# vseib/point-cloud-donkey

Hardware: AMD Instinct MI355X
Metric: objects/sec classified (ModelNet10-like, SHOT-352) (higher is better)
Workload: dtype f32; 1 GPU; configs[1]: ModelNet10-like test split, 16384 pts, 1024 uniform keypoints/object, SHOT-352 (Radius 0.4, LRF 0.3), exact kNN K=1 squared-L2, mean-shift bandwidth 0.6; points_per_object=16384, keypoints_per_object=1024, classes=10, codebook_words=102400, descriptor_dim=352, collective_world_size=1

## Files before the change

point-cloud-donkey_amd/csrc/common.h:

```cpp
#pragma once
#include <hip/hip_runtime.h>
#include <stdint.h>
#include <map>
#include <set>
#include <string>
#include <vector>
#include "../../include/ismhip.h"

#define ISM_WAVE 64

#define ISM_GRID_MAXDIM 32
#define ISM_GRID_MAXCELLS (ISM_GRID_MAXDIM * ISM_GRID_MAXDIM * ISM_GRID_MAXDIM)
#define ISM_GRID_STRIDE (ISM_GRID_MAXCELLS + 1)

#define ISM_GRID_XFRAC 3
struct GridMeta {
    float minv[3];
    float cell[3];
    float inv_cell[3];
    int   dim[3];
    float centroid[3];
    uint32_t n_finite;
};

struct ismhip_cloud {
    int n_obj = 0;
    uint32_t n_pts = 0;
    uint32_t max_pts = 0;
    std::vector<uint32_t> pt_off_h;
    uint32_t* pt_off = nullptr;
    const float *x = nullptr, *y = nullptr, *z = nullptr, *nx = nullptr, *ny = nullptr, *nz = nullptr;
    const uint32_t* rgba = nullptr;
    float4* sp4 = nullptr;
    float4* sn4 = nullptr;
    float4* slab4 = nullptr;
    uint32_t* cell_of_pt = nullptr;
    uint32_t* rank_of_pt = nullptr;
    uint32_t* members = nullptr;
    GridMeta* meta = nullptr;
    uint32_t* cell_start = nullptr;
    float requested_cell = 0.f;
    uint32_t* kp_perm = nullptr;
    size_t kp_perm_cap = 0;
    const float* kp_perm_key = nullptr;
    std::vector<uint32_t> kp_perm_off;
    uint16_t* cospair_code = nullptr;
    size_t cospair_code_cap = 0;
    bool cospair_code_valid = false;
    size_t cap_pts = 0; int cap_obj = 0; bool cap_color = false;
};

struct PcaImage {
    int m = 0;
    float* R = nullptr;
    unsigned short* f16t = nullptr;
    float* cn_scaled = nullptr;
    float* osc = nullptr;
    float sq = 1.f, sc = 1.f;
    float cmax2 = 0.f;
    float inv_sig2 = 1.f;
    float d_rel = 0.f;
    float dq_abs = 0.f, dc_abs = 0.f;
    float resid2 = 0.f;
    float energy = 0.f;
};

struct ismhip_codebook {
    int n_words = 0, dim = 0, dim_pad = 0, n_votes = 0, max_votes = 0, n_classes = 0;
    float* words = nullptr;
    int n_words_pad = 0;
    float* word_norm = nullptr;
    unsigned short* words_bf16_hi = nullptr;
    unsigned short* words_bf16_lo = nullptr;
    unsigned short* words_f16 = nullptr;
    unsigned short* words_f16t = nullptr;
    int ld16 = 0;
    float f16_scale = 1.f;
    bool words_nonneg = false;
    float max_norm2 = 0.f;
    float* word_weight = nullptr;
    uint32_t* vote_off = nullptr;
    float* vote_xyz = nullptr;
    float* vote_weight = nullptr;
    float* vote_class_weight = nullptr;
    uint32_t* vote_class = nullptr;
    uint32_t* vote_instance = nullptr;
    float* vote_bbox_quat = nullptr;
    float* vote_bbox_size = nullptr;
    float* class_sigma = nullptr;
    uint32_t* word_class = nullptr;
    float* word_keypoint = nullptr;
    ismhip_codebook* chi_shadow = nullptr;
    uint32_t* shadow_perm = nullptr;
    PcaImage pca, pca2;
    int8_t* bin_words = nullptr;
    int32_t* bin_norm = nullptr;
    int bin_ld = 0, bin_shift = 0;
};

struct TimerAcc {
    std::vector<std::pair<hipEvent_t, hipEvent_t>> pending;
    double ms = 0.0;
    int64_t launches = 0;
};

struct ismhip_ctx {
    int device = 0;
    hipStream_t stream = nullptr;
    bool own_stream = false;
    std::string err;
    bool timers_on = false;
    std::map<std::string, TimerAcc> timers;
    std::vector<hipEvent_t> event_pool;
    struct Slot { void* p = nullptr; size_t bytes = 0; };
    std::map<int, Slot> scratch;
    float* lut_srgb = nullptr;
    float* lut_sxyz = nullptr;
    std::vector<ismhip_cloud*> cloud_pool;
    uint32_t* truncated_d = nullptr;
    unsigned long long* ransac_counters_d = nullptr;
    uint32_t knn_stats[2] = {0, 0};
    std::set<const void*> attr_done;
    uint32_t knn_stage2_queries = 0;
    uint32_t knn_seed_launches = 0;
    bool knn_stage2_seed = true;
    bool knn_two_stage = true;
    bool knn_join = true;
    bool knn_qpanel2 = true;
    bool knn_half = false;
    int knn_splits = 0;
    int knn_t = 0;
    bool xcd_map = true;
    bool grid_fused = true;
    bool kp_order = true;
    float grid_xfrac = 0.f;
    int shot_var = 0;
    bool knn_hell_emit = true;
    bool knn_hellinger = true;
    int knn_t1 = 2;
    int knn_pre_step = 32;
    float knn_pre_gamma = 1.0f;
    bool knn_prepass = true;
    int knn_pca_m = -1;
    bool knn_stage2_t4 = false;
    bool codebook_light = false;
    int knn_pca_m2 = -1;
    uint32_t knn_pca_launches = 0;
    uint32_t knn_thr_overflow = 0;
    uint32_t knn_thr_mfma_launches = 0;
    bool knn_lk_fast = false;
    bool knn_lk_exact = false;
    float knn_lk_seed_scale = 1.0f;
    uint32_t knn_lk_stats[3] = {0, 0, 0};
    uint32_t knn_binary_launches = 0;
    uint32_t rank_launches = 0;
    int knn_mode = 0;
};

enum ScratchSlot {
    SCR_KP_OFF = 1, SCR_TIE_LIST, SCR_TIE_REC, SCR_TIE_KEYS, SCR_COUNTERS, SCR_KNN_CAND_IDX, SCR_KNN_CAND_VAL,
    SCR_QNORM, SCR_FPFH_FLAG, SCR_FPFH_LIST, SCR_FPFH_SPFH, SCR_FPFH_LOOKUP, SCR_SLOT_OFF, SCR_CLASS_BW,
    SCR_COMPACT_KEEP, SCR_COMPACT_POS, SCR_OBJ_COUNT, SCR_QPAD, SCR_LRF_COV, SCR_KNN_FLAGS, SCR_KNN_QSPLIT, SCR_MAX_REC, SCR_QNORM2, SCR_KNN_Q2, SCR_KNN_LIST2, SCR_TRAIN, SCR_TRAIN2, SCR_MAX_WORK, SCR_KMEANS, SCR_KNN_CLOCK, SCR_PCA, SCR_KNN_THR0, SCR_KNN_QSQRT, SCR_KNN_HELL_EMIT, SCR_KNN_THR, SCR_KNN_THR2, SCR_TRAIN_ACT, SCR_KNN_LK, SCR_KNN_LK2, SCR_KNN_LK3, SCR_PREFILTER, SCR_RANSAC, SCR_COSPAIR, SCR_KNNB_FLAG, SCR_KNNB_Q, SCR_KNNB_CAND, SCR_RANK, SCR_RANK_KNN
};

int  ism_set_err(ismhip_ctx* ctx, int code, const std::string& msg);
void* ism_scratch(ismhip_ctx* ctx, int slot, size_t bytes);
int  ism_lds_cap(ismhip_ctx* ctx, const void* kern, size_t bytes);

uint32_t* ism_upload_offsets(ismhip_ctx* ctx, int slot, const uint32_t* off_h, int n);
struct RaggedOffsets { uint32_t max_run = 0, total = 0; uint32_t* dev = nullptr; };
enum { RAGGED_START0 = 1,
       RAGGED_EMPTY = 2 };
int ism_ragged_offsets(ismhip_ctx* ctx, const std::string& name, const uint32_t* off_h, int n, int slot, int flags, RaggedOffsets* r);
int ism_offsets_from_counts(ismhip_ctx* ctx, int n, const uint32_t* cnt_d, uint32_t* off_h_out, uint32_t* max_run_out);
const uint32_t* ism_kp_order(ismhip_ctx* ctx, const ismhip_cloud* cloud, const uint32_t* kp_offsets_h, const uint32_t* ko,
                             const float* kpx, const float* kpy, const float* kpz, uint32_t maxk);

#define ISM_HIP(ctx, call)                                                                          \
    do {                                                                                            \
        hipError_t e__ = (call);                                                                    \
        if (e__ != hipSuccess)                                                                      \
            return ism_set_err((ctx), ISMHIP_ERR_HIP, std::string(#call) + ": " + hipGetErrorString(e__)); \
    } while (0)

#define ISM_CHECK_LAUNCH(ctx, name)                                                                 \
    do {                                                                                            \
        hipError_t e__ = hipGetLastError();                                                         \
        if (e__ != hipSuccess)                                                                      \
            return ism_set_err((ctx), ISMHIP_ERR_HIP, std::string("launch ") + name + ": " + hipGetErrorString(e__)); \
    } while (0)

struct TimerScope {
    ismhip_ctx* ctx; const char* name; hipEvent_t a = nullptr, b = nullptr;
    TimerScope(ismhip_ctx* c, const char* n);
    ~TimerScope();
};

#ifdef __HIPCC__
__device__ __forceinline__ int lane_id() { return threadIdx.x & 63; }

__device__ __forceinline__ float sqdist3(float ax, float ay, float az, float bx, float by, float bz) {
    float r = 0.f, d;
    d = ax - bx; r += d * d;
    d = ay - by; r += d * d;
    d = az - bz; r += d * d;
    return r;
}

template <int CTRL>
__device__ __forceinline__ int dpp_mov0(int v) { return __builtin_amdgcn_update_dpp(0, v, CTRL, 0xf, 0xf, false); }

__device__ __forceinline__ float wave_sum_f(float v) {
    v += __int_as_float(dpp_mov0<0xb1>(__float_as_int(v)));
    v += __int_as_float(dpp_mov0<0x4e>(__float_as_int(v)));
    v += __int_as_float(dpp_mov0<0x114>(__float_as_int(v)));
    v += __int_as_float(dpp_mov0<0x118>(__float_as_int(v)));
    v += __int_as_float(dpp_mov0<0x142>(__float_as_int(v)));
    v += __int_as_float(dpp_mov0<0x143>(__float_as_int(v)));
    return __int_as_float(__builtin_amdgcn_readlane(__float_as_int(v), 63));
}
__device__ __forceinline__ int wave_sum_i(int v) {
    v += dpp_mov0<0xb1>(v);
    v += dpp_mov0<0x4e>(v);
    v += dpp_mov0<0x114>(v);
    v += dpp_mov0<0x118>(v);
    v += dpp_mov0<0x142>(v);
    v += dpp_mov0<0x143>(v);
    return __builtin_amdgcn_readlane(v, 63);
}
template <int CTRL>
__device__ __forceinline__ int dpp_movi(int ident, int v) { return __builtin_amdgcn_update_dpp(ident, v, CTRL, 0xf, 0xf, false); }
__device__ __forceinline__ float wave_min_f(float v) {
    const int inf = 0x7f800000;
    v = fminf(v, __int_as_float(dpp_movi<0xb1>(inf, __float_as_int(v))));
    v = fminf(v, __int_as_float(dpp_movi<0x4e>(inf, __float_as_int(v))));
    v = fminf(v, __int_as_float(dpp_movi<0x114>(inf, __float_as_int(v))));
    v = fminf(v, __int_as_float(dpp_movi<0x118>(inf, __float_as_int(v))));
    v = fminf(v, __int_as_float(dpp_movi<0x142>(inf, __float_as_int(v))));
    v = fminf(v, __int_as_float(dpp_movi<0x143>(inf, __float_as_int(v))));
    return __int_as_float(__builtin_amdgcn_readlane(__float_as_int(v), 63));
}
template <int CTRL>
__device__ __forceinline__ unsigned long long dpp_min_u64(unsigned long long v) {
    const unsigned lo = (unsigned)dpp_movi<CTRL>(-1, (int)(unsigned)(v & 0xffffffffull)), hi = (unsigned)dpp_movi<CTRL>(-1, (int)(unsigned)(v >> 32));
    const unsigned long long o = ((unsigned long long)hi << 32) | lo;
    return o < v ? o : v;
}
__device__ __forceinline__ unsigned long long wave_min_u64(unsigned long long v) {
    v = dpp_min_u64<0xb1>(v); v = dpp_min_u64<0x4e>(v); v = dpp_min_u64<0x114>(v);
    v = dpp_min_u64<0x118>(v); v = dpp_min_u64<0x142>(v); v = dpp_min_u64<0x143>(v);
    const unsigned lo = (unsigned)__builtin_amdgcn_readlane((int)(unsigned)(v & 0xffffffffull), 63), hi = (unsigned)__builtin_amdgcn_readlane((int)(unsigned)(v >> 32), 63);
    return ((unsigned long long)hi << 32) | lo;
}
__device__ __forceinline__ float wave_max_f(float v) {
    const int ninf = (int)0xff800000;
    v = fmaxf(v, __int_as_float(dpp_movi<0xb1>(ninf, __float_as_int(v))));
    v = fmaxf(v, __int_as_float(dpp_movi<0x4e>(ninf, __float_as_int(v))));
    v = fmaxf(v, __int_as_float(dpp_movi<0x114>(ninf, __float_as_int(v))));
    v = fmaxf(v, __int_as_float(dpp_movi<0x118>(ninf, __float_as_int(v))));
    v = fmaxf(v, __int_as_float(dpp_movi<0x142>(ninf, __float_as_int(v))));
    v = fmaxf(v, __int_as_float(dpp_movi<0x143>(ninf, __float_as_int(v))));
    return __int_as_float(__builtin_amdgcn_readlane(__float_as_int(v), 63));
}
__device__ __forceinline__ uint32_t wave_max_u32(uint32_t v) {
    v = max(v, (uint32_t)dpp_mov0<0xb1>((int)v)); v = max(v, (uint32_t)dpp_mov0<0x4e>((int)v)); v = max(v, (uint32_t)dpp_mov0<0x114>((int)v));
    v = max(v, (uint32_t)dpp_mov0<0x118>((int)v)); v = max(v, (uint32_t)dpp_mov0<0x142>((int)v)); v = max(v, (uint32_t)dpp_mov0<0x143>((int)v));
    return (uint32_t)__builtin_amdgcn_readlane((int)v, 63);
}
template <int CTRL>
__device__ __forceinline__ unsigned long long dpp_mov0_u64(unsigned long long v) {
    const unsigned lo = (unsigned)dpp_mov0<CTRL>((int)(unsigned)(v & 0xffffffffull)), hi = (unsigned)dpp_mov0<CTRL>((int)(unsigned)(v >> 32));
    return ((unsigned long long)hi << 32) | lo;
}
__device__ __forceinline__ unsigned long long readlane63_u64(unsigned long long v) {
    const unsigned lo = (unsigned)__builtin_amdgcn_readlane((int)(unsigned)(v & 0xffffffffull), 63), hi = (unsigned)__builtin_amdgcn_readlane((int)(unsigned)(v >> 32), 63);
    return ((unsigned long long)hi << 32) | lo;
}
template <int CTRL>
__device__ __forceinline__ unsigned long long dpp_max_u64(unsigned long long v) { const unsigned long long o = dpp_mov0_u64<CTRL>(v); return o > v ? o : v; }
__device__ __forceinline__ unsigned long long wave_max_u64(unsigned long long v) {
    v = dpp_max_u64<0xb1>(v); v = dpp_max_u64<0x4e>(v); v = dpp_max_u64<0x114>(v);
    v = dpp_max_u64<0x118>(v); v = dpp_max_u64<0x142>(v); v = dpp_max_u64<0x143>(v);
    return readlane63_u64(v);
}
__device__ __forceinline__ unsigned long long wave_sum_u64(unsigned long long v) {
    v += dpp_mov0_u64<0xb1>(v); v += dpp_mov0_u64<0x4e>(v); v += dpp_mov0_u64<0x114>(v);
    v += dpp_mov0_u64<0x118>(v); v += dpp_mov0_u64<0x142>(v); v += dpp_mov0_u64<0x143>(v);
    return readlane63_u64(v);
}
__device__ __forceinline__ uint32_t wave_incl_scan_u32(uint32_t v) {
    int x = (int)v;
    x += dpp_mov0<0x111>(x); x += dpp_mov0<0x112>(x); x += dpp_mov0<0x114>(x); x += dpp_mov0<0x118>(x);
    x += __builtin_amdgcn_update_dpp(0, x, 0x142, 0xa, 0xf, false);
    x += __builtin_amdgcn_update_dpp(0, x, 0x143, 0xc, 0xf, false);
    return (uint32_t)x;
}
template <int NT>
struct BlockScan {
    uint32_t wave[NT / 64];
    uint32_t carry;
    __device__ __forceinline__ void init() {
        if (threadIdx.x == 0) carry = 0;
        __syncthreads();
    }
    __device__ __forceinline__ uint32_t step(uint32_t v) {
        const uint32_t incl = wave_incl_scan_u32(v);
        const int w = threadIdx.x >> 6;
        if (lane_id() == 63) wave[w] = incl;
        __syncthreads();
        uint32_t before = carry;
        for (int k = 0; k < w; ++k) before += wave[k];
        __syncthreads();
        if (threadIdx.x == NT - 1) carry = before + incl;
        __syncthreads();
        return before + incl - v;
// ... 256 lines not shown
```

point-cloud-donkey_amd/csrc/ctx.hip:

```cpp
#include "common.h"
#include <cmath>
#include <cstring>
#include <cstdlib>

extern "C" void ism_cloud_pool_release(ismhip_ctx* ctx);

int ism_set_err(ismhip_ctx* ctx, int code, const std::string& msg) {
    if (ctx) ctx->err = msg;
    return code;
}

int ism_lds_cap(ismhip_ctx* ctx, const void* kern, size_t bytes) {
    if (ctx->attr_done.count(kern)) return ISMHIP_OK;
    ISM_HIP(ctx, hipFuncSetAttribute(kern, hipFuncAttributeMaxDynamicSharedMemorySize, (int)bytes));
    ctx->attr_done.insert(kern);
    return ISMHIP_OK;
}

void* ism_scratch(ismhip_ctx* ctx, int slot, size_t bytes) {
    if (bytes == 0) bytes = 16;
    auto& s = ctx->scratch[slot];
    if (s.bytes >= bytes) return s.p;
    if (s.p) { (void)hipStreamSynchronize(ctx->stream); (void)hipFree(s.p); s.p = nullptr; s.bytes = 0; }
    size_t want = bytes + bytes / 4;
    void* p = nullptr;
    if (hipMalloc(&p, want) != hipSuccess) { ism_set_err(ctx, ISMHIP_ERR_NOMEM, "scratch hipMalloc failed"); return nullptr; }
    s.p = p; s.bytes = want;
    return p;
}

TimerScope::TimerScope(ismhip_ctx* c, const char* n) : ctx(c), name(n) {
    if (!ctx->timers_on) return;
    auto get = [&]() {
        hipEvent_t e = nullptr;
        if (!ctx->event_pool.empty()) { e = ctx->event_pool.back(); ctx->event_pool.pop_back(); }
        else (void)hipEventCreate(&e);
        return e;
    };
    a = get(); b = get();
    (void)hipEventRecord(a, ctx->stream);
}
TimerScope::~TimerScope() {
    if (!a) return;
    (void)hipEventRecord(b, ctx->stream);
    ctx->timers[name].pending.emplace_back(a, b);
}

extern "C" {

int ismhip_abi_version(void) { return ISMHIP_ABI_VERSION; }

static int ctx_create_impl(int device, void* stream, bool own, ismhip_ctx** out);

int ismhip_ctx_create(int device, void* stream, ismhip_ctx** out) { return ctx_create_impl(device, stream, stream == nullptr, out); }
int ismhip_ctx_create_on_stream(int device, void* stream, ismhip_ctx** out) { return ctx_create_impl(device, stream, false, out); }

static int ctx_create_impl(int device, void* stream, bool own, ismhip_ctx** out) {
    if (!out) return ISMHIP_ERR_INVALID;
    *out = nullptr;
    int n = 0;
    if (hipGetDeviceCount(&n) != hipSuccess || n <= 0) return ISMHIP_ERR_NODEVICE;
    if (device < 0 || device >= n) return ISMHIP_ERR_INVALID;
    if (hipSetDevice(device) != hipSuccess) return ISMHIP_ERR_HIP;
    hipDeviceProp_t prop;
    if (hipGetDeviceProperties(&prop, device) != hipSuccess) return ISMHIP_ERR_HIP;
    if (std::strncmp(prop.gcnArchName, "gfx950", 6) != 0) return ISMHIP_ERR_NODEVICE;
    ismhip_ctx* ctx = new ismhip_ctx();
    ctx->device = device;
    { const char* e = getenv("ISMHIP_KNN_MODE"); ctx->knn_mode = !e ? 0 : (!strcmp(e, "bf16x3") ? 1 : (!strcmp(e, "f32") ? 2 : 0)); }
    { const char* e = getenv("ISMHIP_XCD_MAP"); ctx->xcd_map = !(e && e[0] == '0'); }
    { const char* e = getenv("ISMHIP_GRID_FUSED"); ctx->grid_fused = !(e && e[0] == '0'); }
    { const char* e = getenv("ISMHIP_KP_ORDER"); ctx->kp_order = !(e && e[0] == '0'); }
    { const char* e = getenv("ISMHIP_GRID_XFRAC"); ctx->grid_xfrac = e ? (float)atof(e) : 0.f; }
    { const char* e = getenv("ISMHIP_SHOT_VAR"); ctx->shot_var = e ? atoi(e) : 0; }
    { const char* e = getenv("ISMHIP_KNN_TWOSTAGE"); ctx->knn_two_stage = !(e && e[0] == '0'); }
    { const char* e = getenv("ISMHIP_KNN_JOIN"); ctx->knn_join = !(e && e[0] == '0'); }
    { const char* e = getenv("ISMHIP_KNN_QPANEL2"); ctx->knn_qpanel2 = !(e && e[0] == '0'); }
    { const char* e = getenv("ISMHIP_KNN_HALF"); ctx->knn_half = e && e[0] == '1'; }
    { const char* e = getenv("ISMHIP_KNN_SPLITS"); ctx->knn_splits = e ? atoi(e) : 0; }
    { const char* e = getenv("ISMHIP_KNN_T"); ctx->knn_t = e ? atoi(e) : 0; }
    { const char* e = getenv("ISMHIP_KNN_HELL_EMIT"); ctx->knn_hell_emit = !(e && e[0] == '0'); }
    { const char* e = getenv("ISMHIP_KNN_HELLINGER"); ctx->knn_hellinger = !(e && e[0] == '0'); }
    { const char* e = getenv("ISMHIP_KNN_T1"); if (e) ctx->knn_t1 = atoi(e); }
    { const char* e = getenv("ISMHIP_KNN_STAGE2_T4"); if (e) ctx->knn_stage2_t4 = atoi(e) != 0; }
    { const char* e = getenv("ISMHIP_KNN_STAGE2_SEED"); ctx->knn_stage2_seed = !(e && e[0] == '0'); }
    { const char* e = getenv("ISMHIP_KNN_PRE_STEP"); if (e && atoi(e) > 0) ctx->knn_pre_step = atoi(e); }
    { const char* e = getenv("ISMHIP_KNN_PRE_GAMMA"); if (e) ctx->knn_pre_gamma = (float)atof(e); }
    { const char* e = getenv("ISMHIP_KNN_PREPASS"); ctx->knn_prepass = !(e && e[0] == '0'); }
    { const char* e = getenv("ISMHIP_KNN_PCA_M"); ctx->knn_pca_m = e ? atoi(e) : -1; }
    { const char* e = getenv("ISMHIP_KNN_LARGE_K_FAST"); ctx->knn_lk_fast = e && e[0] == '1'; }
    { const char* e = getenv("ISMHIP_KNN_LARGE_K_EXACT"); ctx->knn_lk_exact = e && e[0] == '1'; }
    { const char* e = getenv("ISMHIP_KNN_LARGE_K_SEED_SCALE"); if (e) ctx->knn_lk_seed_scale = (float)atof(e); }
    { const char* e = getenv("ISMHIP_KNN_PCA_M2"); ctx->knn_pca_m2 = e ? atoi(e) : -1; }
    if (!own) { ctx->stream = (hipStream_t)stream; ctx->own_stream = false; }
    else {
        if (hipStreamCreateWithFlags(&ctx->stream, hipStreamNonBlocking) != hipSuccess) { delete ctx; return ISMHIP_ERR_HIP; }
        ctx->own_stream = true;
    }
    std::vector<float> srgb(256), sxyz(4000);
    for (int i = 0; i < 256; i++) {
        float f = static_cast<float>(i) / 255.0f;
        srgb[i] = (f > 0.04045) ? powf((f + 0.055f) / 1.055f, 2.4f) : f / 12.92f;
    }
    for (int i = 0; i < 4000; i++) {
        float f = static_cast<float>(i) / 4000.0f;
        sxyz[i] = (f > 0.008856) ? static_cast<float>(powf(f, 0.3333f)) : static_cast<float>((7.787 * f) + (16.0 / 116.0));
    }
    if (hipMalloc((void**)&ctx->lut_srgb, 256 * 4) != hipSuccess || hipMalloc((void**)&ctx->lut_sxyz, 4000 * 4) != hipSuccess) {
        delete ctx; return ISMHIP_ERR_NOMEM;
    }
    (void)hipMemcpy(ctx->lut_srgb, srgb.data(), 256 * 4, hipMemcpyHostToDevice);
    (void)hipMemcpy(ctx->lut_sxyz, sxyz.data(), 4000 * 4, hipMemcpyHostToDevice);
    if (hipMalloc((void**)&ctx->truncated_d, 4) != hipSuccess) { delete ctx; return ISMHIP_ERR_NOMEM; }
    (void)hipMemset(ctx->truncated_d, 0, 4);
    (void)hipDeviceSynchronize();
    *out = ctx;
    return ISMHIP_OK;
}

int ismhip_ctx_destroy(ismhip_ctx* ctx) {
    if (!ctx) return ISMHIP_ERR_INVALID;
    (void)hipSetDevice(ctx->device);
    (void)hipStreamSynchronize(ctx->stream);
    ism_cloud_pool_release(ctx);
    for (auto& kv : ctx->scratch) if (kv.second.p) (void)hipFree(kv.second.p);
    for (auto& kv : ctx->timers) for (auto& pr : kv.second.pending) { (void)hipEventDestroy(pr.first); (void)hipEventDestroy(pr.second); }
    for (auto e : ctx->event_pool) (void)hipEventDestroy(e);
    if (ctx->lut_srgb) (void)hipFree(ctx->lut_srgb);
    if (ctx->lut_sxyz) (void)hipFree(ctx->lut_sxyz);
    if (ctx->truncated_d) (void)hipFree(ctx->truncated_d);
    if (ctx->ransac_counters_d) (void)hipFree(ctx->ransac_counters_d);
    if (ctx->own_stream) (void)hipStreamDestroy(ctx->stream);
    delete ctx;
    return ISMHIP_OK;
}

int ismhip_sync(ismhip_ctx* ctx) {
    if (!ctx) return ISMHIP_ERR_INVALID;
    if (ctx->truncated_d) {
        uint32_t n = 0;
        ISM_HIP(ctx, hipMemcpyAsync(&n, ctx->truncated_d, 4, hipMemcpyDeviceToHost, ctx->stream));
        ISM_HIP(ctx, hipStreamSynchronize(ctx->stream));
        if (n) {
            ISM_HIP(ctx, hipMemsetAsync(ctx->truncated_d, 0, 4, ctx->stream));
            ISM_HIP(ctx, hipStreamSynchronize(ctx->stream));
            return ism_set_err(ctx, ISMHIP_ERR_UNSUPPORTED, "find_maxima / hough3d_maxima: " + std::to_string(n) +
                               " (object, class) lists exceeded 128 maxima per class or 1024 per object since the last sync; the results of those objects are truncated");
        }
        return ISMHIP_OK;
    }
    ISM_HIP(ctx, hipStreamSynchronize(ctx->stream));
    return ISMHIP_OK;
}

const char* ismhip_last_error(const ismhip_ctx* ctx) { return ctx ? ctx->err.c_str() : "null ctx"; }

int ismhip_timers_enable(ismhip_ctx* ctx, int on) {
    if (!ctx) return ISMHIP_ERR_INVALID;
    ctx->timers_on = on != 0;
    return ISMHIP_OK;
}

static void resolve_timers(ismhip_ctx* ctx) {
    (void)hipStreamSynchronize(ctx->stream);
    for (auto& kv : ctx->timers) {
        for (auto& pr : kv.second.pending) {
            float ms = 0.f;
            if (hipEventElapsedTime(&ms, pr.first, pr.second) == hipSuccess) { kv.second.ms += ms; kv.second.launches++; }
            ctx->event_pool.push_back(pr.first); ctx->event_pool.push_back(pr.second);
        }
        kv.second.pending.clear();
    }
}

int ismhip_timers_reset(ismhip_ctx* ctx) {
    if (!ctx) return ISMHIP_ERR_INVALID;
    resolve_timers(ctx);
    for (auto& kv : ctx->timers) { kv.second.ms = 0; kv.second.launches = 0; }
    if (ctx->ransac_counters_d) { ISM_HIP(ctx, hipMemsetAsync(ctx->ransac_counters_d, 0, 4 * sizeof(unsigned long long), ctx->stream)); ISM_HIP(ctx, hipStreamSynchronize(ctx->stream)); }
    return ISMHIP_OK;
}

int ismhip_timer_get(ismhip_ctx* ctx, const char* name, double* ms_out, int64_t* launches_out) {
    if (!ctx || !name) return ISMHIP_ERR_INVALID;
    resolve_timers(ctx);
    if (std::strcmp(name, "knn_seed_launches") == 0) { if (ms_out) *ms_out = (double)ctx->knn_seed_launches; if (launches_out) *launches_out = 1; return ISMHIP_OK; }
    if (std::strcmp(name, "knn_binary_launches") == 0) { if (ms_out) *ms_out = (double)ctx->knn_binary_launches; if (launches_out) *launches_out = 1; return ISMHIP_OK; }
    if (std::strcmp(name, "rank_launches") == 0) { if (ms_out) *ms_out = (double)ctx->rank_launches; if (launches_out) *launches_out = 1; return ISMHIP_OK; }
    if (std::strcmp(name, "knn_pca_launches") == 0) { if (ms_out) *ms_out = (double)ctx->knn_pca_launches; if (launches_out) *launches_out = 1; return ISMHIP_OK; }
    if (std::strcmp(name, "knn_threshold_overflow_queries") == 0) { if (ms_out) *ms_out = (double)ctx->knn_thr_overflow; if (launches_out) *launches_out = 1; return ISMHIP_OK; }
    if (std::strcmp(name, "knn_threshold_mfma_launches") == 0) { if (ms_out) *ms_out = (double)ctx->knn_thr_mfma_launches; if (launches_out) *launches_out = 1; return ISMHIP_OK; }
    {
        static const char* const lk[3] = {"knn_large_k_certified_queries", "knn_large_k_retry_queries", "knn_large_k_exact_queries"};
        for (int i = 0; i < 3; ++i)
            if (std::strcmp(name, lk[i]) == 0) { if (ms_out) *ms_out = (double)ctx->knn_lk_stats[i]; if (launches_out) *launches_out = 1; return ISMHIP_OK; }
    }
    {
        static const char* const rs[4] = {"ransac_clusters", "ransac_clusters_kept", "ransac_hypotheses_needed", "ransac_hypotheses_evaluated"};
        for (int i = 0; i < 4; ++i)
            if (std::strcmp(name, rs[i]) == 0) {
                unsigned long long v[4] = {0, 0, 0, 0};
                if (ctx->ransac_counters_d) {
                    ISM_HIP(ctx, hipMemcpyAsync(v, ctx->ransac_counters_d, sizeof(v), hipMemcpyDeviceToHost, ctx->stream));
                    ISM_HIP(ctx, hipStreamSynchronize(ctx->stream));
                }
                if (ms_out) *ms_out = (double)v[i]; if (launches_out) *launches_out = 1; return ISMHIP_OK;
            }
    }
    if (std::strcmp(name, "knn_stage2_queries") == 0) { if (ms_out) *ms_out = (double)ctx->knn_stage2_queries; if (launches_out) *launches_out = 1; return ISMHIP_OK; }
    if (std::strcmp(name, "knn_flagged_queries") == 0 || std::strcmp(name, "knn_flagged_items") == 0) {
        if (ms_out) *ms_out = (double)ctx->knn_stats[name[12] == 'q' ? 0 : 1];
        if (launches_out) *launches_out = 1;
        return ISMHIP_OK;
    }
    auto it = ctx->timers.find(name);
    if (ms_out) *ms_out = it == ctx->timers.end() ? 0.0 : it->second.ms;
    if (launches_out) *launches_out = it == ctx->timers.end() ? 0 : it->second.launches;
    return ISMHIP_OK;
}

}
```

point-cloud-donkey_amd/csrc/knn.hip:

```cpp
#include "knn_internal.h"

int ism_pca_rotate_queries(ismhip_ctx* ctx, const ismhip_codebook* cb, const PcaImage* P, const float* q, int nq, int ldq, unsigned short* dst);

namespace {

__device__ __forceinline__ u16 f32_to_bf16_rn(float x) {
    const unsigned u = __float_as_uint(x);
    return (u16)((u + 0x7FFFu + ((u >> 16) & 1u)) >> 16);
}

__global__ void k_split_bf16(const float* __restrict__ src, int n, int dim, int ld, int n_pad, int dim_pad,
                             u16* __restrict__ hi, u16* __restrict__ lo) {
    const size_t i = (size_t)blockIdx.x * blockDim.x + threadIdx.x;
    if (i >= (size_t)n_pad * dim_pad) return;
    const int row = (int)(i / dim_pad), col = (int)(i % dim_pad);
    float x = 0.f;
    if (row < n && col < dim) x = src[(size_t)row * ld + col];
    const u16 h = f32_to_bf16_rn(x);
    const float hf = __uint_as_float((unsigned)h << 16);
    hi[i] = h; lo[i] = f32_to_bf16_rn(x - hf);
}


__global__ void k_absmax(const float* __restrict__ src, int n, int dim, int ld, uint32_t* __restrict__ out_bits) {
    uint32_t m = 0u;
    const size_t tot = (size_t)n * dim;
    if (ld == dim) {
        const size_t n4 = tot >> 2;
        const uint4* s4 = (const uint4*)src;
        for (size_t i = (size_t)blockIdx.x * blockDim.x + threadIdx.x; i < n4; i += (size_t)gridDim.x * blockDim.x) {
            const uint4 v = s4[i];
            const uint32_t a = max(max(v.x & 0x7fffffffu, v.y & 0x7fffffffu), max(v.z & 0x7fffffffu, v.w & 0x7fffffffu));
            m = a > m ? a : m;
        }
        for (size_t i = 4 * n4 + (size_t)blockIdx.x * blockDim.x + threadIdx.x; i < tot; i += (size_t)gridDim.x * blockDim.x) {
            const uint32_t b = __float_as_uint(src[i]) & 0x7fffffffu; m = b > m ? b : m;
        }
    } else
    for (size_t i = (size_t)blockIdx.x * blockDim.x + threadIdx.x; i < tot; i += (size_t)gridDim.x * blockDim.x) {
        const int row = (int)(i / dim), col = (int)(i % dim);
        const uint32_t b = __float_as_uint(src[(size_t)row * ld + col]) & 0x7fffffffu;
        m = b > m ? b : m;
    }
    __shared__ uint32_t s_m[4];
    m = block_max_u32(m, s_m);
    if (threadIdx.x == 0 && m) atomicMax(out_bits, m);
}
__device__ __forceinline__ float f16_image_scalars(uint32_t* __restrict__ sc, float other_scale, size_t i) {
    const float s = f16_scale_for(sc[0]);
    if (i == 0) {
        ((float*)sc)[1] = -2.0f / (s * other_scale);
        ((float*)sc)[2] = (sc[0] >> 23) == 255u ? __builtin_inff() : F16_FLUSH / s;
    }
    return s;
}
__device__ __forceinline__ u16 f16_image_element(const float* __restrict__ src, int n, int dim, int ld, size_t row, int col, float s) {
    float x = 0.f;
    if (row < (size_t)n && col < dim) x = src[row * ld + col];
    const _Float16 hx = (_Float16)(x * s);
    return __builtin_bit_cast(u16, hx);
}
__global__ void k_to_f16(const float* __restrict__ src, int n, int dim, int ld, int n_pad, int dim_pad,
                         uint32_t* __restrict__ sc, float other_scale, u16* __restrict__ dst) {
    const size_t i = (size_t)blockIdx.x * blockDim.x + threadIdx.x;
    const float s = f16_image_scalars(sc, other_scale, i);
    if (i >= (size_t)n_pad * dim_pad) return;
    dst[i] = f16_image_element(src, n, dim, ld, i / dim_pad, (int)(i % dim_pad), s);
}
__global__ void k_to_f16_tiled(const float* __restrict__ src, int n, int dim, int ld, int n_tiles, int nk,
                               uint32_t* __restrict__ sc, float other_scale, u16* __restrict__ dst) {
    const size_t i = (size_t)blockIdx.x * blockDim.x + threadIdx.x;
    const float s = f16_image_scalars(sc, other_scale, i);
    if (i >= f16t_halves(n_tiles, nk)) return;
    const int e = (int)(i & 7), p = (int)((i >> 3) & 3), r = (int)((i / F16T_KB) % F16T_ROWS);
    const size_t blk = i / F16T_BLOCK;
    const int col = (int)(blk % nk) * F16T_KB + ((p ^ f16t_swizzle(r)) << 3) + e;
    dst[i] = f16_image_element(src, n, dim, ld, blk / nk * F16T_ROWS + r, col, s);
}

__global__ void k_scale_norms(const float* __restrict__ norm, int n, const float* __restrict__ out_scale, float* __restrict__ dst) {
    const int i = blockIdx.x * blockDim.x + threadIdx.x;
    if (i < n) dst[i] = norm[i] * (1.0f / out_scale[0]);
}

#define KNN_MERGE_KEEP 16
__device__ __forceinline__ unsigned knn_sortable(float f) { const unsigned u = __float_as_uint(f); return (u & 0x80000000u) ? ~u : (u | 0x80000000u); }
__global__ __launch_bounds__(256) void k_knn_merge_splits(int nq, const float* __restrict__ cand_val, const int* __restrict__ cand_idx, int n_cand,
                                                          const float* __restrict__ cand_bound, int n_bound,
                                                          float* __restrict__ out_val, int* __restrict__ out_idx, float* __restrict__ out_bound) {
    const int qi = blockIdx.x * 4 + (threadIdx.x >> 6);
    if (qi >= nq) return;
    const int lane = lane_id();
    const float* v = cand_val + (size_t)qi * n_cand; const int* id = cand_idx + (size_t)qi * n_cand;
    unsigned long long prev = 0ull;
    bool first = true;
    float dropped = __builtin_inff();
    for (int r = 0; r <= KNN_MERGE_KEEP; ++r) {
        unsigned long long best = ~0ull;
        for (int i = lane; i < n_cand; i += 64) {
            if (id[i] < 0) continue;
            const unsigned long long key = ((unsigned long long)knn_sortable(v[i]) << 32) | (unsigned)i;
            if ((first || key > prev) && key < best) best = key;
        }
        best = wave_min_u64(best);
        if (r < KNN_MERGE_KEEP) {
            if (lane == 0) {
                const bool have = best != ~0ull;
                const int i = have ? (int)(best & 0xffffffffull) : 0;
                out_val[(size_t)qi * KNN_MERGE_KEEP + r] = have ? v[i] : __builtin_inff();
                out_idx[(size_t)qi * KNN_MERGE_KEEP + r] = have ? id[i] : -1;
            }
        } else if (best != ~0ull) dropped = v[(int)(best & 0xffffffffull)];
        if (best == ~0ull) { for (int rr = r + 1; rr < KNN_MERGE_KEEP; ++rr) if (lane == 0) { out_val[(size_t)qi * KNN_MERGE_KEEP + rr] = __builtin_inff(); out_idx[(size_t)qi * KNN_MERGE_KEEP + rr] = -1; } break; }
        prev = best; first = false;
    }
    float b = dropped;
    for (int i = lane; i < n_bound; i += 64) { const float x = cand_bound[(size_t)qi * n_bound + i]; if (x < b || x != x) b = x; }
#pragma unroll
    for (int o = 32; o > 0; o >>= 1) { const float x = __shfl_xor(b, o, 64); if (x < b || x != x) b = x; }
    if (lane == 0) out_bound[qi] = b;
}

#define KNN_HELL_CPL 4

#include "functor.h"

enum KnnCounter {
    KNN_CNT_QUERIES = 0, KNN_CNT_ITEMS = 1,
    KNN_CNT_QSC = 4,
    KNN_CNT_NEGATIVE = 12,
    KNN_CNT_WORDS = 16
};
enum KnnFbLayout { KNN_FB_TILE128 = 64, KNN_FB_TILE256 = 128, KNN_FB_RING = -1, KNN_FB_ALL = -2, KNN_FB_RING_HALF = -3 };

__device__ __forceinline__ int knn_load_cand(const int* __restrict__ cand_idx, const float* __restrict__ cand_val, int qi, int cand_stride,
                                             int j, int n_cand, int n_words, float& av) {
    int id = -1; av = __builtin_inff();
    if (j < n_cand) { id = cand_idx[(size_t)qi * cand_stride + j]; av = cand_val[(size_t)qi * cand_stride + j]; }
    if (!(id >= 0 && id < n_words)) { id = -1; av = __builtin_inff(); }
    return id;
}
template <int CPL>
__device__ __forceinline__ bool knn_select_write(unsigned long long* key, int qi, int k, int lane, int32_t* __restrict__ idx_out, float* __restrict__ dist_out, float& dk) {
    bool have_k = true;
    dk = 0.f;
    for (int j = 0; j < k; ++j) {
        unsigned long long lm = key[0];
#pragma unroll
        for (int c = 1; c < CPL; ++c) lm = key[c] < lm ? key[c] : lm;
        const unsigned long long mn = wave_min_u64(lm);
        if (lane == 0) {
            if (mn == ~0ull) { idx_out[(size_t)qi * k + j] = -1; dist_out[(size_t)qi * k + j] = __builtin_nanf(""); }
            else { idx_out[(size_t)qi * k + j] = (int)(mn & 0xffffffffull); dist_out[(size_t)qi * k + j] = __uint_as_float((unsigned)(mn >> 32)); }
        }
        if (mn == ~0ull) have_k = false; else dk = __uint_as_float((unsigned)(mn >> 32));
#pragma unroll
        for (int c = 0; c < CPL; ++c) if (key[c] == mn) key[c] = ~0ull;
    }
    return have_k;
}
__device__ __forceinline__ void knn_queue_unproven(bool viol, int qi, int lane, uint32_t* __restrict__ flag_count, uint32_t* __restrict__ qrec, uint32_t* __restrict__ items) {
    const unsigned long long vmask = __ballot(viol);
    if (vmask != 0ull) {
        const int nv = __popcll(vmask);
        uint32_t ibase = 0;
        if (lane == 0) {
            const uint32_t qs = atomicAdd(&flag_count[KNN_CNT_QUERIES], 1u);
            ibase = atomicAdd(&flag_count[KNN_CNT_ITEMS], (uint32_t)nv);
            qrec[3 * (size_t)qs] = (uint32_t)qi; qrec[3 * (size_t)qs + 1] = ibase; qrec[3 * (size_t)qs + 2] = (uint32_t)nv;
        }
        ibase = __shfl(ibase, 0, 64);
        if (viol) {
            const uint32_t it = ibase + __popcll(vmask & ((1ull << lane) - 1ull));
            items[2 * (size_t)it] = (uint32_t)qi; items[2 * (size_t)it + 1] = (uint32_t)lane;
        }
    }
}

__global__ __launch_bounds__(256) void k_knn_rerank(const float* __restrict__ words, int dim, int dim_pad, int n_words,
                                                    const float* __restrict__ q, int nq, int ldq, int metric,
                                                    const int* __restrict__ cand_idx, const float* __restrict__ cand_val, int cand_stride, int n_cand,
                                                    const float* __restrict__ cand_bound, int n_bound, VerifyParams vp,
                                                    int k, int32_t* __restrict__ idx_out, float* __restrict__ dist_out,
                                                    uint32_t* __restrict__ flag_count, uint32_t* __restrict__ qrec, uint32_t* __restrict__ items) {
    const int qi = blockIdx.x * 4 + (threadIdx.x >> 6);
    if (qi >= nq) return;
    const int lane = lane_id();
    const float* qp = q + (size_t)qi * ldq;
    const float qn2 = wave_norm2(qp, dim, lane);
    float av;
    const int id = knn_load_cand(cand_idx, cand_val, qi, cand_stride, lane, n_cand, n_words, av);
    float kth = av;
    {
        float cur = av;
        for (int j = 0; j < k; ++j) {
            const float mn = wave_min_f(cur);
            kth = mn;
            const unsigned long long eq = __ballot(cur == mn);
            if (eq && lane == __ffsll((long long)eq) - 1) cur = __builtin_inff();
        }
    }
    float slack;
    if (metric == ISMHIP_METRIC_CHI2) slack = 4.f * (((float)dim_pad + 8.f) * KNN_U + vp.ku) * fabsf(kth);
    else slack = 2.f * knn_eps_s_raw(vp, qn2) + 4.f * vp.ku * (qn2 + fabsf(kth) + vp.cmax2);
    unsigned long long key = ~0ull;
    {
        __shared__ __attribute__((aligned(16))) float s_terms[4][KNN_TERMS];
        float* sT = s_terms[threadIdx.x >> 6];
        unsigned long long need = __ballot(id >= 0 && !(av > kth + slack));
        while (need) {
            const int src = __ffsll((long long)need) - 1; need &= need - 1;
            const int cid = __shfl(id, src, 64);
            const float d = wave_functor(metric, qp, words + (size_t)cid * dim_pad, dim, lane, sT);
            if (lane == src) key = ((unsigned long long)__float_as_uint(d) << 32) | (unsigned)id;
        }
    }
    float bnd = __builtin_inff();
    if (lane < n_bound) bnd = cand_bound[(size_t)qi * n_bound + lane];
    float dk;
    const bool have_k = knn_select_write<1>(&key, qi, k, lane, idx_out, dist_out, dk);
    bool viol = false;
    const float eps_chk = metric == ISMHIP_METRIC_CHI2 ? qn2 + vp.cmax2 : knn_eps_s_raw(vp, qn2) + qn2;
    if (lane < n_bound && (bnd != __builtin_inff() || !(eps_chk < __builtin_inff()))) {
        if (!have_k) viol = true;
        else if (metric == ISMHIP_METRIC_CHI2) {
            const float lo = bnd * (1.f - ((float)dim_pad + 8.f) * KNN_U) * (1.f - vp.ku);
            viol = !(dk < lo);
        } else viol = !knn_l2_slot_proven(dk, bnd, qn2, vp);
    }
    knn_queue_unproven(viol, qi, lane, flag_count, qrec, items);
}

struct PcaVerify {
    const u16* qimg; int nk;
    float inv_sq2;
    float inv_sig2, d_rel, dq_abs, dc;
    float eps_c2, dot2, cmax2;
    float ku;
};
__device__ __forceinline__ PcaLb pca_lb_query(const PcaVerify& pv, int qi, float qn2, int lane) {
    float qn2h = 0.f;
    for (int i = lane; i < pv.nk * F16T_KB; i += 64) {
        const float v = (float)__builtin_bit_cast(_Float16, pv.qimg[f16t_stored(qi, pv.nk, i)]);
        qn2h += v * v;
    }
    PcaLb b;
    b.qn2h = wave_sum_f(qn2h) * pv.inv_sq2;
    b.dlt = pv.d_rel * (sqrtf(qn2) * 1.00001f) + pv.dq_abs + pv.dc;
    b.eps_s = (pv.eps_c2 + pv.dot2 * sqrtf(b.qn2h * pv.cmax2)) * 1.00001f;
    b.inv_sig2 = pv.inv_sig2;
    return b;
}
__global__ __launch_bounds__(256) void k_knn_rerank_pca(const float* __restrict__ words, int dim, int dim_pad, int n_words,
                                                        const float* __restrict__ q, int nq, int ldq,
                                                        const int* __restrict__ cand_idx, const float* __restrict__ cand_val, int cand_stride, int n_cand,
                                                        const float* __restrict__ cand_bound, int n_bound, PcaVerify pv,
                                                        int k, int32_t* __restrict__ idx_out, float* __restrict__ dist_out,
                                                        uint32_t* __restrict__ flag_count, uint32_t* __restrict__ qrec, uint32_t* __restrict__ items) {
    const int qi = blockIdx.x * 4 + (threadIdx.x >> 6);
    if (qi >= nq) return;
    const int lane = lane_id();
    const float* qp = q + (size_t)qi * ldq;
    const PcaLb lbq = pca_lb_query(pv, qi, wave_norm2(qp, dim, lane), lane);
    float av;
    const int id = knn_load_cand(cand_idx, cand_val, qi, cand_stride, lane, n_cand, n_words, av);
    const float lb = id >= 0 ? pca_lb_of(lbq, av) : __builtin_inff();
    bool done = id < 0;
    unsigned long long key = ~0ull;
    {
        __shared__ __attribute__((aligned(16))) float s_terms[4][KNN_TERMS];
        float* sT = s_terms[threadIdx.x >> 6];
        float kth = __builtin_inff(); int n_eval = 0;
        for (;;) {
            const float cur = done ? __builtin_inff() : lb;
            const float mn = wave_min_f(cur);
            if (!(mn < __builtin_inff())) break;
            if (n_eval >= k && mn * (1.f - pv.ku) > kth) break;
            const unsigned long long eq = __ballot(!done && cur == mn);
            const int src = __ffsll((long long)eq) - 1;
            const int cid = __shfl(id, src, 64);
            const float d = wave_functor(ISMHIP_METRIC_L2SQ, qp, words + (size_t)cid * dim_pad, dim, lane, sT);
            if (lane == src) { key = ((unsigned long long)__float_as_uint(d) << 32) | (unsigned)id; done = true; }
            if (++n_eval >= k) {
                unsigned long long kk = key, m_ = ~0ull;
                for (int j = 0; j < k; ++j) { m_ = wave_min_u64(kk); if (kk == m_) kk = ~0ull; }
                kth = __uint_as_float((unsigned)(m_ >> 32));
            }
        }
    }
    float bnd = __builtin_inff();
    if (lane < n_bound) bnd = cand_bound[(size_t)qi * n_bound + lane];
    float dk;
    const bool have_k = knn_select_write<1>(&key, qi, k, lane, idx_out, dist_out, dk);
    bool viol = false;
    if (lane < n_bound && (bnd != __builtin_inff() || !(lbq.eps_s + lbq.qn2h + lbq.dlt < __builtin_inff()))) {
        if (!have_k) viol = true;
        else viol = !pca_slot_proven(dk, bnd, lbq, pv.ku);
    }
    knn_queue_unproven(viol, qi, lane, flag_count, qrec, items);
}

__global__ __launch_bounds__(256) void k_knn_seed_thr(const float* __restrict__ q, int nq, int ldq, int dim, const float* __restrict__ seed_dk,
                                                      bool pca, PcaVerify pv, VerifyParams vp, const float* __restrict__ out_scale, float* __restrict__ thr) {
    const int qi = blockIdx.x * 4 + (threadIdx.x >> 6);
    if (qi >= nq) return;
    const int lane = lane_id();
    const float qn2 = wave_norm2(q + (size_t)qi * ldq, dim, lane);
    PcaLb lbq{};
    if (pca) lbq = pca_lb_query(pv, qi, qn2, lane);
    if (lane != 0) return;
    const float U = seed_dk[qi], osc = out_scale[0];
    float t0 = -__builtin_inff();
    if (U >= 0.f && U < __builtin_inff()) {
        float s, step;
        if (pca) {
            const float t = sqrtf((U + 1e-37f) / (lbq.inv_sig2 * (1.f - 8.f * KNN_U) * (1.f - pv.ku))) * (1.f + 4.f * KNN_U);
            const float rl = (t + lbq.dlt) / (1.f - 4.f * KNN_U);
            s = rl * rl * (1.f + 8.f * KNN_U) + lbq.eps_s - lbq.qn2h * (1.f - 16.f * KNN_U);
            step = 4.f * KNN_U * (lbq.qn2h + fabsf(s) + lbq.eps_s);
        } else {
            s = thr_tau_of(U, qn2, dim, vp);
            step = 4.f * KNN_U * (qn2 + fabsf(s) + vp.cmax2);
        }
        s += step;
        for (int it = 0; it < 24 && s < __builtin_inff(); ++it, s += step, step *= 2.f) {
            const float a = s / osc;
            if (pca ? pca_slot_proven(U, osc * a, lbq, pv.ku) : knn_l2_slot_proven(U, osc * a, qn2, vp)) { t0 = a; break; }
        }
    }
    thr[qi] = t0;
}

#define CHI_FAST_CH 6
__device__ __forceinline__ void chi2_fast_load_q(const float* __restrict__ qp, int n4, int lane, f32x4* qv) {
#pragma unroll
    for (int j = 0; j < CHI_FAST_CH; ++j) { const int g = lane + 64 * j; qv[j] = g < n4 ? *(const f32x4*)(qp + 4 * g) : f32x4{0.f, 0.f, 0.f, 0.f}; }
}
__device__ __forceinline__ float chi2_fast(const f32x4* qv, const float* __restrict__ wp, int n4, int lane) {
    f32x4 wv[CHI_FAST_CH];
#pragma unroll
    for (int j = 0; j < CHI_FAST_CH; ++j) { const int g = lane + 64 * j; wv[j] = g < n4 ? *(const f32x4*)(wp + 4 * g) : f32x4{0.f, 0.f, 0.f, 0.f}; }
    float part = 0.f;
#pragma unroll
    for (int j = 0; j < CHI_FAST_CH; ++j)
#pragma unroll
        for (int e = 0; e < 4; ++e) { const float sm = qv[j][e] + wv[j][e], df = qv[j][e] - wv[j][e]; part += sm > 0.f ? df * df / sm : 0.f; }
    return wave_sum_f(part);
}

__global__ __launch_bounds__(256) void k_knn_rerank_hell(const float* __restrict__ words, int dim, int dim_pad, int n_words,
                                                         const float* __restrict__ q, int nq, int ldq, const float* __restrict__ sq ,
                                                         const uint32_t* __restrict__ perm ,
                                                         const int* __restrict__ cand_idx, const float* __restrict__ cand_val, int cand_stride, int n_cand,
                                                         const float* __restrict__ cand_bound, int n_bound, VerifyParams vp,
                                                         int k, int32_t* __restrict__ idx_out, float* __restrict__ dist_out,
                                                         uint32_t* __restrict__ flag_count, uint32_t* __restrict__ qrec, uint32_t* __restrict__ items) {
    const int qi = blockIdx.x * 4 + (threadIdx.x >> 6);
    if (qi >= nq) return;
    const int lane = lane_id();
    const float* qp = q + (size_t)qi * ldq;
    const float qn2 = wave_norm2(sq + (size_t)qi * dim_pad, dim, lane);
    const float eps_s = knn_eps_s(vp, qn2);
    auto lb_of = [&](float s) -> float {
        float L = qn2 * (1.f - 16.f * KNN_U) + s - eps_s;
        L -= 4.f * KNN_U * (qn2 + fabsf(s));
        return L > 0.f ? L : 0.f;
    };
    int id[KNN_HELL_CPL]; float lb[KNN_HELL_CPL], fd[KNN_HELL_CPL]; unsigned long long key[KNN_HELL_CPL];
#pragma unroll
    for (int c = 0; c < KNN_HELL_CPL; ++c) {
        float av;
        const int x = knn_load_cand(cand_idx, cand_val, qi, cand_stride, lane + 64 * c, n_cand, n_words, av);
        id[c] = -1; lb[c] = __builtin_inff(); fd[c] = __builtin_inff(); key[c] = ~0ull;
        if (x >= 0) { id[c] = (int)perm[x]; lb[c] = lb_of(av); }
    }
    const float mg = 4.f * vp.ku;
    float kth_fast = __builtin_inff();
    {
        const int n4 = (ldq >= dim_pad ? dim_pad : dim) >> 2;
        f32x4 qv[CHI_FAST_CH];
        chi2_fast_load_q(qp, n4, lane, qv);
        int n_eval = 0;
        for (;;) {
            float cur = lb[0];
#pragma unroll
            for (int c = 1; c < KNN_HELL_CPL; ++c) cur = fminf(cur, lb[c]);
            const float mn = wave_min_f(cur);
            if (!(mn < __builtin_inff())) break;
            if (n_eval >= k && mn * (1.f - vp.ku) > kth_fast * (1.f + mg)) break;
            const unsigned long long eq = __ballot(cur == mn);
            const int src = __ffsll((long long)eq) - 1;
            int mine = -1, cs = 0;
#pragma unroll
            for (int c = KNN_HELL_CPL - 1; c >= 0; --c) if (lb[c] == mn) { mine = id[c]; cs = c; }
            const int cid = __shfl(mine, src, 64);
            float d = chi2_fast(qv, words + (size_t)cid * dim_pad, n4, lane);
            if (d != d) d = 0.f;
            if (lane == src) {
#pragma unroll
                for (int c = 0; c < KNN_HELL_CPL; ++c) if (c == cs) { fd[c] = d; lb[c] = __builtin_inff(); }
            }
            if (++n_eval >= k) {
                float ff[KNN_HELL_CPL], m_ = __builtin_inff();
#pragma unroll
                for (int c = 0; c < KNN_HELL_CPL; ++c) ff[c] = fd[c];
                for (int j = 0; j < k; ++j) {
                    float lm = ff[0];
#pragma unroll
                    for (int c = 1; c < KNN_HELL_CPL; ++c) lm = fminf(lm, ff[c]);
                    m_ = wave_min_f(lm);
                    const unsigned long long e2 = __ballot(lm == m_);
                    if (lane == __ffsll((long long)e2) - 1) {
                        bool gone = false;
#pragma unroll
                        for (int c = 0; c < KNN_HELL_CPL; ++c) if (!gone && ff[c] == m_) { ff[c] = __builtin_inff(); gone = true; }
                    }
                }
                kth_fast = m_;
            }
        }
    }
    {
        __shared__ __attribute__((aligned(16))) float s_terms[4][KNN_TERMS];
        float* sT = s_terms[threadIdx.x >> 6];
        const float win = kth_fast * (1.f + 3.f * mg);
        for (;;) {
            int mine = -1, cs = 0;
#pragma unroll
            for (int c = KNN_HELL_CPL - 1; c >= 0; --c) if (fd[c] <= win && key[c] == ~0ull && id[c] >= 0) { mine = id[c]; cs = c; }
            const unsigned long long pend = __ballot(mine >= 0);
            if (pend == 0ull) break;
            const int src = __ffsll((long long)pend) - 1;
            const int cid = __shfl(mine, src, 64);
            const float d = wave_functor(ISMHIP_METRIC_CHI2, qp, words + (size_t)cid * dim_pad, dim, lane, sT);
            if (lane == src) {
#pragma unroll
                for (int c = 0; c < KNN_HELL_CPL; ++c) if (c == cs) { key[c] = ((unsigned long long)__float_as_uint(d) << 32) | (unsigned)id[c]; fd[c] = __builtin_inff(); }
            }
        }
    }
    float bnd = __builtin_inff();
    if (lane < n_bound) bnd = cand_bound[(size_t)qi * n_bound + lane];
    float dk;
    const bool have_k = knn_select_write<KNN_HELL_CPL>(key, qi, k, lane, idx_out, dist_out, dk);
    bool viol = false;
    if (lane < n_bound && (bnd != __builtin_inff() || !(eps_s + qn2 < __builtin_inff()))) {
        if (!have_k) viol = true;
        else viol = !(dk < lb_of(bnd) * (1.f - vp.ku) - 1e-37f);
    }
    knn_queue_unproven(viol, qi, lane, flag_count, qrec, items);
}

#define KNN_FB_UNITS 8192u
__host__ __device__ inline uint32_t knn_fb_parts(uint32_t n_items) {
    if (n_items == 0 || n_items > KNN_FB_UNITS / 2) return 1u;
    const uint32_t p = KNN_FB_UNITS / n_items;
    return p > 256u ? 256u : p;
}
template <int KM>
__global__ __launch_bounds__(256) void k_knn_fallback(const float* __restrict__ words, int dim, int dim_pad, int n_words,
                                                      const float* __restrict__ q, int ldq, int metric, int k, int tiles_per_split, int n_tiles,
                                                      int tile_rows, int wr_rows ,
                                                      const uint32_t* __restrict__ flag_count, const uint32_t* __restrict__ items,
                                                      const int32_t* __restrict__ idx_in, const float* __restrict__ dist_in,
                                                      unsigned long long* __restrict__ item_out, size_t part_base) {
    __shared__ __attribute__((aligned(16))) float s_terms[4][KNN_TERMS];
    const int lane = threadIdx.x & 63;
    const int g = lane >> 4, l16 = lane & 15;
    const uint32_t n_items = flag_count[KNN_CNT_ITEMS];
    const bool l2 = metric != ISMHIP_METRIC_CHI2;
    const bool lay_all = l2 && wr_rows == KNN_FB_ALL;
    const bool lay16 = l2 && wr_rows == KNN_FB_RING;
    const bool lay16h = l2 && wr_rows == KNN_FB_RING_HALF;
    const int rows_per_tile = lay_all ? tile_rows : ((lay16 || lay16h) ? 32 : (l2 ? wr_rows / 2 : tile_rows));
    const int nj = dim_pad / 16;
    const uint32_t gw = blockIdx.x * 4 + (threadIdx.x >> 6), nw = gridDim.x * 4;
    const uint32_t P = knn_fb_parts(n_items);
    unsigned long long* outp = P > 1 ? item_out + KM * part_base : item_out;
    for (uint32_t u = gw; u < n_items * P; u += nw) {
        const uint32_t it = u / P, part_i = u % P;
        const int qi = (int)items[2 * (size_t)it], b = (int)items[2 * (size_t)it + 1];
        const float* qp = q + (size_t)qi * ldq;
        const int split = lay_all ? 0 : (lay16 ? (b >> 3) : (l2 ? (b >> 2) : b));
        const int wr = lay16h ? 0 : (lay16 ? (b >> 2) & 1 : (b >> 1) & 1), h = b & 1, fq = b & 3;
        const int mt0 = split * tiles_per_split, mt1 = min(n_tiles, mt0 + tiles_per_split);
        const int total = (mt1 - mt0) * rows_per_tile;
        unsigned long long best[KM];
#pragma unroll
        for (int j = 0; j < KM; ++j) best[j] = ~0ull;
        float thr = __builtin_inff();
        {
            const int id = idx_in[(size_t)qi * k + (k - 1)];
            if (id >= 0) thr = dist_in[(size_t)qi * k + (k - 1)];
        }
        const int steps = (total + 3) / 4;
        const int e_beg = 4 * (int)((long long)steps * part_i / P), e_end = min(total, 4 * (int)((long long)steps * (part_i + 1) / P));
        for (int e0 = e_beg; e0 < e_end; e0 += 4) {
            const int e = e0 + g;
            int r = n_words;
            if (e < e_end) {
                const int tile = mt0 + e / rows_per_tile, y = e % rows_per_tile;
                const int x = lay_all ? y : ((lay16 || lay16h) ? (wr * 128 + ((y >> 2) << 4) + (fq << 2) + (y & 3)) : (l2 ? (wr * wr_rows + (((y >> 2) << 3) | (h << 2) | (y & 3))) : y));
                r = tile * tile_rows + x;
            }
            float part = 0.f;
            if (r < n_words) {
                const float* wp = words + (size_t)r * dim_pad;
                if (!l2) { for (int j = 0; j < nj; ++j) { const int i = l16 + 16 * j; const float a = i < dim ? qp[i] : 0.f, c = wp[i], sm = a + c, df = a - c; part += sm > 0.f ? df * df / sm : 0.f; } }
                else { for (int j = 0; j < nj; ++j) { const int i = l16 + 16 * j; const float df = (i < dim ? qp[i] : 0.f) - wp[i]; part += df * df; } }
            }
#pragma unroll
            for (int o = 8; o > 0; o >>= 1) part += __shfl_xor(part, o, 64);
            const bool hit = r < n_words && !(part > thr * 1.0001f + 1e-30f);
            unsigned long long hm = __ballot(hit && l16 == 0);
            while (hm) {
                const int src = __ffsll((long long)hm) - 1; hm &= hm - 1;
                const int rr = __shfl(r, src, 64);
                const float d = wave_functor(metric, qp, words + (size_t)rr * dim_pad, dim, lane, s_terms[threadIdx.x >> 6]);
                unsigned long long key = ((unsigned long long)__float_as_uint(d) << 32) | (unsigned)rr;
                if (d != d) key = (0x7fc00000ull << 32) | (unsigned)rr;
#pragma unroll
                for (int j = 0; j < KM; ++j) if (j < k && key < best[j]) { const unsigned long long tmp = best[j]; best[j] = key; key = tmp; }
                unsigned long long kth = ~0ull;
#pragma unroll
                for (int j = 0; j < KM; ++j) if (j == k - 1) kth = best[j];
                if (kth != ~0ull) thr = fminf(thr, __uint_as_float((unsigned)(kth >> 32)));
            }
        }
#pragma unroll
        for (int j = 0; j < KM; ++j) if (lane == j) outp[KM * (size_t)u + j] = best[j];
    }
}

template <int KM>
__global__ __launch_bounds__(256) void k_knn_fallback_merge(int k, const uint32_t* __restrict__ flag_count, const uint32_t* __restrict__ qrec,
                                     const unsigned long long* __restrict__ item_out, size_t part_base, int32_t* __restrict__ idx_out, float* __restrict__ dist_out) {
    const uint32_t n_q = flag_count[KNN_CNT_QUERIES];
    const uint32_t P = knn_fb_parts(flag_count[KNN_CNT_ITEMS]);
    const unsigned long long* outp = P > 1 ? item_out + KM * part_base : item_out;
    const int lane = threadIdx.x & 63;
    for (uint32_t t = blockIdx.x * 4 + (threadIdx.x >> 6); t < n_q; t += gridDim.x * 4) {
        const int qi = (int)qrec[3 * (size_t)t]; const uint32_t ibase = qrec[3 * (size_t)t + 1], ni = qrec[3 * (size_t)t + 2];
        unsigned long long fin[KM];
#pragma unroll
        for (int j = 0; j < KM; ++j) fin[j] = ~0ull;
        auto ins = [&](unsigned long long key) {
#pragma unroll
            for (int j = 0; j < KM; ++j) if (fin[j] != ~0ull && (fin[j] & 0xffffffffull) == (key & 0xffffffffull)) return;
#pragma unroll
            for (int j = 0; j < KM; ++j) if (key < fin[j]) { const unsigned long long tmp = fin[j]; fin[j] = key; key = tmp; }
        };
        if (lane < k) {
            const int id = idx_out[(size_t)qi * k + lane];
            if (id >= 0) ins(((unsigned long long)__float_as_uint(dist_out[(size_t)qi * k + lane]) << 32) | (unsigned)id);
        }
        for (uint32_t i = lane; i < ni * P; i += 64)
            for (int j = 0; j < k; ++j) { const unsigned long long key = outp[KM * ((size_t)ibase * P + i) + j]; if (key != ~0ull) ins(key); }
        for (int j = 0; j < k; ++j) {
            const unsigned long long mn = wave_min_u64(fin[0]);
            if (lane == 0) {
                if (mn == ~0ull) { idx_out[(size_t)qi * k + j] = -1; dist_out[(size_t)qi * k + j] = __builtin_nanf(""); }
                else { idx_out[(size_t)qi * k + j] = (int)(mn & 0xffffffffull); dist_out[(size_t)qi * k + j] = __uint_as_float((unsigned)(mn >> 32)); }
            }
            if (mn == ~0ull) continue;
            bool gone = false;
#pragma unroll
            for (int x = 0; x < KM; ++x) {
                if (!gone && fin[x] != ~0ull && (fin[x] & 0xffffffffull) == (mn & 0xffffffffull)) gone = true;
                if (gone) fin[x] = x + 1 < KM ? fin[x + 1] : ~0ull;
            }
        }
    }
}

__global__ void k_pad_rows(const float* __restrict__ src, int n, int dim, float* __restrict__ dst, int dim_pad) {
    const size_t i = (size_t)blockIdx.x * blockDim.x + threadIdx.x;
    if (i >= (size_t)n * dim_pad) return;
    const int row = (int)(i / dim_pad), col = (int)(i % dim_pad);
    dst[i] = col < dim ? src[(size_t)row * dim + col] : 0.f;
}

__global__ void k_ratio(int nq, float thr, const int32_t* __restrict__ idx2, const float* __restrict__ d2,
                        int32_t* __restrict__ idx_out, float* __restrict__ dist_out) {
    const int i = blockIdx.x * blockDim.x + threadIdx.x;
    if (i >= nq) return;
    int id = idx2[i * 2]; const float a = d2[i * 2], b = d2[i * 2 + 1];
    if (idx2[i * 2 + 1] >= 0 && a / b > thr) id = -1;
    idx_out[i] = id; dist_out[i] = a;
}

__global__ void k_rule(int nq, float thr, const int32_t* __restrict__ idx3, const float* __restrict__ d3, const uint32_t* __restrict__ word_class,
                       int32_t* __restrict__ idx_out, float* __restrict__ dist_out) {
    const int i = blockIdx.x * blockDim.x + threadIdx.x;
    if (i >= nq) return;
    const int i0 = idx3[i * 3], i1 = idx3[i * 3 + 1], i2 = idx3[i * 3 + 2];
    const float a = d3[i * 3], b = d3[i * 3 + 1], c = d3[i * 3 + 2];
    int id = -1; float dd = __builtin_nanf("");
    if (i2 < 0) {
        if (i0 >= 0) { id = i0; dd = a; }
    } else {
        const uint32_t c0 = word_class[i0], c1 = word_class[i1], c2 = word_class[i2];
        if (c0 == c1 && c0 == c2) { id = i0; dd = a; }
        else if (c0 == c1 && c0 != c2) { if (a / c < thr) { id = i0; dd = a; } }
        else if (c0 != c1 && c1 == c2) { if (a / b >= thr) { id = i1; dd = b; } }
        else if (c0 != c1 && c1 != c2) { if (a / b < thr) { id = i0; dd = a; } }
    }
    idx_out[i] = id; dist_out[i] = dd;
}

struct KnnStage1 { uint32_t* flag_count; uint32_t* qrec; };
struct KnnRequest {
    KnnStage1* stage1 = nullptr;
    const char* tname = nullptr;
    bool many_splits = false;
    int use_pca = 0;
    const float* hell_q = nullptr;
    bool half = false;
    const float* seed_dk = nullptr;
};

enum KnnCand { KNN_CAND_F32, KNN_CAND_CHI2, KNN_CAND_MFMA16, KNN_CAND_RING16 };
struct KnnPlan {
    bool hell;
    int mode;
    KnnCand cand;
    const void* kern;
    int BM, BN, threads;
    bool big_tile, half, qpanel2, pca, merged, prepass, seeded, join;
    int slots, ring_nk;
    int n_qt, n_splits, tiles_per_split, cand_per_split, n_cand, n_bound;
    int fb_tiles_per_split; KnnFbLayout fb_layout;
    size_t lds, lds_cap;
};

KnnPlan knn_plan(const ismhip_ctx* ctx, const ismhip_codebook* cb, int metric, int nq, int k, int T, const KnnRequest& rq) {
    KnnPlan p{};
    p.hell = rq.hell_q != nullptr && metric == ISMHIP_METRIC_CHI2 && cb->chi_shadow;
    const ismhip_codebook* xb = p.hell ? cb->chi_shadow : cb;
    const bool l2 = p.hell || metric == ISMHIP_METRIC_L2SQ;
    const PcaImage& PI = rq.use_pca == 2 ? cb->pca2 : cb->pca;
    const bool short_dim = cb->dim <= 64 && ctx->knn_mode == 0 && !(rq.use_pca && PI.m > 0);
    p.mode = !l2 ? -1 : (p.hell ? 0 : (short_dim ? 2 : (ctx->knn_mode == 0 && cb->words_f16 ? 0 : (ctx->knn_mode <= 1 && cb->words_bf16_hi ? 1 : 2))));
    const bool use_lp = p.mode == 0 || p.mode == 1;
    p.big_tile = use_lp && nq >= 4096 && cb->n_words_pad >= 4096;
    const bool ring = p.big_tile && p.mode == 0 && xb->words_f16t && (cb->dim + 15) / 16 > 2;
    p.half = ring && (rq.half || ctx->knn_half);
    p.qpanel2 = ring && !p.half && ctx->knn_qpanel2 && rq.use_pca && PI.m > 0 && PI.m <= 160;
    p.pca = rq.use_pca && ring && PI.m > 0;
    p.ring_nk = p.pca ? PI.m / 32 : ((cb->dim + 15) / 16 + 1) / 2;
    p.merged = rq.many_splits && l2 && use_lp && !p.big_tile;
    p.join = ring && ctx->knn_join;
    p.BM = !l2 ? CHI_B : (p.half ? 128 : (p.big_tile ? 256 : KNN_BM));
    p.BN = !l2 ? CHI_B : (p.big_tile ? 256 : KNN_BN);
    p.slots = ring && !p.half ? 8 : 4;
    p.n_qt = (nq + p.BN - 1) / p.BN;
    const int n_mt = cb->n_words_pad / p.BM;
    if (l2) {
        const int max_s = (p.hell ? 64 * KNN_HELL_CPL : 64) / (p.slots * T);
        p.n_splits = std::max(1, std::min(std::min(max_s, n_mt), std::max(p.pca ? 2 : 3, (1024 + p.n_qt - 1) / p.n_qt)));
        if (p.big_tile && p.n_qt >= 512) p.n_splits = std::min(p.n_splits, std::max(1, n_mt / 32));
        if (p.hell) p.n_splits = std::max(1, std::min(std::min(max_s, 8), n_mt / 4));
        if (ctx->knn_splits > 0) p.n_splits = std::max(1, std::min(std::min(max_s, n_mt), ctx->knn_splits));
        if (p.merged) p.n_splits = std::max(1, std::min(n_mt, (1024 + 8 * ((p.n_qt + 7) / 8) - 1) / (8 * ((p.n_qt + 7) / 8))));
        p.cand_per_split = p.slots * T;
    } else {
        const int max_s = 64 / T;
        p.n_splits = std::max(1, std::min(std::min(max_s, n_mt), (2048 + p.n_qt - 1) / p.n_qt));
        if (k > T) p.n_splits = std::max(p.n_splits, std::min(std::min(max_s, n_mt), (2 * k + T - 1) / T));
        p.cand_per_split = T;
    }
    p.tiles_per_split = (n_mt + p.n_splits - 1) / p.n_splits;
    p.n_splits = (n_mt + p.tiles_per_split - 1) / p.tiles_per_split;
    p.n_cand = p.n_splits * p.cand_per_split;
    p.n_bound = l2 ? p.n_splits * p.slots : p.n_splits;
    p.prepass = rq.stage1 && ring && !p.half && ctx->knn_prepass && n_mt >= 128 && !(p.pca && PI.resid2 <= 0.f);
    p.seeded = rq.seed_dk && ring && !p.prepass;
    p.fb_tiles_per_split = p.merged ? n_mt : p.tiles_per_split;
    p.fb_layout = p.merged ? KNN_FB_ALL : (p.half ? KNN_FB_RING_HALF : (ring ? KNN_FB_RING : (p.big_tile ? KNN_FB_TILE256 : KNN_FB_TILE128)));
    p.threads = 256;
    if (!l2) p.cand = KNN_CAND_CHI2;
    else if (!use_lp) p.cand = KNN_CAND_F32;
    else if (ring) {
        p.cand = KNN_CAND_RING16;
        p.threads = p.half ? 256 : 512;
        if (p.half) { p.kern = knn_ring16_kernel(T, 1, 0); p.lds = p.lds_cap = Ring16Lds<1, 0>::total(0); }
        else if (p.qpanel2) { p.kern = knn_ring16_kernel(T, 2, 2); p.lds = Ring16Lds<2, 2>::total(p.ring_nk); p.lds_cap = Ring16Lds<2, 2>::total(160 / 32); }
        else { p.kern = knn_ring16_kernel(T, 2, 0); p.lds = p.lds_cap = Ring16Lds<2, 0>::total(0); }
    } else {
        p.cand = KNN_CAND_MFMA16;
        p.threads = p.big_tile ? 512 : 256;
        p.kern = knn_mfma16_kernel(T, p.mode, p.big_tile);
        p.lds = p.lds_cap = knn_mfma16_lds(p.BM, p.BN, p.mode == 1 ? 32 : 64, p.mode == 1 ? 3 : 1);
    }
    return p;
}

struct KnnScratch {
    float *cand_val, *cand_bound; int* cand_idx; int n_cand, n_bound;
    uint32_t *flag_count, *qrec, *items; unsigned long long* item_out; size_t q_items;
    uint32_t* qsc;
};
struct KnnRun : KnnScratch {
    ismhip_ctx* ctx; const ismhip_codebook *cb, *xb; const PcaImage* PI; const KnnRequest* rq; KnnPlan p;
    int metric, nq, k, T;
    const float* qq; int ldq;
    u16 *q_hi, *q_lo;
};

int knn_carve_scratch(KnnRun& r) {
    const KnnPlan& p = r.p; const size_t nq = (size_t)r.nq;
    r.n_cand = p.n_cand; r.n_bound = p.n_bound; r.q_items = nq * p.n_bound;
    r.cand_val = (float*)ism_scratch(r.ctx, SCR_KNN_CAND_VAL, nq * (p.n_cand + p.n_bound + (p.merged ? KNN_MERGE_KEEP + 1 : 0)) * sizeof(float));
    r.cand_idx = (int*)ism_scratch(r.ctx, SCR_KNN_CAND_IDX, nq * (p.n_cand + (p.merged ? KNN_MERGE_KEEP : 0)) * sizeof(int));
    r.flag_count = (uint32_t*)ism_scratch(r.ctx, SCR_KNN_FLAGS, (KNN_CNT_WORDS + 3 * nq + 2 * r.q_items) * sizeof(uint32_t) + 8 + (r.q_items + KNN_FB_UNITS) * (r.k > 4 ? KNN_MAX_K : 4) * sizeof(unsigned long long));
    if (!r.cand_val || !r.cand_idx || !r.flag_count) return ISMHIP_ERR_NOMEM;
    r.cand_bound = r.cand_val + nq * p.n_cand;
    r.qrec = r.flag_count + KNN_CNT_WORDS; r.items = r.qrec + 3 * nq; r.qsc = r.flag_count + KNN_CNT_QSC;
    r.item_out = (unsigned long long*)(((uintptr_t)(r.items + 2 * r.q_items) + 7) & ~(uintptr_t)7);
    ISM_HIP(r.ctx, hipMemsetAsync(r.flag_count, 0, KNN_CNT_WORDS * sizeof(uint32_t), r.ctx->stream));
    return ISMHIP_OK;
}

int knn_query_images(KnnRun& r) {
    ismhip_ctx* ctx = r.ctx; const ismhip_codebook* cb = r.cb; const KnnPlan& p = r.p; const int nq = r.nq;
    if (p.mode != 0 && p.mode != 1) return ISMHIP_OK;
    const bool ring = p.cand == KNN_CAND_RING16;
    const int nq_pad = ring ? (nq + F16T_ROWS - 1) / F16T_ROWS * F16T_ROWS : (nq + p.BN - 1) / p.BN * p.BN;
    const size_t tot = ring ? f16t_halves(nq_pad / F16T_ROWS, p.ring_nk) : (size_t)nq_pad * cb->ld16;
    r.q_hi = (u16*)ism_scratch(ctx, SCR_KNN_QSPLIT, tot * 2 * sizeof(u16));
    if (!r.q_hi) return ISMHIP_ERR_NOMEM;
    r.q_lo = r.q_hi + tot;
    if (p.pca) {
        TimerScope tr(ctx, "knn_rotate");
        const int rc = ism_pca_rotate_queries(ctx, cb, r.PI, r.qq, nq, r.ldq, r.q_hi);
        if (rc != ISMHIP_OK) return rc;
        ++ctx->knn_pca_launches;
    } else if (p.mode == 0) {
        const float* cq = p.hell ? r.rq->hell_q : r.qq; const int cldq = p.hell ? cb->dim_pad : r.ldq;
        hipLaunchKernelGGL(k_absmax, dim3(512), dim3(256), 0, ctx->stream, cq, nq, cb->dim, cldq, r.qsc);
        ISM_CHECK_LAUNCH(ctx, "k_absmax");
        if (ring) hipLaunchKernelGGL(k_to_f16_tiled, dim3((unsigned)((tot + 255) / 256)), dim3(256), 0, ctx->stream, cq, nq, cb->dim, cldq, nq_pad / F16T_ROWS, p.ring_nk, r.qsc, r.xb->f16_scale, r.q_hi);
        else hipLaunchKernelGGL(k_to_f16, dim3((unsigned)((tot + 255) / 256)), dim3(256), 0, ctx->stream, cq, nq, cb->dim, cldq, nq_pad, cb->ld16, r.qsc, r.xb->f16_scale, r.q_hi);
        ISM_CHECK_LAUNCH(ctx, "k_to_f16");
    } else {
        hipLaunchKernelGGL(k_split_bf16, dim3((unsigned)((tot + 255) / 256)), dim3(256), 0, ctx->stream, r.qq, nq, cb->dim, r.ldq, nq_pad, cb->ld16, r.q_hi, r.q_lo);
        ISM_CHECK_LAUNCH(ctx, "k_split_bf16");
    }
    return ISMHIP_OK;
}

PcaVerify knn_pca_verify(const KnnRun& r, const VerifyParams& vp) {
    const PcaImage& PI = *r.PI;
    PcaVerify pv;
    const float acc_rel = 1.01f * (float)PI.m * 1.1920929e-07f;
    pv.qimg = r.q_hi; pv.nk = r.p.ring_nk; pv.inv_sq2 = 1.0f / (PI.sq * PI.sq);
    pv.inv_sig2 = PI.inv_sig2; pv.d_rel = PI.d_rel; pv.dq_abs = PI.dq_abs;
    pv.dc = (PI.d_rel * sqrtf(r.cb->max_norm2) + PI.dc_abs) * 1.00001f;
    pv.cmax2 = PI.cmax2;
    const float fq = F16_FLUSH / PI.sq, fc = F16_FLUSH / PI.sc, sm = sqrtf((float)PI.m);
    pv.eps_c2 = (17.f * KNN_U + 1.01f * (float)(PI.m + 1) * 1.1920929e-07f) * PI.cmax2 + 2.02f * (sm * fq * sqrtf(PI.cmax2) + sm * sm * fq * fc);
    pv.dot2 = 2.f * acc_rel + 2.f * KNN_U + 2.02f * sm * fc / sqrtf(PI.cmax2);
    pv.ku = vp.ku;
    return pv;
}

int knn_launch_candidates(KnnRun& r) {
    ismhip_ctx* ctx = r.ctx; const ismhip_codebook *cb = r.cb, *xb = r.xb; const KnnPlan& p = r.p; const PcaImage& PI = *r.PI; const int nq = r.nq;
    {
        TimerScope ts(ctx, r.rq->tname ? r.rq->tname : (r.metric == ISMHIP_METRIC_L2SQ ? "knn_l2_mfma" : "knn_chi2"));
        const unsigned grid = 8 * ((p.n_qt + 7) / 8) * p.n_splits;
        KnnCandArgs a{};
        a.n_tiles_m = cb->n_words_pad / p.BM; a.ld = cb->ld16; a.k_steps = p.pca ? PI.m / 16 : (cb->dim + 15) / 16;
        a.qh = r.q_hi; a.ql = r.q_lo; a.nq = nq; a.out_scale = (const float*)(r.qsc + 1);
        a.tiles_per_split = p.tiles_per_split; a.n_splits = p.n_splits;
        a.cand_val = r.cand_val; a.cand_idx = r.cand_idx; a.cand_stride = r.n_cand; a.cand_bound = r.cand_bound; a.bound_stride = r.n_bound;
        int rc = ISMHIP_OK;
        if (p.cand == KNN_CAND_RING16) {
            rc = ism_lds_cap(ctx, p.kern, p.lds_cap);
            if (rc != ISMHIP_OK) return rc;
            a.wh = xb->words_f16t;
            if (p.pca) { a.wh = PI.f16t; a.out_scale = PI.osc; a.word_norm = PI.cn_scaled; }
            else {
                float* cn_scaled = (float*)ism_scratch(ctx, SCR_QNORM2, ((size_t)cb->n_words_pad + 256) * sizeof(float));
                if (!cn_scaled) return ISMHIP_ERR_NOMEM;
                hipLaunchKernelGGL(k_scale_norms, dim3((cb->n_words_pad + 255) / 256), dim3(256), 0, ctx->stream, xb->word_norm, cb->n_words_pad, a.out_scale, cn_scaled);
                ISM_CHECK_LAUNCH(ctx, "k_scale_norms");
                a.word_norm = cn_scaled;
            }
            unsigned int* clock = nullptr;
            if (p.join) {
                clock = (unsigned int*)ism_scratch(ctx, SCR_KNN_CLOCK, 8 * 64 * sizeof(unsigned int));
                if (!clock) return ISMHIP_ERR_NOMEM;
                ISM_HIP(ctx, hipMemsetAsync(clock, 0, 8 * 64 * sizeof(unsigned int), ctx->stream));
            }
            float* thr0 = nullptr;
            float relax = 0.f;
            if (p.prepass || p.seeded) {
                thr0 = (float*)ism_scratch(ctx, SCR_KNN_THR0, (size_t)((nq + 255) / 256 * 256) * sizeof(float));
                if (!thr0) return ISMHIP_ERR_NOMEM;
                if (p.pca) relax = -ctx->knn_pre_gamma * 2.0f * PI.resid2 * (PI.sq * PI.sc * 0.5f);
            }
            if (p.seeded) {
                const VerifyParams vp = knn_verify_params(xb, cb->dim_pad, p.mode, r.qsc, true);
                hipLaunchKernelGGL(k_knn_seed_thr, dim3((nq + 3) / 4), dim3(256), 0, ctx->stream, r.qq, nq, r.ldq, cb->dim, r.rq->seed_dk,
                                   p.pca, p.pca ? knn_pca_verify(r, vp) : PcaVerify{}, vp, a.out_scale, thr0);
                ISM_CHECK_LAUNCH(ctx, "k_knn_seed_thr");
                ++ctx->knn_seed_launches;
            }
            rc = knn_ring16_launch(ctx, r.T, p.kern, grid, p.threads, p.lds, a, clock, thr0, p.prepass ? ctx->knn_pre_step : 0, relax);
        } else if (p.cand == KNN_CAND_MFMA16) {
            rc = ism_lds_cap(ctx, p.kern, p.lds_cap);
            if (rc != ISMHIP_OK) return rc;
            a.wh = p.mode == 0 ? xb->words_f16 : xb->words_bf16_hi;
            a.wl = p.mode == 0 ? nullptr : xb->words_bf16_lo;
            a.word_norm = xb->word_norm;
            rc = knn_mfma16_launch(ctx, p.kern, grid, p.threads, p.lds, a, nullptr, nullptr, nullptr, 0);
        } else if (p.cand == KNN_CAND_F32) {
            rc = knn_l2_f32_launch(ctx, r.T, grid, cb, r.qq, nq, r.ldq, p.tiles_per_split, p.n_splits, r.cand_val, r.cand_idx, r.n_cand, r.cand_bound, r.n_bound);
        } else {
            rc = knn_chi2_launch(ctx, r.T, p.n_qt, cb, r.qq, nq, r.ldq, r.flag_count + KNN_CNT_NEGATIVE, p.tiles_per_split, p.n_splits, r.cand_val, r.cand_idx, r.n_cand, r.cand_bound, r.n_bound);
        }
        if (rc != ISMHIP_OK) return rc;
    }
    if (p.merged) {
        float* m_val = r.cand_bound + (size_t)nq * r.n_bound; float* m_bound = m_val + (size_t)nq * KNN_MERGE_KEEP;
        int* m_idx = r.cand_idx + (size_t)nq * r.n_cand;
        hipLaunchKernelGGL(k_knn_merge_splits, dim3((nq + 3) / 4), dim3(256), 0, ctx->stream, nq, r.cand_val, r.cand_idx, r.n_cand, r.cand_bound, r.n_bound, m_val, m_idx, m_bound);
        ISM_CHECK_LAUNCH(ctx, "k_knn_merge_splits");
        r.cand_val = m_val; r.cand_idx = m_idx; r.cand_bound = m_bound; r.n_cand = KNN_MERGE_KEEP; r.n_bound = 1;
    }
    return ISMHIP_OK;
}

int knn_rerank_prove(KnnRun& r, int32_t* idx_out, float* dist_out) {
    ismhip_ctx* ctx = r.ctx; const ismhip_codebook* cb = r.cb; const KnnPlan& p = r.p;
    const VerifyParams vp = knn_verify_params(r.xb, cb->dim_pad, p.mode, r.qsc, true);
    const dim3 grid((r.nq + 3) / 4), block(256);
    TimerScope trr(ctx, "knn_rerank");
    if (p.pca) {
        const PcaVerify pv = knn_pca_verify(r, vp);
        hipLaunchKernelGGL(k_knn_rerank_pca, grid, block, 0, ctx->stream, cb->words, cb->dim, cb->dim_pad, cb->n_words,
                           r.qq, r.nq, r.ldq, r.cand_idx, r.cand_val, r.n_cand, r.n_cand, r.cand_bound, r.n_bound, pv, r.k, idx_out, dist_out, r.flag_count, r.qrec, r.items);
    } else if (p.hell) {
        hipLaunchKernelGGL(k_knn_rerank_hell, grid, block, 0, ctx->stream, cb->words, cb->dim, cb->dim_pad, cb->n_words,
                           r.qq, r.nq, r.ldq, r.rq->hell_q, r.xb->shadow_perm, r.cand_idx, r.cand_val, r.n_cand, r.n_cand, r.cand_bound, r.n_bound, vp, r.k, idx_out, dist_out, r.flag_count, r.qrec, r.items);
    } else
    hipLaunchKernelGGL(k_knn_rerank, grid, block, 0, ctx->stream, cb->words, cb->dim, cb->dim_pad, cb->n_words,
                       r.qq, r.nq, r.ldq, r.metric, r.cand_idx, r.cand_val, r.n_cand, r.n_cand, r.cand_bound, r.n_bound, vp, r.k, idx_out, dist_out, r.flag_count, r.qrec, r.items);
    ISM_CHECK_LAUNCH(ctx, "k_knn_rerank");
    return ISMHIP_OK;
}

int knn_exact_scan(KnnRun& r, int32_t* idx_out, float* dist_out) {
    ismhip_ctx* ctx = r.ctx; const ismhip_codebook* cb = r.cb; const KnnPlan& p = r.p; const int k = r.k;
    TimerScope ts(ctx, "knn_fallback");
    const int n_tiles = cb->n_words_pad / p.BM;
    const auto scan = k <= 4 ? k_knn_fallback<4> : k_knn_fallback<KNN_MAX_K>;
    const auto merge = k <= 4 ? k_knn_fallback_merge<4> : k_knn_fallback_merge<KNN_MAX_K>;
    hipLaunchKernelGGL(scan, dim3(1024), dim3(256), 0, ctx->stream, cb->words, cb->dim, cb->dim_pad, cb->n_words, r.qq, r.ldq, r.metric, k,
                       p.fb_tiles_per_split, n_tiles, p.BM, (int)p.fb_layout, r.flag_count, r.items, idx_out, dist_out, r.item_out, r.q_items);
    ISM_CHECK_LAUNCH(ctx, "k_knn_fallback");
    hipLaunchKernelGGL(merge, dim3(256), dim3(256), 0, ctx->stream, k, r.flag_count, r.qrec, r.item_out, r.q_items, idx_out, dist_out);
    ISM_CHECK_LAUNCH(ctx, "k_knn_fallback_merge");
    return ISMHIP_OK;
}

int run_knn(ismhip_ctx* ctx, const ismhip_codebook* cb, int metric, int nq, const float* q, int k, int T,
            int32_t* idx_out, float* dist_out, const KnnRequest& rq = KnnRequest()) {
    if (cb->dim_pad / 16 > KNN_FB_MAXJ) return ism_set_err(ctx, ISMHIP_ERR_UNSUPPORTED, "knn: descriptor longer than 1344 not built");
    KnnRun r{};
    r.ctx = ctx; r.cb = cb; r.rq = &rq; r.metric = metric; r.nq = nq; r.k = k; r.T = T;
    r.p = knn_plan(ctx, cb, metric, nq, k, T, rq);
    if (r.p.cand == KNN_CAND_MFMA16 && !r.p.kern) return ism_set_err(ctx, ISMHIP_ERR_UNSUPPORTED, "knn: f16 256x256 tile without the ring not built");
    r.xb = r.p.hell ? cb->chi_shadow : cb;
    r.PI = rq.use_pca == 2 ? &cb->pca2 : &cb->pca;
    r.qq = q; r.ldq = cb->dim;
    if (cb->dim_pad != cb->dim) {
        float* qpad = (float*)ism_scratch(ctx, SCR_QPAD, (size_t)nq * cb->dim_pad * sizeof(float));
        if (!qpad) return ISMHIP_ERR_NOMEM;
        const size_t tot = (size_t)nq * cb->dim_pad;
        hipLaunchKernelGGL(k_pad_rows, dim3((unsigned)((tot + 255) / 256)), dim3(256), 0, ctx->stream, q, nq, cb->dim, qpad, cb->dim_pad);
        ISM_CHECK_LAUNCH(ctx, "k_pad_rows");
        r.qq = qpad; r.ldq = cb->dim_pad;
    }
    int rc = knn_carve_scratch(r);
    if (rc == ISMHIP_OK) rc = knn_query_images(r);
    if (rc == ISMHIP_OK) rc = knn_launch_candidates(r);
    if (rc == ISMHIP_OK) rc = knn_rerank_prove(r, idx_out, dist_out);
    if (rc != ISMHIP_OK) return rc;
    if (rq.stage1) { *rq.stage1 = KnnStage1{r.flag_count, r.qrec}; return ISMHIP_OK; }
    rc = knn_exact_scan(r, idx_out, dist_out);
    if (rc != ISMHIP_OK) return rc;
    if (ctx->timers_on) ISM_HIP(ctx, hipMemcpyAsync(ctx->knn_stats, r.flag_count, 8, hipMemcpyDeviceToHost, ctx->stream));
    return ISMHIP_OK;
}

__global__ __launch_bounds__(256) void k_knn_gather_flagged(const uint32_t* __restrict__ qrec, int n2, const float* __restrict__ q, int dim,
                                                            float* __restrict__ q2, uint32_t* __restrict__ list2,
                                                            const int32_t* __restrict__ idx1, const float* __restrict__ dist1, int k, float* __restrict__ dk2) {
    const int i = blockIdx.x;
    if (i >= n2) return;
    const uint32_t qi = qrec[3 * (size_t)i];
    if (threadIdx.x == 0) {
        list2[i] = qi;
        if (dk2) dk2[i] = idx1[(size_t)qi * k + (k - 1)] >= 0 ? dist1[(size_t)qi * k + (k - 1)] : __builtin_nanf("");
    }
    for (int c = threadIdx.x; c < dim; c += blockDim.x) q2[(size_t)i * dim + c] = q[(size_t)qi * dim + c];
}
__global__ void k_knn_scatter_results(const uint32_t* __restrict__ list2, int n2, int k, const int32_t* __restrict__ idx2, const float* __restrict__ dist2,
                                      int32_t* __restrict__ idx_out, float* __restrict__ dist_out) {
    const int t = blockIdx.x * blockDim.x + threadIdx.x;
    if (t >= n2 * k) return;
    const size_t o = (size_t)list2[t / k] * k + (t % k);
    idx_out[o] = idx2[t]; dist_out[o] = dist2[t];
}

struct KnnStage2 { int n2; float* q2; uint32_t* list2; int32_t* idx2; float* dist2; float* dk2; };
int knn_gather_stage2(ismhip_ctx* ctx, const ismhip_codebook* cb, const KnnStage1& s1, const float* q, int k, KnnStage2& g,
                      const int32_t* idx1, const float* dist1) {
    uint32_t n2u = 0;
    ISM_HIP(ctx, hipMemcpyAsync(&n2u, s1.flag_count, 4, hipMemcpyDeviceToHost, ctx->stream));
    ISM_HIP(ctx, hipStreamSynchronize(ctx->stream));
    ctx->knn_stage2_queries = n2u;
    const int n2 = g.n2 = (int)n2u;
    if (n2 == 0) { ctx->knn_stats[0] = ctx->knn_stats[1] = 0; return ISMHIP_OK; }
    g.q2 = (float*)ism_scratch(ctx, SCR_KNN_Q2, (size_t)n2 * cb->dim * sizeof(float));
    g.list2 = (uint32_t*)ism_scratch(ctx, SCR_KNN_LIST2, (size_t)n2 * (sizeof(uint32_t) + (size_t)k * (sizeof(int32_t) + sizeof(float)) + (idx1 ? sizeof(float) : 0)));
    if (!g.q2 || !g.list2) return ISMHIP_ERR_NOMEM;
    g.idx2 = (int32_t*)(g.list2 + n2);
    g.dist2 = (float*)(g.idx2 + (size_t)n2 * k);
    g.dk2 = idx1 ? g.dist2 + (size_t)n2 * k : nullptr;
    hipLaunchKernelGGL(k_knn_gather_flagged, dim3(n2), dim3(256), 0, ctx->stream, s1.qrec, n2, q, cb->dim, g.q2, g.list2, idx1, dist1, k, g.dk2);
    ISM_CHECK_LAUNCH(ctx, "k_knn_gather_flagged");
    return ISMHIP_OK;
}
int knn_scatter_stage2(ismhip_ctx* ctx, const KnnStage2& g, int k, int32_t* idx_out, float* dist_out) {
    hipLaunchKernelGGL(k_knn_scatter_results, dim3((g.n2 * k + 255) / 256), dim3(256), 0, ctx->stream, g.list2, g.n2, k, g.idx2, g.dist2, idx_out, dist_out);
    ISM_CHECK_LAUNCH(ctx, "k_knn_scatter_results");
    return ISMHIP_OK;
}

int run_knn_two_stage(ismhip_ctx* ctx, const ismhip_codebook* cb, int nq, const float* q, int k, int32_t* idx_out, float* dist_out) {
    KnnStage1 s1{};
    KnnRequest r1; r1.stage1 = &s1; r1.use_pca = 1;
    int rc = run_knn(ctx, cb, ISMHIP_METRIC_L2SQ, nq, q, k, ctx->knn_t1 == 1 && k == 1 ? 1 : 2, idx_out, dist_out, r1);
    if (rc != ISMHIP_OK) return rc;
    KnnStage2 g;
    const bool seed = ctx->knn_stage2_seed;
    rc = knn_gather_stage2(ctx, cb, s1, q, k, g, seed ? idx_out : nullptr, seed ? dist_out : nullptr);
    if (rc != ISMHIP_OK || g.n2 == 0) return rc;
    const int n2 = g.n2;
    for (int o = 0; o < n2;) {
        const int left = n2 - o, n = left >= 32768 ? left / 32768 * 32768 : left;
        KnnRequest r2; r2.tname = "knn_stage2"; r2.many_splits = n < 4096;
        r2.use_pca = cb->pca2.m > 0 && !(n < 4096) ? 2 : 0;
        r2.half = n >= 4096 && n < 32768 && !ctx->knn_stage2_t4;
        r2.seed_dk = g.dk2 ? g.dk2 + o : nullptr;
        rc = run_knn(ctx, cb, ISMHIP_METRIC_L2SQ, n, g.q2 + (size_t)o * cb->dim, k, 4, g.idx2 + (size_t)o * k, g.dist2 + (size_t)o * k, r2);
        if (rc != ISMHIP_OK) return rc;
        o += n;
    }
    return knn_scatter_stage2(ctx, g, k, idx_out, dist_out);
}


__global__ void k_sqrt_rows(const float* __restrict__ src, int n, int dim, int ld, int dim_pad, float* __restrict__ dst, uint32_t* __restrict__ flag) {
    const size_t i = (size_t)blockIdx.x * blockDim.x + threadIdx.x;
    bool bad = false;
    if (i < (size_t)n * dim_pad) {
        const int row = (int)(i / dim_pad), col = (int)(i % dim_pad);
        float v = 0.f;
        if (col < dim) { v = src[(size_t)row * ld + col]; bad = !(v >= 0.f); }
        dst[i] = sqrtf(v);
    }
    if (__any(bad) && (threadIdx.x & 63) == 0) atomicOr(flag, 1u);
}

#define HELL_EMIT_CAP 2048
__global__ __launch_bounds__(256) void k_hell_tau(int n2, const uint32_t* __restrict__ list2, const float* __restrict__ sq2, int dim, int dim_pad,
                                                  const float* __restrict__ dist_out, VerifyParams vp, float* __restrict__ tau) {
    const int i = blockIdx.x * 4 + (threadIdx.x >> 6);
    if (i >= n2) return;
    const int lane = lane_id();
    const float qn2 = wave_norm2(sq2 + (size_t)i * dim_pad, dim, lane);
    if (lane == 0) {
        const float dk = dist_out[list2[i]];
        const float eps_s = knn_eps_s(vp, qn2);
        float t = dk * (1.f + 2.f * vp.ku) - qn2 * (1.f - 16.f * KNN_U) + eps_s + 8.f * KNN_U * (qn2 + vp.cmax2 + dk);
        if (!(dk == dk)) t = __builtin_inff();
        tau[i] = t;
    }
}
__global__ __launch_bounds__(256) void k_hell_eval(int n2, const uint32_t* __restrict__ list2, const uint32_t* __restrict__ cnt, const uint32_t* __restrict__ rows, int cap,
                                                   const uint32_t* __restrict__ perm, const float* __restrict__ q, int dim, const float* __restrict__ words, int dim_pad, float ku,
                                                   int32_t* __restrict__ idx_out, float* __restrict__ dist_out, uint32_t* __restrict__ overflow) {
    __shared__ float s_fast[HELL_EMIT_CAP];
    __shared__ __attribute__((aligned(16))) float s_terms[KNN_TERMS];
    const int i = blockIdx.x;
    const int lane = lane_id(), wv = threadIdx.x >> 6;
    const uint32_t qi = list2[i];
    const uint32_t n = cnt[i];
    if (n > (uint32_t)cap) { if (threadIdx.x == 0) atomicAdd(overflow, 1u); return; }
    const float* qp = q + (size_t)qi * dim;
    {
        const int n4 = dim >> 2;
        f32x4 qv[CHI_FAST_CH];
        chi2_fast_load_q(qp, n4, lane, qv);
        for (uint32_t s_ = wv; s_ < n; s_ += 4) {
            const float part = chi2_fast(qv, words + (size_t)perm[rows[(size_t)i * cap + s_]] * dim_pad, n4, lane);
            if (lane == 0) s_fast[s_] = part;
        }
    }
    __syncthreads();
    if (wv != 0) return;
    float mn = __builtin_inff();
    for (uint32_t s_ = lane; s_ < n; s_ += 64) mn = fminf(mn, s_fast[s_]);
    mn = wave_min_f(mn);
    const float win = mn * (1.f + 12.f * ku);
    unsigned long long best = ~0ull;
    {
        const int id0 = idx_out[qi];
        if (id0 >= 0) best = ((unsigned long long)__float_as_uint(dist_out[qi]) << 32) | (unsigned)id0;
    }
    for (uint32_t s0 = 0; s0 < n; s0 += 64) {
        const uint32_t s_ = s0 + lane;
        const bool in = s_ < n && !(s_fast[s_] > win);
        unsigned long long pend = __ballot(in);
        const int row = in ? (int)perm[rows[(size_t)i * cap + s_]] : -1;
        while (pend) {
            const int src = __ffsll((long long)pend) - 1; pend &= pend - 1;
            const int cid = __shfl(row, src, 64);
            const float d = wave_functor(ISMHIP_METRIC_CHI2, qp, words + (size_t)cid * dim_pad, dim, lane, s_terms);
            const unsigned long long key = ((unsigned long long)__float_as_uint(d) << 32) | (unsigned)cid;
            best = key < best ? key : best;
        }
    }
    if (lane == 0 && best != ~0ull) { idx_out[qi] = (int)(best & 0xffffffffull); dist_out[qi] = __uint_as_float((unsigned)(best >> 32)); }
}

int run_knn_chi2_hellinger(ismhip_ctx* ctx, const ismhip_codebook* cb, int nq, const float* q, int k, int32_t* idx_out, float* dist_out, bool& taken) {
    taken = false;
    float* sq = (float*)ism_scratch(ctx, SCR_KNN_QSQRT, (size_t)nq * cb->dim_pad * sizeof(float) + 16);
    if (!sq) return ISMHIP_ERR_NOMEM;
    bool neg = false;
    int rc = knn_sqrt_queries(ctx, cb, nq, q, sq, neg);
    if (rc != ISMHIP_OK || neg) return rc;
    taken = true;
    KnnStage1 s1{};
    KnnRequest rh; rh.stage1 = &s1; rh.hell_q = sq;
    rc = run_knn(ctx, cb, ISMHIP_METRIC_CHI2, nq, q, k, 4, idx_out, dist_out, rh);
    if (rc != ISMHIP_OK) return rc;
    KnnStage2 g;
    rc = knn_gather_stage2(ctx, cb, s1, q, k, g, nullptr, nullptr);
    if (rc != ISMHIP_OK || g.n2 == 0) return rc;
    const int n2 = g.n2;
    uint32_t* list2 = g.list2;
    if (k == 1 && ctx->knn_hell_emit) {
        uint32_t over = 0;
        {
        TimerScope t2(ctx, "knn_stage2");
        const ismhip_codebook* xb = cb->chi_shadow;
        const int dp = cb->dim_pad, cap = HELL_EMIT_CAP;
        const int n2p = (n2 + 127) / 128 * 128;
        const size_t b_sq2 = (size_t)n2 * dp * 4, b_tau = (size_t)n2p * 4, b_cnt = (size_t)n2p * 4 + 64, b_rows = (size_t)n2 * cap * 4, b_img = (size_t)n2p * cb->ld16 * 2;
        char* buf = (char*)ism_scratch(ctx, SCR_KNN_HELL_EMIT, b_sq2 + b_tau + b_cnt + b_rows + b_img + 64);
        if (!buf) return ISMHIP_ERR_NOMEM;
        float* sq2 = (float*)buf; float* tau = (float*)(buf + b_sq2); uint32_t* cnt = (uint32_t*)(buf + b_sq2 + b_tau);
        uint32_t* sc = cnt + n2p;
        uint32_t* rows = (uint32_t*)(buf + b_sq2 + b_tau + b_cnt); u16* qimg = (u16*)(buf + b_sq2 + b_tau + b_cnt + b_rows);
        ISM_HIP(ctx, hipMemsetAsync(cnt, 0, b_cnt, ctx->stream));
        hipLaunchKernelGGL(k_knn_gather_flagged, dim3(n2), dim3(256), 0, ctx->stream, s1.qrec, n2, (const float*)sq, dp, sq2, list2,
                           (const int32_t*)nullptr, (const float*)nullptr, k, (float*)nullptr);
        ISM_CHECK_LAUNCH(ctx, "k_knn_gather_flagged");
        rc = knn_f16_emit_image(ctx, cb, xb, sq2, n2, dp, n2p, sc, qimg);
        if (rc != ISMHIP_OK) return rc;
        const VerifyParams vp = knn_verify_params(xb, dp, 0, sc, false);
        hipLaunchKernelGGL(k_hell_tau, dim3((n2 + 3) / 4), dim3(256), 0, ctx->stream, n2, (const uint32_t*)list2, (const float*)sq2, cb->dim, dp, (const float*)dist_out, vp, tau);
        ISM_CHECK_LAUNCH(ctx, "k_hell_tau");
        rc = knn_mfma16_emit(ctx, cb, xb, n2, n2p, sc, qimg, tau, cnt, rows, cap);
        if (rc != ISMHIP_OK) return rc;
        hipLaunchKernelGGL(k_hell_eval, dim3(n2), dim3(256), 0, ctx->stream, n2, (const uint32_t*)list2, (const uint32_t*)cnt, (const uint32_t*)rows, cap,
                           (const uint32_t*)xb->shadow_perm, q, cb->dim, (const float*)cb->words, dp, vp.ku, idx_out, dist_out, sc + 8);
        ISM_CHECK_LAUNCH(ctx, "k_hell_eval");
        ISM_HIP(ctx, hipMemcpyAsync(&over, sc + 8, 4, hipMemcpyDeviceToHost, ctx->stream));
        ISM_HIP(ctx, hipStreamSynchronize(ctx->stream));
        }
        ctx->knn_stats[0] = over; ctx->knn_stats[1] = 0;
        if (over == 0) return ISMHIP_OK;
    }
    {
        TimerScope t2(ctx, "knn_stage2");
        KnnRequest rv; rv.tname = "knn_chi2_valu";
        rc = run_knn(ctx, cb, ISMHIP_METRIC_CHI2, g.n2, g.q2, k, k > 2 ? 4 : 2, g.idx2, g.dist2, rv);
        if (rc != ISMHIP_OK) return rc;
    }
    return knn_scatter_stage2(ctx, g, k, idx_out, dist_out);
}

}

int knn_sqrt_queries(ismhip_ctx* ctx, const ismhip_codebook* cb, int nq, const float* q, float* sq, bool& negative) {
    uint32_t* flag = (uint32_t*)(sq + (size_t)nq * cb->dim_pad);
    ISM_HIP(ctx, hipMemsetAsync(flag, 0, 4, ctx->stream));
    const size_t tot = (size_t)nq * cb->dim_pad;
    hipLaunchKernelGGL(k_sqrt_rows, dim3((unsigned)((tot + 255) / 256)), dim3(256), 0, ctx->stream, q, nq, cb->dim, cb->dim, cb->dim_pad, sq, flag);
    ISM_CHECK_LAUNCH(ctx, "k_sqrt_rows");
    uint32_t neg = 0;
    ISM_HIP(ctx, hipMemcpyAsync(&neg, flag, 4, hipMemcpyDeviceToHost, ctx->stream));
    ISM_HIP(ctx, hipStreamSynchronize(ctx->stream));
    negative = neg != 0;
// ... 92 lines not shown
```

point-cloud-donkey_amd/csrc/knn_internal.h:

```cpp
#pragma once
#include "common.h"

namespace {

typedef float f32x16 __attribute__((ext_vector_type(16)));
typedef float f32x4 __attribute__((ext_vector_type(4)));
typedef __bf16 bf16x8 __attribute__((ext_vector_type(8)));
typedef unsigned short u16;
typedef _Float16 f16x8 __attribute__((ext_vector_type(8)));

#define KNN_BM 128
#define KNN_BN 128
#define CHI_B 64
#define KNN_MAX_K 16
#define KNN_FB_MAXJ 84
#define KNN_TERMS (16 * KNN_FB_MAXJ)

template <int T>
struct TopT {
    float v[T]; int i[T];
    __device__ __forceinline__ void init() {
#pragma unroll
        for (int t = 0; t < T; ++t) { v[t] = __builtin_inff(); i[t] = -1; }
    }
    __device__ __forceinline__ void push_flat(float x, int idx) {
        bool c[T];
#pragma unroll
        for (int t = 0; t < T; ++t) c[t] = x < v[t];
#pragma unroll
        for (int t = T - 1; t > 0; --t) {
            v[t] = c[t - 1] ? v[t - 1] : (c[t] ? x : v[t]);
            i[t] = c[t - 1] ? i[t - 1] : (c[t] ? idx : i[t]);
        }
        v[0] = c[0] ? x : v[0];
        i[0] = c[0] ? idx : i[0];
    }
    __device__ __forceinline__ void push(float x, int idx) {
        if (!(x < v[T - 1])) return;
        v[T - 1] = x; i[T - 1] = idx;
#pragma unroll
        for (int t = T - 1; t > 0; --t) {
            if (v[t] < v[t - 1]) {
                float tv = v[t]; v[t] = v[t - 1]; v[t - 1] = tv;
                int ti = i[t]; i[t] = i[t - 1]; i[t - 1] = ti;
            }
        }
    }
};

constexpr size_t knn_mfma16_lds(int BM, int BN, int KB, int NTERM) { return (size_t)2 * (BM + BN) * KB * sizeof(u16) * (NTERM == 3 ? 2 : 1) + BM * sizeof(float); }
#define RG_BN 256
#define RG_KB 32
template <int WR, int QP>
struct Ring16Lds {
    static constexpr int STAGES = WR == 2 ? 4 : 3, STAGE_HALVES = (QP ? WR * 128 : WR * 128 + RG_BN) * RG_KB;
    static constexpr size_t cn = (size_t)STAGES * STAGE_HALVES * sizeof(u16);
    static constexpr size_t thr = cn + 4 * 256 * sizeof(float);
    static constexpr size_t panel = thr + (WR == 2 ? 8 * 4 * 64 * sizeof(float) : 0);
    static constexpr size_t total(int ring_nk) { return panel + (QP ? (size_t)ring_nk * 256 * RG_KB * sizeof(u16) : 0); }
};

#define F16_FLUSH 6.103515625e-05f
__host__ __device__ inline float f16_scale_for(uint32_t bits) {
    const int e = (int)(bits >> 23);
    if (e == 0 || e == 255) return 1.0f;
    int k = 13 - (e - 127);
    k = k > 40 ? 40 : (k < -40 ? -40 : k);
    return __builtin_bit_cast(float, (uint32_t)(127 + k) << 23);
}
#define F16T_ROWS 256
#define F16T_KB 32
#define F16T_BLOCK (F16T_ROWS * F16T_KB)
__host__ __device__ inline size_t f16t_halves(size_t n_tiles, int nk) { return n_tiles * nk * F16T_BLOCK; }
__device__ __forceinline__ int f16t_swizzle(int r) { return (0x78 >> (2 * ((r >> 2) & 3))) & 3; }
__device__ __forceinline__ size_t f16t_row(size_t tile, int r, int nk, int kc) { return ((tile * nk + kc) * F16T_ROWS + r) * F16T_KB; }
__device__ __forceinline__ size_t f16t_stored(unsigned row, int nk, unsigned h) { return f16t_row(row / F16T_ROWS, row % F16T_ROWS, nk, h / F16T_KB) + h % F16T_KB; }

struct VerifyParams {
    float ku;
    float dot_rel;
    float cmax2;
    float dabs_c;
    const float* dabs_q;
    float sqrt_dim;
    float cn_acc;
};
__device__ __forceinline__ float knn_abs_err(const VerifyParams& vp, float qn2) {
    if (!vp.dabs_q) return 0.f;
    const float dq = vp.dabs_q[0], dc = vp.dabs_c;
    return 1.01f * (vp.sqrt_dim * (dq * sqrtf(vp.cmax2) + dc * sqrtf(qn2)) + vp.sqrt_dim * vp.sqrt_dim * dq * dc);
}
#define KNN_U 5.9604645e-08f
__device__ __forceinline__ float knn_eps_s_raw(const VerifyParams& vp, float qn2) {
    return 17.f * KNN_U * vp.cmax2 + (2.f * vp.dot_rel + 2.f * KNN_U) * sqrtf(qn2 * vp.cmax2) + 2.f * knn_abs_err(vp, qn2) + vp.cn_acc * vp.cmax2;
}
__device__ __forceinline__ float knn_eps_s(const VerifyParams& vp, float qn2) { return knn_eps_s_raw(vp, qn2) * 1.00001f; }
__device__ __forceinline__ float wave_norm2(const float* __restrict__ x, int dim, int lane) {
    float s = 0.f;
    for (int i = lane; i < dim; i += 64) { const float v = x[i]; s += v * v; }
    return wave_sum_f(s);
}

VerifyParams knn_verify_params(const ismhip_codebook* xb, int dim_pad, int mode, const uint32_t* qsc, bool cn_acc) {
    VerifyParams vp;
    vp.ku = 1.01f * (float)dim_pad * KNN_U;
    vp.dot_rel = mode == 0 ? (2.002f * 4.8828125e-04f + 1.01f * (float)dim_pad * 1.1920929e-07f)
               : mode == 1 ? (3.1f * 1.52587890625e-05f + 1.01f * 3.f * (float)dim_pad * 1.1920929e-07f) : vp.ku;
    vp.cmax2 = xb->max_norm2;
    vp.dabs_c = mode == 0 ? F16_FLUSH / xb->f16_scale : 0.f;
    vp.dabs_q = mode == 0 ? (const float*)(qsc + 2) : nullptr;
    vp.sqrt_dim = sqrtf((float)dim_pad);
    vp.cn_acc = mode == 0 && cn_acc ? 1.01f * (float)(dim_pad + 1) * 1.1920929e-07f : 0.f;
    return vp;
}

__device__ __forceinline__ float thr_tau_of(float thr, float qn2, int dim, const VerifyParams& vp) {
    const float eps_s = knn_eps_s(vp, qn2);
    float t = thr * (1.f + 2.f * vp.ku) - qn2 * (1.f - 16.f * KNN_U) + eps_s + 8.f * KNN_U * (qn2 + vp.cmax2 + thr)
            + (float)(dim / 64 + 8) * KNN_U * qn2;
    if (!(fabsf(t) < __builtin_inff())) t = __builtin_inff();
    return t;
}

__device__ __forceinline__ bool knn_l2_slot_proven(float dk, float bnd, float qn2, const VerifyParams& vp) {
    const float eps_s = knn_eps_s_raw(vp, qn2);
    const float rhs = qn2 * (1.f - 16.f * KNN_U) + bnd - eps_s;
    return dk < rhs - vp.ku * fabsf(rhs) - 1e-37f;
}
struct PcaLb { float qn2h, eps_s, dlt, inv_sig2; };
__device__ __forceinline__ float pca_lb_of(const PcaLb& b, float s) {
    float L = b.qn2h * (1.f - 16.f * KNN_U) + s - b.eps_s;
    L -= 4.f * KNN_U * (b.qn2h + fabsf(s));
    if (!(L > 0.f)) return 0.f;
    const float t = sqrtf(L) * (1.f - 4.f * KNN_U) - b.dlt;
    if (!(t > 0.f)) return 0.f;
    return t * t * b.inv_sig2 * (1.f - 8.f * KNN_U);
}
__device__ __forceinline__ bool pca_slot_proven(float dk, float bnd, const PcaLb& b, float ku) { return dk < pca_lb_of(b, bnd) * (1.f - ku) - 1e-37f; }

bool knn_matrix_gate(const ismhip_ctx* ctx, const ismhip_codebook* cb, int nq) {
    return ctx->knn_mode == 0 && ctx->knn_t == 0 && nq >= 256 && cb->n_words >= 1024 && cb->dim % 4 == 0;
}

}

int knn_sqrt_queries(ismhip_ctx* ctx, const ismhip_codebook* cb, int nq, const float* q, float* sq, bool& negative);
int knn_f16_emit_image(ismhip_ctx* ctx, const ismhip_codebook* cb, const ismhip_codebook* xb, const float* qv, int n, int ldv, int n_pad,
                       uint32_t* sc, u16* qimg);

struct KnnCandArgs {
    const u16 *wh, *wl; const float* word_norm; int n_tiles_m, ld, k_steps;
    const u16 *qh, *ql; int nq; const float* out_scale; int tiles_per_split, n_splits;
    float* cand_val; int* cand_idx; int cand_stride; float* cand_bound; int bound_stride;
};
const void* knn_ring16_kernel(int T, int WR, int QP, int PRE = 0);
int knn_ring16_launch(ismhip_ctx* ctx, int T, const void* kern, unsigned grid, int threads, size_t lds, KnnCandArgs a,
                      unsigned int* stream_clock, float* thr0, int pre_step, float pre_relax);
const void* knn_mfma16_kernel(int T, int mode, bool big_tile);
int knn_mfma16_launch(ismhip_ctx* ctx, const void* kern, unsigned grid, int threads, size_t lds, KnnCandArgs a,
                      const float* emit_tau, uint32_t* emit_cnt, uint32_t* emit_list, int emit_cap);
int knn_mfma16_emit(ismhip_ctx* ctx, const ismhip_codebook* cb, const ismhip_codebook* xb, int n, int n_pad, const uint32_t* sc, const u16* qimg,
                    const float* tau, uint32_t* emit_cnt, uint32_t* rows, int cap);

int knn_l2_f32_launch(ismhip_ctx* ctx, int T, unsigned grid, const ismhip_codebook* cb, const float* q, int nq, int ldq, int tiles_per_split, int n_splits,
                      float* cand_val, int* cand_idx, int n_cand, float* cand_bound, int n_bound);
int knn_chi2_launch(ismhip_ctx* ctx, int T, int n_qt, const ismhip_codebook* cb, const float* q, int nq, int ldq, uint32_t* q_negative, int tiles_per_split, int n_splits,
                    float* cand_val, int* cand_idx, int n_cand, float* cand_bound, int n_bound);
```

point-cloud-donkey_amd/csrc/knn_mfma16.hip:

```cpp
#include "knn_internal.h"

namespace {


template <int T, int WR, int WC, int MI, int NI, int NTERM, int KB, int EMIT = 0>
__global__ __launch_bounds__(WR * WC * 64, 2) void k_knn_l2_mfma16(const u16* __restrict__ wh, const u16* __restrict__ wl,
                                                          const float* __restrict__ word_norm, int n_tiles_m, int ld, int k_steps,
                                                          const u16* __restrict__ qh, const u16* __restrict__ ql, int nq,
                                                          const float* __restrict__ out_scale,
                                                          int tiles_per_split, int n_splits,
                                                          float* __restrict__ cand_val, int* __restrict__ cand_idx, int cand_stride,
                                                          float* __restrict__ cand_bound, int bound_stride,
                                                          const float* __restrict__ emit_tau, uint32_t* __restrict__ emit_cnt, uint32_t* __restrict__ emit_list, int emit_cap) {
    constexpr int BM = WR * MI * 32, BN = WC * NI * 32, NT = WR * WC * 64;
    constexpr int SEGS = KB / 8;
    constexpr int KS = KB / 16;
    constexpr int RPP = NT / SEGS;
    constexpr int PA = BM / RPP, PB = BN / RPP;
    constexpr int SW_SH = KB == 64 ? 1 : 2, SW_MASK = SEGS - 1;
    extern __shared__ __attribute__((aligned(16))) unsigned char knn_smem[];
    constexpr bool X3 = NTERM == 3;
    u16* sAh = (u16*)knn_smem;
    u16* sAl = sAh + (X3 ? 2 * BM * KB : 0);
    u16* sBh = sAl + 2 * BM * KB;
    u16* sBl = sBh + (X3 ? 2 * BN * KB : 0);
    float* sCn = (float*)(sBl + 2 * BN * KB);
    const float oscale = NTERM == 1 ? out_scale[0] : -2.0f;

    const int tid = threadIdx.x;
    const int lane = tid & 63, wv = tid >> 6;
    const int wr = wv / WC, wc = wv % WC;
    const int r = lane & 31, h = lane >> 5;
    const int xcd = blockIdx.x & 7, jx = blockIdx.x >> 3;
    const int split = jx % n_splits, qtile = (jx / n_splits) * 8 + xcd;
    if (qtile * BN >= nq) return;
    const int mt0 = split * tiles_per_split;
    const int mt1 = min(n_tiles_m, mt0 + tiles_per_split);
    const int nk = (k_steps + KS - 1) / KS;

    const int srow = tid / SEGS, sseg = tid % SEGS;
    const int sdst0 = srow * KB + ((sseg ^ ((srow >> SW_SH) & SW_MASK)) << 3);
    const size_t qoff = (size_t)(qtile * BN + srow) * ld + sseg * 8;
    const int fragA = (wr * (MI * 32) + r) * KB, fragB = (wc * (NI * 32) + r) * KB;
    const int fsw = (r >> SW_SH) & SW_MASK;

    TopT<T + 1> top[NI];
    float tau[NI];
#pragma unroll
    for (int n = 0; n < NI; ++n) {
        top[n].init();
        tau[n] = -__builtin_inff();
        if (EMIT) { const int qi_ = qtile * BN + wc * (NI * 32) + n * 32 + r; if (qi_ < nq) tau[n] = emit_tau[qi_]; }
    }

    for (int mt = mt0; mt < mt1; ++mt) {
        const size_t aoff = (size_t)(mt * BM + srow) * ld + sseg * 8;
        f32x16 acc[MI][NI];
#pragma unroll
        for (int mi = 0; mi < MI; ++mi)
#pragma unroll
            for (int ni = 0; ni < NI; ++ni)
#pragma unroll
                for (int e = 0; e < 16; ++e) acc[mi][ni][e] = 0.f;

        f32x4 gah[PA], gal[X3 ? PA : 1], gbh[PB], gbl[X3 ? PB : 1];
#pragma unroll
        for (int p = 0; p < PA; ++p) { gah[p] = *(const f32x4*)(wh + aoff + (size_t)p * RPP * ld); if constexpr (X3) gal[p] = *(const f32x4*)(wl + aoff + (size_t)p * RPP * ld); }
#pragma unroll
        for (int p = 0; p < PB; ++p) { gbh[p] = *(const f32x4*)(qh + qoff + (size_t)p * RPP * ld); if constexpr (X3) gbl[p] = *(const f32x4*)(ql + qoff + (size_t)p * RPP * ld); }
        __syncthreads();
        for (int i = tid; i < BM; i += NT) sCn[i] = word_norm[mt * BM + i];
#pragma unroll
        for (int p = 0; p < PA; ++p) { *(f32x4*)(&sAh[sdst0 + p * RPP * KB]) = gah[p]; if constexpr (X3) *(f32x4*)(&sAl[sdst0 + p * RPP * KB]) = gal[p]; }
#pragma unroll
        for (int p = 0; p < PB; ++p) { *(f32x4*)(&sBh[sdst0 + p * RPP * KB]) = gbh[p]; if constexpr (X3) *(f32x4*)(&sBl[sdst0 + p * RPP * KB]) = gbl[p]; }
        __syncthreads();

        for (int kc = 0; kc < nk; ++kc) {
            const int cur = kc & 1;
            if (kc + 1 < nk) {
                const int ko = (kc + 1) * KB;
#pragma unroll
                for (int p = 0; p < PA; ++p) { gah[p] = *(const f32x4*)(wh + aoff + (size_t)p * RPP * ld + ko); if constexpr (X3) gal[p] = *(const f32x4*)(wl + aoff + (size_t)p * RPP * ld + ko); }
#pragma unroll
                for (int p = 0; p < PB; ++p) { gbh[p] = *(const f32x4*)(qh + qoff + (size_t)p * RPP * ld + ko); if constexpr (X3) gbl[p] = *(const f32x4*)(ql + qoff + (size_t)p * RPP * ld + ko); }
            }
            const u16* cAh = sAh + cur * BM * KB + fragA; const u16* cAl = sAl + cur * BM * KB + fragA;
            const u16* cBh = sBh + cur * BN * KB + fragB; const u16* cBl = sBl + cur * BN * KB + fragB;
            const int ks_n = min(KS, k_steps - kc * KS);
#pragma unroll
            for (int ks = 0; ks < KS; ++ks) {
                if (ks < ks_n) {
                    const int so = ((ks * 2 + h) ^ fsw) << 3;
                    if constexpr (X3) {
                        bf16x8 bh[NI], bl[NI];
#pragma unroll
                        for (int n = 0; n < NI; ++n) { bh[n] = *(const bf16x8*)(cBh + n * 32 * KB + so); bl[n] = *(const bf16x8*)(cBl + n * 32 * KB + so); }
#pragma unroll
                        for (int mi = 0; mi < MI; ++mi) {
                            const bf16x8 ah = *(const bf16x8*)(cAh + mi * 32 * KB + so);
                            const bf16x8 al = *(const bf16x8*)(cAl + mi * 32 * KB + so);
#pragma unroll
                            for (int ni = 0; ni < NI; ++ni) {
                                acc[mi][ni] = __builtin_amdgcn_mfma_f32_32x32x16_bf16(al, bh[ni], acc[mi][ni], 0, 0, 0);
                                acc[mi][ni] = __builtin_amdgcn_mfma_f32_32x32x16_bf16(ah, bl[ni], acc[mi][ni], 0, 0, 0);
                                acc[mi][ni] = __builtin_amdgcn_mfma_f32_32x32x16_bf16(ah, bh[ni], acc[mi][ni], 0, 0, 0);
                            }
                        }
                    } else {
                        f16x8 bh[NI];
#pragma unroll
                        for (int n = 0; n < NI; ++n) bh[n] = *(const f16x8*)(cBh + n * 32 * KB + so);
#pragma unroll
                        for (int mi = 0; mi < MI; ++mi) {
                            const f16x8 ah = *(const f16x8*)(cAh + mi * 32 * KB + so);
#pragma unroll
                            for (int ni = 0; ni < NI; ++ni) acc[mi][ni] = __builtin_amdgcn_mfma_f32_32x32x16_f16(ah, bh[ni], acc[mi][ni], 0, 0, 0);
                        }
                    }
                }
            }
            if (kc + 1 < nk) {
                const int nx = cur ^ 1;
#pragma unroll
                for (int p = 0; p < PA; ++p) { *(f32x4*)(&sAh[nx * BM * KB + sdst0 + p * RPP * KB]) = gah[p]; if constexpr (X3) *(f32x4*)(&sAl[nx * BM * KB + sdst0 + p * RPP * KB]) = gal[p]; }
#pragma unroll
                for (int p = 0; p < PB; ++p) { *(f32x4*)(&sBh[nx * BN * KB + sdst0 + p * RPP * KB]) = gbh[p]; if constexpr (X3) *(f32x4*)(&sBl[nx * BN * KB + sdst0 + p * RPP * KB]) = gbl[p]; }
            }
            __syncthreads();
        }
#pragma unroll
        for (int mi = 0; mi < MI; ++mi) {
            float cn[16];
#pragma unroll
            for (int e = 0; e < 16; ++e) cn[e] = sCn[wr * (MI * 32) + mi * 32 + (e & 3) + 8 * (e >> 2) + 4 * h];
#pragma unroll
            for (int ni = 0; ni < NI; ++ni) {
                if (EMIT) {
                    bool any = false;
#pragma unroll
                    for (int e = 0; e < 16; ++e) { acc[mi][ni][e] = cn[e] + oscale * acc[mi][ni][e]; any |= acc[mi][ni][e] <= tau[ni]; }
                    if (__any(any)) {
                        const int qi_ = qtile * BN + wc * (NI * 32) + ni * 32 + r;
#pragma unroll
                        for (int e = 0; e < 16; ++e)
                            if (acc[mi][ni][e] <= tau[ni]) {
                                const int row_ = mt * BM + wr * (MI * 32) + mi * 32 + (e & 3) + 8 * (e >> 2) + 4 * h;
                                if (row_ < cand_stride) {
                                    const uint32_t slot = atomicAdd(&emit_cnt[qi_], 1u);
                                    if (slot < (uint32_t)emit_cap) emit_list[(size_t)qi_ * emit_cap + slot] = (uint32_t)row_;
                                }
                            }
                    }
                    continue;
                }
                const float tau_ = top[ni].v[T];
                bool any = false;
#pragma unroll
                for (int e = 0; e < 16; ++e) { acc[mi][ni][e] = cn[e] + oscale * acc[mi][ni][e]; any |= acc[mi][ni][e] < tau_; }
                if (__any(any)) {
#pragma unroll
                    for (int e = 0; e < 16; ++e)
                        top[ni].push(acc[mi][ni][e], mt * BM + wr * (MI * 32) + mi * 32 + (e & 3) + 8 * (e >> 2) + 4 * h);
                }
            }
        }
    }
    if (EMIT) return;
#pragma unroll
    for (int ni = 0; ni < NI; ++ni) {
        const int qi = qtile * BN + wc * (NI * 32) + ni * 32 + r;
        if (qi < nq) {
#pragma unroll
            for (int t = 0; t < T; ++t) {
                const size_t o = (size_t)qi * cand_stride + split * (2 * WR * T) + (wr * 2 + h) * T + t;
                cand_val[o] = top[ni].v[t]; cand_idx[o] = top[ni].i[t];
            }
            cand_bound[(size_t)qi * bound_stride + split * (2 * WR) + (wr * 2 + h)] = top[ni].v[T];
        }
    }
}

template <int T>
const void* mfma16_instance(int mode, bool big_tile) {
    if (mode == 1) return big_tile ? (const void*)k_knn_l2_mfma16<T, 2, 4, 4, 2, 3, 32> : (const void*)k_knn_l2_mfma16<T, 2, 2, 2, 2, 3, 32>;
    return big_tile ? nullptr : (const void*)k_knn_l2_mfma16<T, 2, 2, 2, 2, 1, 64>;
}

}

const void* knn_mfma16_kernel(int T, int mode, bool big_tile) {
    switch (T) {
    case 1: return mfma16_instance<1>(mode, big_tile);
    case 2: return mfma16_instance<2>(mode, big_tile);
    case 3: return mfma16_instance<3>(mode, big_tile);
    case 4: return mfma16_instance<4>(mode, big_tile);
    }
    return nullptr;
}

int knn_mfma16_launch(ismhip_ctx* ctx, const void* kern, unsigned grid, int threads, size_t lds, KnnCandArgs a,
                      const float* emit_tau, uint32_t* emit_cnt, uint32_t* emit_list, int emit_cap) {
    void* args[] = {&a.wh, &a.wl, &a.word_norm, &a.n_tiles_m, &a.ld, &a.k_steps, &a.qh, &a.ql, &a.nq, &a.out_scale, &a.tiles_per_split, &a.n_splits,
                    &a.cand_val, &a.cand_idx, &a.cand_stride, &a.cand_bound, &a.bound_stride, &emit_tau, &emit_cnt, &emit_list, &emit_cap};
    ISM_HIP(ctx, hipLaunchKernel(kern, dim3(grid), dim3(threads), args, lds, ctx->stream));
    ISM_CHECK_LAUNCH(ctx, (emit_tau ? "k_knn_l2_mfma16<emit>" : "k_knn_l2_mfma16"));
    return ISMHIP_OK;
}

int knn_mfma16_emit(ismhip_ctx* ctx, const ismhip_codebook* cb, const ismhip_codebook* xb, int n, int n_pad, const uint32_t* sc, const u16* qimg,
                    const float* tau, uint32_t* emit_cnt, uint32_t* rows, int cap) {
    const void* kern = (const void*)k_knn_l2_mfma16<4, 2, 2, 2, 2, 1, 64, 1>;
    const size_t lds = knn_mfma16_lds(128, 128, 64, 1);
    const int rc = ism_lds_cap(ctx, kern, lds);
    if (rc != ISMHIP_OK) return rc;
    const int n_qt = n_pad / 128, n_mt = cb->n_words_pad / 128;
    int nsp = std::max(1, std::min(n_mt / 2, (2048 + 8 * ((n_qt + 7) / 8) - 1) / (8 * ((n_qt + 7) / 8))));
    int tps = (n_mt + nsp - 1) / nsp; nsp = (n_mt + tps - 1) / tps;
    KnnCandArgs a{};
    a.wh = xb->words_f16; a.word_norm = xb->word_norm; a.n_tiles_m = n_mt; a.ld = cb->ld16; a.k_steps = (cb->dim + 15) / 16;
    a.qh = qimg; a.nq = n; a.out_scale = (const float*)(sc + 1); a.tiles_per_split = tps; a.n_splits = nsp; a.cand_stride = cb->n_words;
    return knn_mfma16_launch(ctx, kern, 8 * ((n_qt + 7) / 8) * nsp, 256, lds, a, tau, emit_cnt, rows, cap);
}
```

point-cloud-donkey_amd/csrc/knn_ring16.hip:

```cpp
#include "knn_internal.h"

namespace {

__device__ __forceinline__ void lds_dma16(const void* g, void* l) {
    __builtin_amdgcn_global_load_lds((const void __attribute__((address_space(1)))*)g, (void __attribute__((address_space(3)))*)l, 16, 0, 0);
}
__device__ __forceinline__ float max_of_row_groups(float x) {
    const auto h = __builtin_amdgcn_permlane32_swap(__float_as_uint(x), __float_as_uint(x), false, false);
    float sh;
    asm("v_max_f32 %0, %1, %2" : "=v"(sh) : "v"(__uint_as_float(h[0])), "v"(__uint_as_float(h[1])));
    const auto q = __builtin_amdgcn_permlane16_swap(__float_as_uint(sh), __float_as_uint(sh), false, false);
    asm("v_max_f32 %0, %1, %2" : "=v"(sh) : "v"(__uint_as_float(q[0])), "v"(__uint_as_float(q[1])));
    return sh;
}
__device__ __forceinline__ float sel_f(unsigned long long m, float t, float f) { float r; asm("v_cndmask_b32_e64 %0, %1, %2, %3" : "=v"(r) : "v"(f), "v"(t), "s"(m)); return r; }
__device__ __forceinline__ int sel_i(unsigned long long m, int t, int f) { int r; asm("v_cndmask_b32_e64 %0, %1, %2, %3" : "=v"(r) : "v"(f), "v"(t), "s"(m)); return r; }
template <int N>
__device__ __forceinline__ void push_cnd(TopT<N>& tp, float x, int idx) {
    unsigned long long c[N];
#pragma unroll
    for (int t = 0; t < N; ++t) asm("v_cmp_lt_f32_e64 %0, %1, %2" : "=s"(c[t]) : "v"(x), "v"(tp.v[t]));
#pragma unroll
    for (int t = N - 1; t > 0; --t) {
        tp.v[t] = sel_f(c[t - 1], tp.v[t - 1], sel_f(c[t], x, tp.v[t]));
        tp.i[t] = sel_i(c[t - 1], tp.i[t - 1], sel_i(c[t], idx, tp.i[t]));
    }
    tp.v[0] = sel_f(c[0], x, tp.v[0]);
    tp.i[0] = sel_i(c[0], idx, tp.i[0]);
}
template <int T, int WR = 2, int QP = 0, int PRE = 0>
__global__ __launch_bounds__(WR * 256, 2) void k_knn_l2_ring16(const u16* __restrict__ wh, const float* __restrict__ word_norm, int n_tiles_m, int ld, int k_steps,
                                                          const u16* __restrict__ qh, int nq, const float* __restrict__ out_scale,
                                                          int tiles_per_split, int n_splits,
                                                          float* __restrict__ cand_val, int* __restrict__ cand_idx, int cand_stride,
                                                          float* __restrict__ cand_bound, int bound_stride, unsigned int* __restrict__ stream_clock,
                                                          const float* __restrict__ thr_init, float* __restrict__ thr_out, int tile_step, float thr_relax) {
    using L = Ring16Lds<WR, QP>;
    constexpr int WC = 4, MT = 8, NT = 4, KB = RG_KB, BM = WR * 128, BN = RG_BN;
    constexpr int STAGES = L::STAGES, STAGE_HALVES = L::STAGE_HALVES, CNS = 256;
    constexpr bool LEAN_WALK = T <= 3;
    extern __shared__ __attribute__((aligned(16))) unsigned char knn_smem[];
    u16* ring = (u16*)knn_smem;
    float* sCn = (float*)(knn_smem + L::cn);
    float* sThr = (float*)(knn_smem + L::thr);
    u16* panel = (u16*)(knn_smem + L::panel);
    const float oscale = out_scale[0];

    const int tid = threadIdx.x;
    const int lane = tid & 63;
    const int wv = __builtin_amdgcn_readfirstlane(tid >> 6);
    const int wr = wv / WC, wc = wv % WC;
    const int fr = lane & 15, fq = lane >> 4;
    const int xcd = blockIdx.x & 7, jx = blockIdx.x >> 3;
    const int split = jx % n_splits, qtile = (jx / n_splits) * 8 + xcd;
    if (qtile * BN >= nq) return;
    const int mt0 = split * tiles_per_split;
    const int n_t = PRE ? (n_tiles_m + tile_step - 1) / tile_step : min(n_tiles_m, mt0 + tiles_per_split) - mt0;
    if (n_t <= 0) return;
    const int nk = (k_steps + 1) / 2;
    const int G = n_t * nk;
    int toff = 0; unsigned c0 = 0u;
    if (stream_clock) {
        unsigned int* clk = stream_clock + xcd * n_splits + split;
        if (tid == 0) *(volatile unsigned*)ring = __hip_atomic_load(clk, __ATOMIC_RELAXED, __HIP_MEMORY_SCOPE_AGENT);
        __syncthreads();
        c0 = __builtin_amdgcn_readfirstlane(*(volatile unsigned*)ring);
        __syncthreads();
        toff = (int)(c0 % (unsigned)n_t);
        stream_clock = clk;
    }
    auto tile_of = [&](int i) { if (PRE) return i * tile_step; const int x = i + toff; return mt0 + (x >= n_t ? x - n_t : x); };

    constexpr int NA = QP ? 2 : (WR == 2 ? 4 : 2), NB = 4;
    const bool dma_a = QP || WR == 1 || wv < 4, dma_b = !QP && (WR == 1 || wv >= 4);
    const unsigned lane_off = (unsigned)(lane * 16);
    const int row_a = QP ? wv * 32 : (WR == 2 ? (wv & 3) * 64 : wv * 32), row_b = (wv & 3) * 64;
    const char* qbase = QP ? (const char*)(qh + (size_t)qtile * nk * (256 * KB)) + (wv * 32) * (KB * 2)
                           : (const char*)(qh + (size_t)qtile * nk * (BN * KB)) + row_b * (KB * 2);
    if (QP) {
        for (int s_ = 0; s_ < nk; ++s_) {
            lds_dma16(qbase + (size_t)s_ * (256 * KB * 2) + lane_off, panel + (s_ * 256 + wv * 32) * KB);
            lds_dma16(qbase + (size_t)s_ * (256 * KB * 2) + 16 * KB * 2 + lane_off, panel + (s_ * 256 + wv * 32 + 16) * KB);
        }
    }
    int pt = 0, pkc = 0, ps = 0;
    auto issue = [&]() {
        u16* st = ring + ps * STAGE_HALVES;
        const int tt = tile_of(pt);
        if (wv == 0 && pkc == 0) lds_dma16(word_norm + (size_t)tt * BM + lane * 4, sCn + (pt & 3) * CNS);
        if (dma_a) {
            const char* sp = (const char*)wh + ((size_t)(WR == 2 ? tt : (tt >> 1)) * nk + pkc) * (256 * KB * 2) + ((WR == 2 ? 0 : (tt & 1) * 128) + row_a) * (KB * 2);
#pragma unroll
            for (int j = 0; j < NA; ++j) lds_dma16(sp + j * (16 * KB * 2) + lane_off, st + (row_a + j * 16) * KB);
        }
        if (dma_b) {
            const char* sp = qbase + (size_t)pkc * (BN * KB * 2);
#pragma unroll
            for (int j = 0; j < NB; ++j) lds_dma16(sp + j * (16 * KB * 2) + lane_off, st + BM * KB + (row_b + j * 16) * KB);
        }
        if (++ps == STAGES) ps = 0;
        if (pt * nk + pkc + 1 < G) { if (++pkc == nk) { pkc = 0; ++pt; } }
    };
#pragma unroll
    for (int i = 0; i < STAGES; ++i) issue();

    const int fso = (fr * KB) + ((fq ^ f16t_swizzle(fr)) << 3);
    const int fragA = wr * (MT * 16) * KB + fso, fragB = (QP ? 0 : BM * KB) + wc * (NT * 16) * KB + fso;
    TopT<T + 1> top[NT];
    float thr[NT];
#pragma unroll
    for (int n = 0; n < NT; ++n) {
        top[n].init(); thr[n] = -__builtin_inff();
        if (!PRE && thr_init) { const int qi_ = qtile * BN + wc * (NT * 16) + n * 16 + fr; if (qi_ < nq) thr[n] = thr_init[qi_]; }
    }
    f32x4 acc[MT][NT];
    const int pw = (1 - wr) * WC + wc;
    if (WR == 2) {
#pragma unroll
        for (int n = 0; n < NT; ++n) sThr[(wv * NT + n) * 64 + lane] = -__builtin_inff();
    }

    f16x8 xa[4], ya[4], bq[NT];
    if (QP) asm volatile("s_waitcnt vmcnt(6)\n\ts_barrier" ::: "memory");
    else asm volatile("s_waitcnt vmcnt(12)\n\ts_barrier" ::: "memory");
#pragma unroll
    for (int m = 0; m < 4; ++m) xa[m] = *(const f16x8*)(ring + fragA + m * 16 * KB);
    int t = 0, kc = 0, gs = 0;
    for (int g = 0; g < G; ++g) {
        const int gn = gs + 1 == STAGES ? 0 : gs + 1;
        const u16* st = ring + gs * STAGE_HALVES;
        const u16* sn = ring + gn * STAGE_HALVES;
        gs = gn;
#pragma unroll
        for (int n = 0; n < NT; ++n) bq[n] = *(const f16x8*)((QP ? panel + kc * (256 * KB) : st) + fragB + n * 16 * KB);
        __builtin_amdgcn_sched_barrier(0);
        __builtin_amdgcn_s_setprio(1);
        const float* cnp = sCn + (t & 3) * CNS + wr * (MT * 16) + 4 * fq;
        auto mma4 = [&](int mb, const f16x8* af, f16x8* nxt, const u16* nsrc) {
            if (kc == 0) {
#pragma unroll
                for (int mt = 0; mt < 4; ++mt) {
                    const f32x4 c0 = *(const f32x4*)(cnp + (mb + mt) * 16);
#pragma unroll
                    for (int nt = 0; nt < NT; ++nt) acc[mb + mt][nt] = __builtin_amdgcn_mfma_f32_16x16x32_f16(af[mt], bq[nt], c0, 0, 0, 0);
                    nxt[mt] = *(const f16x8*)(nsrc + mt * 16 * KB);
                    __builtin_amdgcn_sched_barrier(0);
                }
            } else {
#pragma unroll
                for (int mt = 0; mt < 4; ++mt) {
#pragma unroll
                    for (int nt = 0; nt < NT; ++nt) acc[mb + mt][nt] = __builtin_amdgcn_mfma_f32_16x16x32_f16(af[mt], bq[nt], acc[mb + mt][nt], 0, 0, 0);
                    nxt[mt] = *(const f16x8*)(nsrc + mt * 16 * KB);
                    __builtin_amdgcn_sched_barrier(0);
                }
            }
        };
        mma4(0, xa, ya, st + fragA + 4 * 16 * KB);
        __builtin_amdgcn_sched_barrier(0);
        if (QP) asm volatile("s_waitcnt vmcnt(4) lgkmcnt(0)\n\ts_barrier" ::: "memory");
        else if (WR == 2) asm volatile("s_waitcnt vmcnt(8) lgkmcnt(0)\n\ts_barrier" ::: "memory");
        else asm volatile("s_waitcnt vmcnt(6) lgkmcnt(0)\n\ts_barrier" ::: "memory");
        issue();
        __builtin_amdgcn_sched_barrier(0);
        mma4(4, ya, xa, sn + fragA);
        __builtin_amdgcn_s_setprio(0);
        __builtin_amdgcn_sched_barrier(0);
        if (++kc == nk) {
            const int row0 = tile_of(t) * BM + wr * (MT * 16) + 4 * fq;
            if (stream_clock && tid == 0) atomicMax(stream_clock, c0 + (unsigned)t + 1u);
            if (PRE) {
#pragma unroll
                for (int nt = 0; nt < NT; ++nt) {
                    float m = thr[nt];
#pragma unroll
                    for (int mt = 0; mt < MT; ++mt) {
                        asm("v_max3_f32 %0, %1, %2, %3" : "=v"(m) : "v"(m), "v"(acc[mt][nt][0]), "v"(acc[mt][nt][1]));
                        asm("v_max3_f32 %0, %1, %2, %3" : "=v"(m) : "v"(m), "v"(acc[mt][nt][2]), "v"(acc[mt][nt][3]));
                    }
                    thr[nt] = m;
                }
            } else {
                float other[NT];
                if (WR == 2) {
#pragma unroll
                    for (int nt = 0; nt < NT; ++nt) other[nt] = sThr[(pw * NT + nt) * 64 + lane];
                    __builtin_amdgcn_sched_barrier(0);
                }
                float gm[LEAN_WALK ? NT : 1][MT], mx[NT];
#pragma unroll
                for (int nt = 0; nt < NT; ++nt) {
                    float m;
                    if (LEAN_WALK) {
#pragma unroll
                        for (int mt = 0; mt < MT; ++mt) {
                            asm("v_max3_f32 %0, %1, %2, %3" : "=v"(gm[nt][mt]) : "v"(acc[mt][nt][0]), "v"(acc[mt][nt][1]), "v"(acc[mt][nt][2]));
                            asm("v_max_f32 %0, %1, %2" : "=v"(gm[nt][mt]) : "v"(gm[nt][mt]), "v"(acc[mt][nt][3]));
                        }
                        asm("v_max3_f32 %0, %1, %2, %3" : "=v"(m) : "v"(gm[nt][0]), "v"(gm[nt][1]), "v"(gm[nt][2]));
                        asm("v_max3_f32 %0, %1, %2, %3" : "=v"(m) : "v"(m), "v"(gm[nt][3]), "v"(gm[nt][4]));
                        asm("v_max3_f32 %0, %1, %2, %3" : "=v"(m) : "v"(m), "v"(gm[nt][5]), "v"(gm[nt][6]));
                        asm("v_max_f32 %0, %1, %2" : "=v"(m) : "v"(m), "v"(gm[nt][7]));
                    } else {
                        asm("v_max3_f32 %0, %1, %2, %3" : "=v"(m) : "v"(acc[0][nt][0]), "v"(acc[0][nt][1]), "v"(acc[0][nt][2]));
                        asm("v_max_f32 %0, %1, %2" : "=v"(m) : "v"(m), "v"(acc[0][nt][3]));
#pragma unroll
                        for (int mt = 1; mt < MT; ++mt) {
                            asm("v_max3_f32 %0, %1, %2, %3" : "=v"(m) : "v"(m), "v"(acc[mt][nt][0]), "v"(acc[mt][nt][1]));
                            asm("v_max3_f32 %0, %1, %2, %3" : "=v"(m) : "v"(m), "v"(acc[mt][nt][2]), "v"(acc[mt][nt][3]));
                        }
                    }
                    mx[nt] = m;
                }
                if (WR == 2) {
#pragma unroll
                    for (int nt = 0; nt < NT; ++nt) asm("v_max_f32 %0, %1, %2" : "=v"(thr[nt]) : "v"(thr[nt]), "v"(other[nt]));
                }
                unsigned long long hit[NT];
#pragma unroll
                for (int nt = 0; nt < NT; ++nt) hit[nt] = __ballot(mx[nt] > thr[nt]);
                unsigned long long any_hit = 0ull;
#pragma unroll
                for (int nt = 0; nt < NT; ++nt) any_hit |= hit[nt];
                if (any_hit != 0ull) {
#pragma unroll
                    for (int nt = 0; nt < NT; ++nt) {
                        if (hit[nt] == 0ull) continue;
                        float gl[MT];
#pragma unroll
                        for (int mt = 0; mt < MT; ++mt) {
                            if (LEAN_WALK) gl[mt] = gm[nt][mt];
                            else {
                                asm("v_max3_f32 %0, %1, %2, %3" : "=v"(gl[mt]) : "v"(acc[mt][nt][0]), "v"(acc[mt][nt][1]), "v"(acc[mt][nt][2]));
                                asm("v_max_f32 %0, %1, %2" : "=v"(gl[mt]) : "v"(gl[mt]), "v"(acc[mt][nt][3]));
                            }
                        }
                        unsigned long long gk[MT];
#pragma unroll
                        for (int mt = 0; mt < MT; ++mt) gk[mt] = __ballot(gl[mt] > thr[nt]);
                        asm volatile("" :: "s"(gk[0]), "s"(gk[1]), "s"(gk[2]), "s"(gk[3]), "s"(gk[4]), "s"(gk[5]), "s"(gk[6]), "s"(gk[7]));
#pragma unroll
                        for (int mt = 0; mt < MT; ++mt) {
                            if (gk[mt] == 0ull) continue;
                            unsigned long long mk[4];
#pragma unroll
                            for (int j = 0; j < 4; ++j) mk[j] = __ballot(acc[mt][nt][j] > thr[nt]);
                            asm volatile("" :: "s"(mk[0]), "s"(mk[1]), "s"(mk[2]), "s"(mk[3]));
#pragma unroll
                            for (int j = 0; j < 4; ++j) {
                                if (mk[j] == 0ull) continue;
                                const float a = acc[mt][nt][j];
                                const float x = a > thr[nt] ? -a : __builtin_inff();
                                if (LEAN_WALK) push_cnd(top[nt], x, row0 + mt * 16 + j); else top[nt].push_flat(x, row0 + mt * 16 + j);
                                asm("v_max_f32_e64 %0, %1, -%2" : "=v"(thr[nt]) : "v"(thr[nt]), "v"(top[nt].v[T]));
                            }
                        }
                        thr[nt] = max_of_row_groups(thr[nt]);
                        if (WR == 2) sThr[(wv * NT + nt) * 64 + lane] = thr[nt];
                    }
                }
            }
            kc = 0; ++t;
        }
    }
    asm volatile("s_waitcnt vmcnt(0)" ::: "memory");
    if (PRE) {
#pragma unroll
        for (int nt = 0; nt < NT; ++nt) thr[nt] = max_of_row_groups(thr[nt]);
        __syncthreads();
#pragma unroll
        for (int nt = 0; nt < NT; ++nt) sThr[(wv * NT + nt) * 64 + lane] = thr[nt];
        __syncthreads();
        if (wr == 0 && fq == 0) {
#pragma unroll
            for (int nt = 0; nt < NT; ++nt) {
                const int qi = qtile * BN + wc * (NT * 16) + nt * 16 + fr;
                const float b = fmaxf(thr[nt], sThr[(pw * NT + nt) * 64 + lane]);
                if (qi < nq) thr_out[qi] = b - fabsf(b) * 3.814697265625e-06f + thr_relax;
            }
        }
        return;
    }
    if (WR == 2) {
        __syncthreads();
#pragma unroll
        for (int nt = 0; nt < NT; ++nt) sThr[(wv * NT + nt) * 64 + lane] = thr[nt];
        __syncthreads();
#pragma unroll
        for (int nt = 0; nt < NT; ++nt) thr[nt] = fmaxf(thr[nt], sThr[(pw * NT + nt) * 64 + lane]);
    }
#pragma unroll
    for (int nt = 0; nt < NT; ++nt) {
        const int qi = qtile * BN + wc * (NT * 16) + nt * 16 + fr;
        if (qi < nq) {
#pragma unroll
            for (int tt = 0; tt < T; ++tt) {
                const size_t o = (size_t)qi * cand_stride + split * (WR * 4 * T) + (wr * 4 + fq) * T + tt;
                cand_val[o] = -oscale * top[nt].v[tt]; cand_idx[o] = top[nt].i[tt];
            }
            cand_bound[(size_t)qi * bound_stride + split * (WR * 4) + (wr * 4 + fq)] = oscale * thr[nt];
        }
    }
}

template <int T>
const void* ring16_instance(int WR, int QP, int PRE) {
    if (PRE) return (const void*)k_knn_l2_ring16<T, 2, 0, 1>;
    if (WR == 1) return (const void*)k_knn_l2_ring16<T, 1>;
    return QP ? (const void*)k_knn_l2_ring16<T, 2, 2> : (const void*)k_knn_l2_ring16<T, 2>;
}

}

const void* knn_ring16_kernel(int T, int WR, int QP, int PRE) {
    switch (T) {
    case 1: return ring16_instance<1>(WR, QP, PRE);
    case 2: return ring16_instance<2>(WR, QP, PRE);
    case 3: return ring16_instance<3>(WR, QP, PRE);
    case 4: return ring16_instance<4>(WR, QP, PRE);
    }
    return nullptr;
}

int knn_ring16_launch(ismhip_ctx* ctx, int T, const void* kern, unsigned grid, int threads, size_t lds, KnnCandArgs a,
                      unsigned int* stream_clock, float* thr0, int pre_step, float pre_relax) {
    const float* thr_init = nullptr; float* thr_out = nullptr; int tile_step = 1;
    if (thr0 && pre_step > 0) {
        const void* pk = knn_ring16_kernel(T, 2, 0, 1);
        const size_t plds = Ring16Lds<2, 0>::total(0);
        const int rc2 = ism_lds_cap(ctx, pk, plds);
        if (rc2 != ISMHIP_OK) return rc2;
        int one = 1, all = a.n_tiles_m; unsigned int* noclk = nullptr; const float* noinit = nullptr;
        void* pargs[] = {&a.wh, &a.word_norm, &a.n_tiles_m, &a.ld, &a.k_steps, &a.qh, &a.nq, &a.out_scale, &all, &one, &a.cand_val, &a.cand_idx, &a.cand_stride, &a.cand_bound, &a.bound_stride, &noclk, &noinit, &thr0, &pre_step, &pre_relax};
        ISM_HIP(ctx, hipLaunchKernel(pk, dim3(grid / a.n_splits), dim3(512), pargs, plds, ctx->stream));
        ISM_CHECK_LAUNCH(ctx, "k_knn_l2_ring16<pre>");
    }
    thr_init = thr0;
    float no_relax = 0.f;
    void* rargs[] = {&a.wh, &a.word_norm, &a.n_tiles_m, &a.ld, &a.k_steps, &a.qh, &a.nq, &a.out_scale, &a.tiles_per_split, &a.n_splits, &a.cand_val, &a.cand_idx, &a.cand_stride, &a.cand_bound, &a.bound_stride, &stream_clock, &thr_init, &thr_out, &tile_step, &no_relax};
    ISM_HIP(ctx, hipLaunchKernel(kern, dim3(grid), dim3(threads), rargs, lds, ctx->stream));
    ISM_CHECK_LAUNCH(ctx, "k_knn_l2_ring16");
    return ISMHIP_OK;
}
```

Before: 18990 objects/s.

## Add per-query-tile codebook row ranges and shared queue for stage-2 kNN

Measured after the change: 19570 objects/s, median of 6. +3.0%, better.

```diff
diff --git a/point-cloud-donkey_amd/csrc/common.h b/point-cloud-donkey_amd/csrc/common.h
--- a/point-cloud-donkey_amd/csrc/common.h
+++ b/point-cloud-donkey_amd/csrc/common.h
@@ -122,7 +122,10 @@
     uint32_t knn_stats[2] = {0, 0};
     std::set<const void*> attr_done;
     uint32_t knn_stage2_queries = 0;
+    uint32_t knn_stage2_list_entries = 0;
+    uint32_t knn_stage2_ranged = 0;
     uint32_t knn_seed_launches = 0;
+    bool knn_stage2_splits = true;
     bool knn_stage2_seed = true;
     bool knn_two_stage = true;
     bool knn_join = true;
@@ -160,7 +163,7 @@
 enum ScratchSlot {
     SCR_KP_OFF = 1, SCR_TIE_LIST, SCR_TIE_REC, SCR_TIE_KEYS, SCR_COUNTERS, SCR_KNN_CAND_IDX, SCR_KNN_CAND_VAL,
     SCR_QNORM, SCR_FPFH_FLAG, SCR_FPFH_LIST, SCR_FPFH_SPFH, SCR_FPFH_LOOKUP, SCR_SLOT_OFF, SCR_CLASS_BW,
-    SCR_COMPACT_KEEP, SCR_COMPACT_POS, SCR_OBJ_COUNT, SCR_QPAD, SCR_LRF_COV, SCR_KNN_FLAGS, SCR_KNN_QSPLIT, SCR_MAX_REC, SCR_QNORM2, SCR_KNN_Q2, SCR_KNN_LIST2, SCR_TRAIN, SCR_TRAIN2, SCR_MAX_WORK, SCR_KMEANS, SCR_KNN_CLOCK, SCR_PCA, SCR_KNN_THR0, SCR_KNN_QSQRT, SCR_KNN_HELL_EMIT, SCR_KNN_THR, SCR_KNN_THR2, SCR_TRAIN_ACT, SCR_KNN_LK, SCR_KNN_LK2, SCR_KNN_LK3, SCR_PREFILTER, SCR_RANSAC, SCR_COSPAIR, SCR_KNNB_FLAG, SCR_KNNB_Q, SCR_KNNB_CAND, SCR_RANK, SCR_RANK_KNN
+    SCR_COMPACT_KEEP, SCR_COMPACT_POS, SCR_OBJ_COUNT, SCR_QPAD, SCR_LRF_COV, SCR_KNN_FLAGS, SCR_KNN_QSPLIT, SCR_MAX_REC, SCR_QNORM2, SCR_KNN_Q2, SCR_KNN_LIST2, SCR_TRAIN, SCR_TRAIN2, SCR_MAX_WORK, SCR_KMEANS, SCR_KNN_CLOCK, SCR_PCA, SCR_KNN_THR0, SCR_KNN_QSQRT, SCR_KNN_HELL_EMIT, SCR_KNN_THR, SCR_KNN_THR2, SCR_TRAIN_ACT, SCR_KNN_LK, SCR_KNN_LK2, SCR_KNN_LK3, SCR_PREFILTER, SCR_RANSAC, SCR_COSPAIR, SCR_KNNB_FLAG, SCR_KNNB_Q, SCR_KNNB_CAND, SCR_RANK, SCR_RANK_KNN, SCR_KNN_LISTS, SCR_KNN_QUEUE
 };
 
 int  ism_set_err(ismhip_ctx* ctx, int code, const std::string& msg);
diff --git a/point-cloud-donkey_amd/csrc/ctx.hip b/point-cloud-donkey_amd/csrc/ctx.hip
--- a/point-cloud-donkey_amd/csrc/ctx.hip
+++ b/point-cloud-donkey_amd/csrc/ctx.hip
@@ -83,6 +83,7 @@
     { const char* e = getenv("ISMHIP_KNN_HELLINGER"); ctx->knn_hellinger = !(e && e[0] == '0'); }
     { const char* e = getenv("ISMHIP_KNN_T1"); if (e) ctx->knn_t1 = atoi(e); }
     { const char* e = getenv("ISMHIP_KNN_STAGE2_T4"); if (e) ctx->knn_stage2_t4 = atoi(e) != 0; }
+    { const char* e = getenv("ISMHIP_KNN_STAGE2_SPLITS"); ctx->knn_stage2_splits = !(e && e[0] == '0'); }
     { const char* e = getenv("ISMHIP_KNN_STAGE2_SEED"); ctx->knn_stage2_seed = !(e && e[0] == '0'); }
     { const char* e = getenv("ISMHIP_KNN_PRE_STEP"); if (e && atoi(e) > 0) ctx->knn_pre_step = atoi(e); }
     { const char* e = getenv("ISMHIP_KNN_PRE_GAMMA"); if (e) ctx->knn_pre_gamma = (float)atof(e); }
@@ -207,6 +208,8 @@
                 if (ms_out) *ms_out = (double)v[i]; if (launches_out) *launches_out = 1; return ISMHIP_OK;
             }
     }
+    if (std::strcmp(name, "knn_stage2_list_entries") == 0) { if (ms_out) *ms_out = (double)ctx->knn_stage2_list_entries; if (launches_out) *launches_out = 1; return ISMHIP_OK; }
+    if (std::strcmp(name, "knn_stage2_ranged") == 0) { if (ms_out) *ms_out = (double)ctx->knn_stage2_ranged; if (launches_out) *launches_out = 1; return ISMHIP_OK; }
     if (std::strcmp(name, "knn_stage2_queries") == 0) { if (ms_out) *ms_out = (double)ctx->knn_stage2_queries; if (launches_out) *launches_out = 1; return ISMHIP_OK; }
     if (std::strcmp(name, "knn_flagged_queries") == 0 || std::strcmp(name, "knn_flagged_items") == 0) {
         if (ms_out) *ms_out = (double)ctx->knn_stats[name[12] == 'q' ? 0 : 1];
diff --git a/point-cloud-donkey_amd/csrc/knn.hip b/point-cloud-donkey_amd/csrc/knn.hip
--- a/point-cloud-donkey_amd/csrc/knn.hip
+++ b/point-cloud-donkey_amd/csrc/knn.hip
@@ -159,7 +159,13 @@
     }
     return have_k;
 }
-__device__ __forceinline__ void knn_queue_unproven(bool viol, int qi, int lane, uint32_t* __restrict__ flag_count, uint32_t* __restrict__ qrec, uint32_t* __restrict__ items) {
+struct KnnQueueTag { const uint32_t* live; int q_base, slot_tag; const float* known_dk; };
+__device__ __forceinline__ bool knn_is_padding(const KnnQueueTag& tg, int qi) { return tg.live && tg.live[qi] == ~0u; }
+__device__ __forceinline__ bool knn_proof_dk(const KnnQueueTag& tg, int qi, bool have_k, float& dk) {
+    if (tg.known_dk) { const float U = tg.known_dk[qi]; if (U == U) { dk = have_k ? fminf(dk, U) : U; return true; } }
+    return have_k;
+}
+__device__ __forceinline__ void knn_queue_unproven(bool viol, int qi, int lane, uint32_t* __restrict__ flag_count, uint32_t* __restrict__ qrec, uint32_t* __restrict__ items, const KnnQueueTag& tg) {
     const unsigned long long vmask = __ballot(viol);
     if (vmask != 0ull) {
         const int nv = __popcll(vmask);
@@ -167,12 +173,12 @@
         if (lane == 0) {
             const uint32_t qs = atomicAdd(&flag_count[KNN_CNT_QUERIES], 1u);
             ibase = atomicAdd(&flag_count[KNN_CNT_ITEMS], (uint32_t)nv);
-            qrec[3 * (size_t)qs] = (uint32_t)qi; qrec[3 * (size_t)qs + 1] = ibase; qrec[3 * (size_t)qs + 2] = (uint32_t)nv;
+            qrec[3 * (size_t)qs] = (uint32_t)(qi + tg.q_base); qrec[3 * (size_t)qs + 1] = ibase; qrec[3 * (size_t)qs + 2] = (uint32_t)nv;
         }
         ibase = __shfl(ibase, 0, 64);
         if (viol) {
             const uint32_t it = ibase + __popcll(vmask & ((1ull << lane) - 1ull));
-            items[2 * (size_t)it] = (uint32_t)qi; items[2 * (size_t)it + 1] = (uint32_t)lane;
+            items[2 * (size_t)it] = (uint32_t)(qi + tg.q_base); items[2 * (size_t)it + 1] = (uint32_t)(lane | tg.slot_tag);
         }
     }
 }
@@ -182,9 +188,9 @@
                                                     const int* __restrict__ cand_idx, const float* __restrict__ cand_val, int cand_stride, int n_cand,
                                                     const float* __restrict__ cand_bound, int n_bound, VerifyParams vp,
                                                     int k, int32_t* __restrict__ idx_out, float* __restrict__ dist_out,
-                                                    uint32_t* __restrict__ flag_count, uint32_t* __restrict__ qrec, uint32_t* __restrict__ items) {
+                                                    uint32_t* __restrict__ flag_count, uint32_t* __restrict__ qrec, uint32_t* __restrict__ items, KnnQueueTag tg) {
     const int qi = blockIdx.x * 4 + (threadIdx.x >> 6);
-    if (qi >= nq) return;
+    if (qi >= nq || knn_is_padding(tg, qi)) return;
     const int lane = lane_id();
     const float* qp = q + (size_t)qi * ldq;
     const float qn2 = wave_norm2(qp, dim, lane);
@@ -218,7 +224,7 @@
     float bnd = __builtin_inff();
     if (lane < n_bound) bnd = cand_bound[(size_t)qi * n_bound + lane];
     float dk;
-    const bool have_k = knn_select_write<1>(&key, qi, k, lane, idx_out, dist_out, dk);
+    const bool have_k = knn_proof_dk(tg, qi, knn_select_write<1>(&key, qi, k, lane, idx_out, dist_out, dk), dk);
     bool viol = false;
     const float eps_chk = metric == ISMHIP_METRIC_CHI2 ? qn2 + vp.cmax2 : knn_eps_s_raw(vp, qn2) + qn2;
     if (lane < n_bound && (bnd != __builtin_inff() || !(eps_chk < __builtin_inff()))) {
@@ -228,7 +234,7 @@
             viol = !(dk < lo);
         } else viol = !knn_l2_slot_proven(dk, bnd, qn2, vp);
     }
-    knn_queue_unproven(viol, qi, lane, flag_count, qrec, items);
+    knn_queue_unproven(viol, qi, lane, flag_count, qrec, items, tg);
 }
 
 struct PcaVerify {
@@ -256,9 +262,9 @@
                                                         const int* __restrict__ cand_idx, const float* __restrict__ cand_val, int cand_stride, int n_cand,
                                                         const float* __restrict__ cand_bound, int n_bound, PcaVerify pv,
                                                         int k, int32_t* __restrict__ idx_out, float* __restrict__ dist_out,
-                                                        uint32_t* __restrict__ flag_count, uint32_t* __restrict__ qrec, uint32_t* __restrict__ items) {
+                                                        uint32_t* __restrict__ flag_count, uint32_t* __restrict__ qrec, uint32_t* __restrict__ items, KnnQueueTag tg) {
     const int qi = blockIdx.x * 4 + (threadIdx.x >> 6);
-    if (qi >= nq) return;
+    if (qi >= nq || knn_is_padding(tg, qi)) return;
     const int lane = lane_id();
     const float* qp = q + (size_t)qi * ldq;
     const PcaLb lbq = pca_lb_query(pv, qi, wave_norm2(qp, dim, lane), lane);
@@ -291,19 +297,21 @@
     float bnd = __builtin_inff();
     if (lane < n_bound) bnd = cand_bound[(size_t)qi * n_bound + lane];
     float dk;
-    const bool have_k = knn_select_write<1>(&key, qi, k, lane, idx_out, dist_out, dk);
+    const bool have_k = knn_proof_dk(tg, qi, knn_select_write<1>(&key, qi, k, lane, idx_out, dist_out, dk), dk);
     bool viol = false;
     if (lane < n_bound && (bnd != __builtin_inff() || !(lbq.eps_s + lbq.qn2h + lbq.dlt < __builtin_inff()))) {
         if (!have_k) viol = true;
         else viol = !pca_slot_proven(dk, bnd, lbq, pv.ku);
     }
-    knn_queue_unproven(viol, qi, lane, flag_count, qrec, items);
+    knn_queue_unproven(viol, qi, lane, flag_count, qrec, items, tg);
 }
 
 __global__ __launch_bounds__(256) void k_knn_seed_thr(const float* __restrict__ q, int nq, int ldq, int dim, const float* __restrict__ seed_dk,
-                                                      bool pca, PcaVerify pv, VerifyParams vp, const float* __restrict__ out_scale, float* __restrict__ thr) {
+                                                      bool pca, PcaVerify pv, VerifyParams vp, const float* __restrict__ out_scale, float* __restrict__ thr,
+                                                      const uint32_t* __restrict__ live ) {
     const int qi = blockIdx.x * 4 + (threadIdx.x >> 6);
     if (qi >= nq) return;
+    if (live && live[qi] == ~0u) { if (lane_id() == 0) thr[qi] = __builtin_inff(); return; }
     const int lane = lane_id();
     const float qn2 = wave_norm2(q + (size_t)qi * ldq, dim, lane);
     PcaLb lbq{};
@@ -354,9 +362,9 @@
                                                          const int* __restrict__ cand_idx, const float* __restrict__ cand_val, int cand_stride, int n_cand,
                                                          const float* __restrict__ cand_bound, int n_bound, VerifyParams vp,
                                                          int k, int32_t* __restrict__ idx_out, float* __restrict__ dist_out,
-                                                         uint32_t* __restrict__ flag_count, uint32_t* __restrict__ qrec, uint32_t* __restrict__ items) {
+                                                         uint32_t* __restrict__ flag_count, uint32_t* __restrict__ qrec, uint32_t* __restrict__ items, KnnQueueTag tg) {
     const int qi = blockIdx.x * 4 + (threadIdx.x >> 6);
-    if (qi >= nq) return;
+    if (qi >= nq || knn_is_padding(tg, qi)) return;
     const int lane = lane_id();
     const float* qp = q + (size_t)qi * ldq;
     const float qn2 = wave_norm2(sq + (size_t)qi * dim_pad, dim, lane);
@@ -448,7 +456,7 @@
         if (!have_k) viol = true;
         else viol = !(dk < lb_of(bnd) * (1.f - vp.ku) - 1e-37f);
     }
-    knn_queue_unproven(viol, qi, lane, flag_count, qrec, items);
+    knn_queue_unproven(viol, qi, lane, flag_count, qrec, items, tg);
 }
 
 #define KNN_FB_UNITS 8192u
@@ -457,10 +465,11 @@
     const uint32_t p = KNN_FB_UNITS / n_items;
     return p > 256u ? 256u : p;
 }
+struct KnnFbDesc { int tiles_per_split, n_tiles, tile_rows, wr_rows, n_splits; };
 template <int KM>
 __global__ __launch_bounds__(256) void k_knn_fallback(const float* __restrict__ words, int dim, int dim_pad, int n_words,
-                                                      const float* __restrict__ q, int ldq, int metric, int k, int tiles_per_split, int n_tiles,
-                                                      int tile_rows, int wr_rows ,
+                                                      const float* __restrict__ q, int ldq, int metric, int k, KnnFbDesc d0, KnnFbDesc d1,
+                                                      const int* __restrict__ qrange,
                                                       const uint32_t* __restrict__ flag_count, const uint32_t* __restrict__ items,
                                                       const int32_t* __restrict__ idx_in, const float* __restrict__ dist_in,
                                                       unsigned long long* __restrict__ item_out, size_t part_base) {
@@ -469,21 +478,27 @@
     const int g = lane >> 4, l16 = lane & 15;
     const uint32_t n_items = flag_count[KNN_CNT_ITEMS];
     const bool l2 = metric != ISMHIP_METRIC_CHI2;
-    const bool lay_all = l2 && wr_rows == KNN_FB_ALL;
-    const bool lay16 = l2 && wr_rows == KNN_FB_RING;
-    const bool lay16h = l2 && wr_rows == KNN_FB_RING_HALF;
-    const int rows_per_tile = lay_all ? tile_rows : ((lay16 || lay16h) ? 32 : (l2 ? wr_rows / 2 : tile_rows));
     const int nj = dim_pad / 16;
     const uint32_t gw = blockIdx.x * 4 + (threadIdx.x >> 6), nw = gridDim.x * 4;
     const uint32_t P = knn_fb_parts(n_items);
     unsigned long long* outp = P > 1 ? item_out + KM * part_base : item_out;
     for (uint32_t u = gw; u < n_items * P; u += nw) {
         const uint32_t it = u / P, part_i = u % P;
-        const int qi = (int)items[2 * (size_t)it], b = (int)items[2 * (size_t)it + 1];
+        const int qi = (int)items[2 * (size_t)it], bt = (int)items[2 * (size_t)it + 1], b = bt & 255;
+        const KnnFbDesc d = (bt >> 8) ? d1 : d0;
+        const int wr_rows = d.wr_rows, tile_rows = d.tile_rows;
+        const bool lay_all = l2 && wr_rows == KNN_FB_ALL;
+        const bool lay16 = l2 && wr_rows == KNN_FB_RING;
+        const bool lay16h = l2 && wr_rows == KNN_FB_RING_HALF;
+        const int rows_per_tile = lay_all ? tile_rows : ((lay16 || lay16h) ? 32 : (l2 ? wr_rows / 2 : tile_rows));
         const float* qp = q + (size_t)qi * ldq;
         const int split = lay_all ? 0 : (lay16 ? (b >> 3) : (l2 ? (b >> 2) : b));
         const int wr = lay16h ? 0 : (lay16 ? (b >> 2) & 1 : (b >> 1) & 1), h = b & 1, fq = b & 3;
-        const int mt0 = split * tiles_per_split, mt1 = min(n_tiles, mt0 + tiles_per_split);
+        int mt0 = split * d.tiles_per_split, mt1 = min(d.n_tiles, mt0 + d.tiles_per_split);
+        if (qrange) {
+            const int* rg = qrange + 4 * (qi >> 8);
+            knn_range_split(rg[0] / tile_rows, rg[1] / tile_rows, split, lay_all ? 1 : d.n_splits, mt0, mt1);
+        }
         const int total = (mt1 - mt0) * rows_per_tile;
         unsigned long long best[KM];
 #pragma unroll
@@ -608,7 +623,8 @@
     idx_out[i] = id; dist_out[i] = dd;
 }
 
-struct KnnStage1 { uint32_t* flag_count; uint32_t* qrec; };
+struct KnnStage1 { uint32_t* flag_count; uint32_t* qrec; uint32_t* items; int n_splits, slots, rows_per_split; };
+struct KnnQueue { uint32_t *count, *qrec, *items; unsigned long long* item_out; size_t q_items; KnnFbDesc desc[2]; };
 struct KnnRequest {
     KnnStage1* stage1 = nullptr;
     const char* tname = nullptr;
@@ -617,6 +633,10 @@
     const float* hell_q = nullptr;
     bool half = false;
     const float* seed_dk = nullptr;
+    const int* qrange = nullptr; const uint32_t* live = nullptr; KnnQueue* queue = nullptr;
+    int q_base = 0, chunk = 0, range_rows_min = 0, range_rows_max = 0;
+    const float* known_dk = nullptr;
+    int q_ld = 0;
 };
 
 enum KnnCand { KNN_CAND_F32, KNN_CAND_CHI2, KNN_CAND_MFMA16, KNN_CAND_RING16 };
@@ -626,7 +646,7 @@
     KnnCand cand;
     const void* kern;
     int BM, BN, threads;
-    bool big_tile, half, qpanel2, pca, merged, prepass, seeded, join;
+    bool big_tile, half, qpanel2, pca, merged, prepass, seeded, join, ranged;
     int slots, ring_nk;
     int n_qt, n_splits, tiles_per_split, cand_per_split, n_cand, n_bound;
     int fb_tiles_per_split; KnnFbLayout fb_layout;
@@ -645,7 +665,7 @@
     p.big_tile = use_lp && nq >= 4096 && cb->n_words_pad >= 4096;
     const bool ring = p.big_tile && p.mode == 0 && xb->words_f16t && (cb->dim + 15) / 16 > 2;
     p.half = ring && (rq.half || ctx->knn_half);
-    p.qpanel2 = ring && !p.half && ctx->knn_qpanel2 && rq.use_pca && PI.m > 0 && PI.m <= 160;
+    p.qpanel2 = ring && !p.half && ctx->knn_qpanel2 && rq.use_pca && PI.m > 0 && PI.m <= 160 && !rq.range_rows_max;
     p.pca = rq.use_pca && ring && PI.m > 0;
     p.ring_nk = p.pca ? PI.m / 32 : ((cb->dim + 15) / 16 + 1) / 2;
     p.merged = rq.many_splits && l2 && use_lp && !p.big_tile;
@@ -654,7 +674,8 @@
     p.BN = !l2 ? CHI_B : (p.big_tile ? 256 : KNN_BN);
     p.slots = ring && !p.half ? 8 : 4;
     p.n_qt = (nq + p.BN - 1) / p.BN;
-    const int n_mt = cb->n_words_pad / p.BM;
+    p.ranged = rq.range_rows_max > 0 && l2 && use_lp;
+    const int n_mt = (p.ranged ? rq.range_rows_max : cb->n_words_pad) / p.BM;
     if (l2) {
         const int max_s = (p.hell ? 64 * KNN_HELL_CPL : 64) / (p.slots * T);
         p.n_splits = std::max(1, std::min(std::min(max_s, n_mt), std::max(p.pca ? 2 : 3, (1024 + p.n_qt - 1) / p.n_qt)));
@@ -669,8 +690,9 @@
         if (k > T) p.n_splits = std::max(p.n_splits, std::min(std::min(max_s, n_mt), (2 * k + T - 1) / T));
         p.cand_per_split = T;
     }
+    if (p.ranged) p.n_splits = std::max(1, std::min(p.n_splits, rq.range_rows_min / p.BM));
     p.tiles_per_split = (n_mt + p.n_splits - 1) / p.n_splits;
-    p.n_splits = (n_mt + p.tiles_per_split - 1) / p.tiles_per_split;
+    if (!p.ranged) p.n_splits = (n_mt + p.tiles_per_split - 1) / p.tiles_per_split;
     p.n_cand = p.n_splits * p.cand_per_split;
     p.n_bound = l2 ? p.n_splits * p.slots : p.n_splits;
     p.prepass = rq.stage1 && ring && !p.half && ctx->knn_prepass && n_mt >= 128 && !(p.pca && PI.resid2 <= 0.f);
@@ -683,9 +705,9 @@
     else if (ring) {
         p.cand = KNN_CAND_RING16;
         p.threads = p.half ? 256 : 512;
-        if (p.half) { p.kern = knn_ring16_kernel(T, 1, 0); p.lds = p.lds_cap = Ring16Lds<1, 0>::total(0); }
+        if (p.half) { p.kern = knn_ring16_kernel(T, 1, 0, 0, p.ranged); p.lds = p.lds_cap = Ring16Lds<1, 0>::total(0); }
         else if (p.qpanel2) { p.kern = knn_ring16_kernel(T, 2, 2); p.lds = Ring16Lds<2, 2>::total(p.ring_nk); p.lds_cap = Ring16Lds<2, 2>::total(160 / 32); }
-        else { p.kern = knn_ring16_kernel(T, 2, 0); p.lds = p.lds_cap = Ring16Lds<2, 0>::total(0); }
+        else { p.kern = knn_ring16_kernel(T, 2, 0, 0, p.ranged); p.lds = p.lds_cap = Ring16Lds<2, 0>::total(0); }
     } else {
         p.cand = KNN_CAND_MFMA16;
         p.threads = p.big_tile ? 512 : 256;
@@ -698,6 +720,7 @@
 struct KnnScratch {
     float *cand_val, *cand_bound; int* cand_idx; int n_cand, n_bound;
     uint32_t *flag_count, *qrec, *items; unsigned long long* item_out; size_t q_items;
+    uint32_t* qcount;
     uint32_t* qsc;
 };
 struct KnnRun : KnnScratch {
@@ -718,6 +741,8 @@
     r.qrec = r.flag_count + KNN_CNT_WORDS; r.items = r.qrec + 3 * nq; r.qsc = r.flag_count + KNN_CNT_QSC;
     r.item_out = (unsigned long long*)(((uintptr_t)(r.items + 2 * r.q_items) + 7) & ~(uintptr_t)7);
     ISM_HIP(r.ctx, hipMemsetAsync(r.flag_count, 0, KNN_CNT_WORDS * sizeof(uint32_t), r.ctx->stream));
+    r.qcount = r.flag_count;
+    if (const KnnQueue* Q = r.rq->queue) { r.qcount = Q->count; r.qrec = Q->qrec; r.items = Q->items; r.item_out = Q->item_out; r.q_items = Q->q_items; }
     return ISMHIP_OK;
 }
 
@@ -774,6 +799,7 @@
         a.qh = r.q_hi; a.ql = r.q_lo; a.nq = nq; a.out_scale = (const float*)(r.qsc + 1);
         a.tiles_per_split = p.tiles_per_split; a.n_splits = p.n_splits;
         a.cand_val = r.cand_val; a.cand_idx = r.cand_idx; a.cand_stride = r.n_cand; a.cand_bound = r.cand_bound; a.bound_stride = r.n_bound;
+        a.qrange = p.ranged ? r.rq->qrange : nullptr;
         int rc = ISMHIP_OK;
         if (p.cand == KNN_CAND_RING16) {
             rc = ism_lds_cap(ctx, p.kern, p.lds_cap);
@@ -803,7 +829,7 @@
             if (p.seeded) {
                 const VerifyParams vp = knn_verify_params(xb, cb->dim_pad, p.mode, r.qsc, true);
                 hipLaunchKernelGGL(k_knn_seed_thr, dim3((nq + 3) / 4), dim3(256), 0, ctx->stream, r.qq, nq, r.ldq, cb->dim, r.rq->seed_dk,
-                                   p.pca, p.pca ? knn_pca_verify(r, vp) : PcaVerify{}, vp, a.out_scale, thr0);
+                                   p.pca, p.pca ? knn_pca_verify(r, vp) : PcaVerify{}, vp, a.out_scale, thr0, r.rq->live);
                 ISM_CHECK_LAUNCH(ctx, "k_knn_seed_thr");
                 ++ctx->knn_seed_launches;
             }
@@ -836,33 +862,38 @@
     ismhip_ctx* ctx = r.ctx; const ismhip_codebook* cb = r.cb; const KnnPlan& p = r.p;
     const VerifyParams vp = knn_verify_params(r.xb, cb->dim_pad, p.mode, r.qsc, true);
     const dim3 grid((r.nq + 3) / 4), block(256);
+    const KnnQueueTag tg{r.rq->live, r.rq->q_base, r.rq->chunk << 8, r.rq->known_dk};
     TimerScope trr(ctx, "knn_rerank");
     if (p.pca) {
         const PcaVerify pv = knn_pca_verify(r, vp);
         hipLaunchKernelGGL(k_knn_rerank_pca, grid, block, 0, ctx->stream, cb->words, cb->dim, cb->dim_pad, cb->n_words,
-                           r.qq, r.nq, r.ldq, r.cand_idx, r.cand_val, r.n_cand, r.n_cand, r.cand_bound, r.n_bound, pv, r.k, idx_out, dist_out, r.flag_count, r.qrec, r.items);
+                           r.qq, r.nq, r.ldq, r.cand_idx, r.cand_val, r.n_cand, r.n_cand, r.cand_bound, r.n_bound, pv, r.k, idx_out, dist_out, r.qcount, r.qrec, r.items, tg);
     } else if (p.hell) {
         hipLaunchKernelGGL(k_knn_rerank_hell, grid, block, 0, ctx->stream, cb->words, cb->dim, cb->dim_pad, cb->n_words,
-                           r.qq, r.nq, r.ldq, r.rq->hell_q, r.xb->shadow_perm, r.cand_idx, r.cand_val, r.n_cand, r.n_cand, r.cand_bound, r.n_bound, vp, r.k, idx_out, dist_out, r.flag_count, r.qrec, r.items);
+                           r.qq, r.nq, r.ldq, r.rq->hell_q, r.xb->shadow_perm, r.cand_idx, r.cand_val, r.n_cand, r.n_cand, r.cand_bound, r.n_bound, vp, r.k, idx_out, dist_out, r.qcount, r.qrec, r.items, tg);
     } else
     hipLaunchKernelGGL(k_knn_rerank, grid, block, 0, ctx->stream, cb->words, cb->dim, cb->dim_pad, cb->n_words,
-                       r.qq, r.nq, r.ldq, r.metric, r.cand_idx, r.cand_val, r.n_cand, r.n_cand, r.cand_bound, r.n_bound, vp, r.k, idx_out, dist_out, r.flag_count, r.qrec, r.items);
+                       r.qq, r.nq, r.ldq, r.metric, r.cand_idx, r.cand_val, r.n_cand, r.n_cand, r.cand_bound, r.n_bound, vp, r.k, idx_out, dist_out, r.qcount, r.qrec, r.items, tg);
     ISM_CHECK_LAUNCH(ctx, "k_knn_rerank");
     return ISMHIP_OK;
 }
 
-int knn_exact_scan(KnnRun& r, int32_t* idx_out, float* dist_out) {
-    ismhip_ctx* ctx = r.ctx; const ismhip_codebook* cb = r.cb; const KnnPlan& p = r.p; const int k = r.k;
+int knn_scan_queue(ismhip_ctx* ctx, const ismhip_codebook* cb, int metric, int k, const float* q, int ldq, const KnnQueue& Q, const int* qrange,
+                   int32_t* idx_out, float* dist_out) {
     TimerScope ts(ctx, "knn_fallback");
-    const int n_tiles = cb->n_words_pad / p.BM;
     const auto scan = k <= 4 ? k_knn_fallback<4> : k_knn_fallback<KNN_MAX_K>;
     const auto merge = k <= 4 ? k_knn_fallback_merge<4> : k_knn_fallback_merge<KNN_MAX_K>;
-    hipLaunchKernelGGL(scan, dim3(1024), dim3(256), 0, ctx->stream, cb->words, cb->dim, cb->dim_pad, cb->n_words, r.qq, r.ldq, r.metric, k,
-                       p.fb_tiles_per_split, n_tiles, p.BM, (int)p.fb_layout, r.flag_count, r.items, idx_out, dist_out, r.item_out, r.q_items);
+    hipLaunchKernelGGL(scan, dim3(1024), dim3(256), 0, ctx->stream, cb->words, cb->dim, cb->dim_pad, cb->n_words, q, ldq, metric, k,
+                       Q.desc[0], Q.desc[1], qrange, Q.count, Q.items, idx_out, dist_out, Q.item_out, Q.q_items);
     ISM_CHECK_LAUNCH(ctx, "k_knn_fallback");
-    hipLaunchKernelGGL(merge, dim3(256), dim3(256), 0, ctx->stream, k, r.flag_count, r.qrec, r.item_out, r.q_items, idx_out, dist_out);
+    hipLaunchKernelGGL(merge, dim3(256), dim3(256), 0, ctx->stream, k, Q.count, Q.qrec, Q.item_out, Q.q_items, idx_out, dist_out);
     ISM_CHECK_LAUNCH(ctx, "k_knn_fallback_merge");
     return ISMHIP_OK;
+}
+KnnFbDesc knn_fb_desc(const KnnPlan& p, const ismhip_codebook* cb) { return KnnFbDesc{p.fb_tiles_per_split, cb->n_words_pad / p.BM, p.BM, (int)p.fb_layout, p.n_splits}; }
+int knn_exact_scan(KnnRun& r, int32_t* idx_out, float* dist_out) {
+    KnnQueue Q{r.qcount, r.qrec, r.items, r.item_out, r.q_items, {knn_fb_desc(r.p, r.cb), KnnFbDesc{}}};
+    return knn_scan_queue(r.ctx, r.cb, r.metric, r.k, r.qq, r.ldq, Q, nullptr, idx_out, dist_out);
 }
 
 int run_knn(ismhip_ctx* ctx, const ismhip_codebook* cb, int metric, int nq, const float* q, int k, int T,
@@ -872,10 +903,11 @@
     r.ctx = ctx; r.cb = cb; r.rq = &rq; r.metric = metric; r.nq = nq; r.k = k; r.T = T;
     r.p = knn_plan(ctx, cb, metric, nq, k, T, rq);
     if (r.p.cand == KNN_CAND_MFMA16 && !r.p.kern) return ism_set_err(ctx, ISMHIP_ERR_UNSUPPORTED, "knn: f16 256x256 tile without the ring not built");
+    if (r.p.cand == KNN_CAND_RING16 && !r.p.kern) return ism_set_err(ctx, ISMHIP_ERR_UNSUPPORTED, "knn: ranged ring instance not built for this T");
     r.xb = r.p.hell ? cb->chi_shadow : cb;
     r.PI = rq.use_pca == 2 ? &cb->pca2 : &cb->pca;
-    r.qq = q; r.ldq = cb->dim;
-    if (cb->dim_pad != cb->dim) {
+    r.qq = q; r.ldq = rq.q_ld ? rq.q_ld : cb->dim;
+    if (cb->dim_pad != r.ldq) {
         float* qpad = (float*)ism_scratch(ctx, SCR_QPAD, (size_t)nq * cb->dim_pad * sizeof(float));
         if (!qpad) return ISMHIP_ERR_NOMEM;
         const size_t tot = (size_t)nq * cb->dim_pad;
@@ -888,7 +920,8 @@
     if (rc == ISMHIP_OK) rc = knn_launch_candidates(r);
     if (rc == ISMHIP_OK) rc = knn_rerank_prove(r, idx_out, dist_out);
     if (rc != ISMHIP_OK) return rc;
-    if (rq.stage1) { *rq.stage1 = KnnStage1{r.flag_count, r.qrec}; return ISMHIP_OK; }
+    if (rq.stage1) { *rq.stage1 = KnnStage1{r.flag_count, r.qrec, r.items, r.p.n_splits, r.p.slots, r.p.tiles_per_split * r.p.BM}; return ISMHIP_OK; }
+    if (rq.queue) { rq.queue->desc[rq.chunk] = knn_fb_desc(r.p, cb); return ISMHIP_OK; }
     rc = knn_exact_scan(r, idx_out, dist_out);
     if (rc != ISMHIP_OK) return rc;
     if (ctx->timers_on) ISM_HIP(ctx, hipMemcpyAsync(ctx->knn_stats, r.flag_count, 8, hipMemcpyDeviceToHost, ctx->stream));
@@ -915,15 +948,36 @@
     idx_out[o] = idx2[t]; dist_out[o] = dist2[t];
 }
 
-struct KnnStage2 { int n2; float* q2; uint32_t* list2; int32_t* idx2; float* dist2; float* dk2; };
+struct KnnStage2 { int n2; float* q2; uint32_t* list2; int32_t* idx2; float* dist2; float* dk2;
+                   bool want_lists = false; uint32_t *head_d = nullptr, *lists_d = nullptr; uint32_t cnt[16] = {}; };
+int knn_gather_unsplit(ismhip_ctx* ctx, const ismhip_codebook* cb, const KnnStage1& s1, const float* q, int k, KnnStage2& g, const int32_t* idx1, const float* dist1);
+__global__ void k_knn_split_lists(const uint32_t* __restrict__ flag_count, const uint32_t* __restrict__ qrec, const uint32_t* __restrict__ items,
+                                  int slots, int nq, uint32_t* __restrict__ head, uint32_t* __restrict__ lists);
 int knn_gather_stage2(ismhip_ctx* ctx, const ismhip_codebook* cb, const KnnStage1& s1, const float* q, int k, KnnStage2& g,
-                      const int32_t* idx1, const float* dist1) {
-    uint32_t n2u = 0;
-    ISM_HIP(ctx, hipMemcpyAsync(&n2u, s1.flag_count, 4, hipMemcpyDeviceToHost, ctx->stream));
+                      const int32_t* idx1, const float* dist1, int nq = 0) {
+    uint32_t hb[17] = {0};
+    if (g.want_lists) {
+        g.head_d = (uint32_t*)ism_scratch(ctx, SCR_KNN_LISTS, (32 + (size_t)s1.n_splits * nq) * sizeof(uint32_t));
+        if (!g.head_d) return ISMHIP_ERR_NOMEM;
+        g.lists_d = g.head_d + 32;
+        ISM_HIP(ctx, hipMemsetAsync(g.head_d, 0, 32 * sizeof(uint32_t), ctx->stream));
+        hipLaunchKernelGGL(k_knn_split_lists, dim3(256), dim3(256), 0, ctx->stream, (const uint32_t*)s1.flag_count, (const uint32_t*)s1.qrec, (const uint32_t*)s1.items,
+                           s1.slots, nq, g.head_d, g.lists_d);
+        ISM_CHECK_LAUNCH(ctx, "k_knn_split_lists");
+        ISM_HIP(ctx, hipMemcpyAsync(hb, g.head_d, 17 * sizeof(uint32_t), hipMemcpyDeviceToHost, ctx->stream));
+    } else ISM_HIP(ctx, hipMemcpyAsync(hb, s1.flag_count, 4, hipMemcpyDeviceToHost, ctx->stream));
     ISM_HIP(ctx, hipStreamSynchronize(ctx->stream));
-    ctx->knn_stage2_queries = n2u;
-    const int n2 = g.n2 = (int)n2u;
-    if (n2 == 0) { ctx->knn_stats[0] = ctx->knn_stats[1] = 0; return ISMHIP_OK; }
+    ctx->knn_stage2_queries = hb[0];
+    for (int s = 0; s < 16; ++s) g.cnt[s] = hb[1 + s];
+    ctx->knn_stage2_list_entries = 0;
+    for (int s = 0; s < 16; ++s) ctx->knn_stage2_list_entries += g.cnt[s];
+    g.n2 = (int)hb[0];
+    if (g.n2 == 0) { ctx->knn_stats[0] = ctx->knn_stats[1] = 0; return ISMHIP_OK; }
+    if (g.want_lists) return ISMHIP_OK;
+    return knn_gather_unsplit(ctx, cb, s1, q, k, g, idx1, dist1);
+}
+int knn_gather_unsplit(ismhip_ctx* ctx, const ismhip_codebook* cb, const KnnStage1& s1, const float* q, int k, KnnStage2& g, const int32_t* idx1, const float* dist1) {
+    const int n2 = g.n2;
     g.q2 = (float*)ism_scratch(ctx, SCR_KNN_Q2, (size_t)n2 * cb->dim * sizeof(float));
     g.list2 = (uint32_t*)ism_scratch(ctx, SCR_KNN_LIST2, (size_t)n2 * (sizeof(uint32_t) + (size_t)k * (sizeof(int32_t) + sizeof(float)) + (idx1 ? sizeof(float) : 0)));
     if (!g.q2 || !g.list2) return ISMHIP_ERR_NOMEM;
@@ -940,6 +994,153 @@
     return ISMHIP_OK;
 }
 
+__global__ void k_knn_split_lists(const uint32_t* __restrict__ flag_count, const uint32_t* __restrict__ qrec, const uint32_t* __restrict__ items,
+                                  int slots, int nq, uint32_t* __restrict__ head, uint32_t* __restrict__ lists) {
+    const uint32_t n = flag_count[KNN_CNT_QUERIES];
+    if (blockIdx.x == 0 && threadIdx.x == 0) head[0] = n;
+    const int lane = lane_id();
+    for (uint32_t t0 = blockIdx.x * blockDim.x + (threadIdx.x & ~63u); t0 < n; t0 += gridDim.x * blockDim.x) {
+        const uint32_t t = t0 + lane;
+        uint32_t qi = 0u, mask = 0u;
+        if (t < n) {
+            qi = qrec[3 * (size_t)t];
+            const uint32_t ibase = qrec[3 * (size_t)t + 1], ni = qrec[3 * (size_t)t + 2];
+            for (uint32_t j = 0; j < ni; ++j) mask |= 1u << (items[2 * (size_t)(ibase + j) + 1] / (uint32_t)slots);
+        }
+        uint32_t any = mask;
+#pragma unroll
+        for (int o = 32; o > 0; o >>= 1) any |= __shfl_xor(any, o, 64);
+        while (any) {
+            const int s = __ffs((int)any) - 1; any &= any - 1u;
+            const unsigned long long in = __ballot((mask >> s) & 1u);
+            uint32_t base = 0u;
+            if (lane == 0) base = atomicAdd(&head[1 + s], (uint32_t)__popcll(in));
+            base = __shfl(base, 0, 64);
+            if ((mask >> s) & 1u) lists[(size_t)s * nq + base + __popcll(in & ((1ull << lane) - 1ull))] = qi;
+        }
+    }
+}
+__global__ void k_knn_range_layout(const uint32_t* __restrict__ head, int n_lists, int rows_per_split, int n_rows, int* __restrict__ qrange) {
+    int off = 0;
+    for (int s = 0; s < n_lists; ++s) {
+        const int groups = (int)((head[1 + s] + 255u) / 256u);
+        for (int g = threadIdx.x; g < groups; g += blockDim.x) {
+            int* e = qrange + 4 * (off / 256 + g);
+            e[0] = s * rows_per_split; e[1] = min(n_rows, (s + 1) * rows_per_split); e[2] = s; e[3] = off;
+        }
+        off += groups * 256;
+    }
+}
+__global__ __launch_bounds__(256) void k_knn_gather_lists(const uint32_t* __restrict__ head, const uint32_t* __restrict__ lists, int nq, const int* __restrict__ qrange,
+                                                          const float* __restrict__ q, int dim, int ld, float* __restrict__ q2, uint32_t* __restrict__ list2,
+                                                          const int32_t* __restrict__ idx1, const float* __restrict__ dist1, int k, float* __restrict__ dk2) {
+    const int i = blockIdx.x;
+    const int* rg = qrange + 4 * (i >> 8);
+    const int s = rg[2], pos = i - rg[3];
+    const bool live = (uint32_t)pos < head[1 + s];
+    const uint32_t qi = live ? lists[(size_t)s * nq + pos] : ~0u;
+    if (threadIdx.x == 0) {
+        list2[i] = qi;
+        if (dk2) dk2[i] = live && idx1[(size_t)qi * k + (k - 1)] >= 0 ? dist1[(size_t)qi * k + (k - 1)] : __builtin_nanf("");
+    }
+    for (int c = threadIdx.x; c < ld; c += blockDim.x) q2[(size_t)i * ld + c] = live && c < dim ? q[(size_t)qi * dim + c] : 0.f;
+}
+__global__ void k_knn_merge_lists(const uint32_t* __restrict__ list2, int i0, int n, int k, const int32_t* __restrict__ idx2, const float* __restrict__ dist2,
+                                  int32_t* __restrict__ idx_out, float* __restrict__ dist_out) {
+    const int t = blockIdx.x * blockDim.x + threadIdx.x;
+    if (t >= n) return;
+    const size_t a = (size_t)list2[i0 + t] * k, b = (size_t)(i0 + t) * k;
+    int32_t oi[KNN_MAX_K]; float od[KNN_MAX_K];
+    int ia = 0, ib = 0, no = 0;
+    while (no < k) {
+        const bool ha = ia < k && idx_out[a + ia] >= 0, hb = ib < k && idx2[b + ib] >= 0;
+        if (!ha && !hb) break;
+        const unsigned long long ka = ha ? ((unsigned long long)__float_as_uint(dist_out[a + ia]) << 32) | (unsigned)idx_out[a + ia] : ~0ull;
+        const unsigned long long kb = hb ? ((unsigned long long)__float_as_uint(dist2[b + ib]) << 32) | (unsigned)idx2[b + ib] : ~0ull;
+        const unsigned long long key = ka <= kb ? ka : kb;
+        if (ka <= kb) ++ia; else ++ib;
+        bool dup = false;
+        for (int j = 0; j < no; ++j) dup |= oi[j] == (int32_t)(key & 0xffffffffull);
+        if (!dup) { oi[no] = (int32_t)(key & 0xffffffffull); od[no] = __uint_as_float((unsigned)(key >> 32)); ++no; }
+    }
+    for (int j = 0; j < k; ++j) { idx_out[a + j] = j < no ? oi[j] : -1; dist_out[a + j] = j < no ? od[j] : __builtin_nanf(""); }
+}
+
+inline int knn_stage2_chunk(int n_total, int o) { const int left = n_total - o; return left >= 32768 ? left / 32768 * 32768 : left; }
+KnnRequest knn_stage2_request(const ismhip_ctx* ctx, const ismhip_codebook* cb, int n, const float* seed_dk) {
+    KnnRequest r2; r2.tname = "knn_stage2"; r2.many_splits = n < 4096;
+    r2.use_pca = cb->pca2.m > 0 && !(n < 4096) ? 2 : 0;
+    r2.half = n >= 4096 && n < 32768 && !ctx->knn_stage2_t4;
+    r2.seed_dk = seed_dk;
+    return r2;
+}
+
+int run_knn_stage2_lists(ismhip_ctx* ctx, const ismhip_codebook* cb, const KnnStage1& s1, const uint32_t* head_d, const uint32_t* lists_d, const uint32_t* cnt, int n2,
+                         int nq, const float* q, int k, int32_t* idx_out, float* dist_out, bool& taken) {
+    taken = false;
+    const int S = s1.n_splits, rps = s1.rows_per_split, n_rows = cb->n_words_pad;
+    if (S < 2 || rps % 256 != 0 || n_rows % 256 != 0) return ISMHIP_OK;
+    int off[17] = {0}, rows_min = n_rows, rows_max = 0;
+    double work = 0.0;
+    for (int s = 0; s < S; ++s) {
+        const int rows = std::min(n_rows, (s + 1) * rps) - s * rps;
+        off[s + 1] = off[s] + (int)((cnt[s] + 255u) / 256u) * 256;
+        if (cnt[s]) { rows_min = std::min(rows_min, rows); rows_max = std::max(rows_max, rows); work += (double)(off[s + 1] - off[s]) * rows; }
+    }
+    if (work * 8.0 > (double)n2 * n_rows * 7.0) return ISMHIP_OK;
+    taken = true;
+    ++ctx->knn_stage2_ranged;
+    const int N = off[S], ld = cb->dim_pad;
+    const bool seed = ctx->knn_stage2_seed;
+    size_t q_items = 0; int n_chunks = 0;
+    for (int o = 0; o < N; ++n_chunks) {
+        const int n = knn_stage2_chunk(N, o);
+        KnnRequest r2 = knn_stage2_request(ctx, cb, n, nullptr);
+        r2.range_rows_min = rows_min; r2.range_rows_max = rows_max;
+        q_items += (size_t)n * knn_plan(ctx, cb, ISMHIP_METRIC_L2SQ, n, k, 4, r2).n_bound;
+        o += n;
+    }
+    if (n_chunks > 2) return ism_set_err(ctx, ISMHIP_ERR_UNSUPPORTED, "knn: more than two stage-2 chunks");
+    const int KM = k > 4 ? KNN_MAX_K : 4;
+    float* q2 = (float*)ism_scratch(ctx, SCR_KNN_Q2, (size_t)N * ld * sizeof(float));
+    uint32_t* list2 = (uint32_t*)ism_scratch(ctx, SCR_KNN_LIST2, (size_t)N * (sizeof(uint32_t) + (size_t)k * (sizeof(int32_t) + sizeof(float)) + sizeof(float)) + (size_t)(N / 256) * 4 * sizeof(int));
+    uint32_t* qmem = (uint32_t*)ism_scratch(ctx, SCR_KNN_QUEUE, (KNN_CNT_WORDS + 3 * (size_t)N + 2 * q_items) * sizeof(uint32_t) + 8 + (q_items + KNN_FB_UNITS) * KM * sizeof(unsigned long long));
+    if (!q2 || !list2 || !qmem) return ISMHIP_ERR_NOMEM;
+    int32_t* idx2 = (int32_t*)(list2 + N);
+    float* dist2 = (float*)(idx2 + (size_t)N * k);
+    float* dk2 = dist2 + (size_t)N * k;
+    int* qrange = (int*)(dk2 + N);
+    KnnQueue Q{};
+    Q.count = qmem; Q.qrec = qmem + KNN_CNT_WORDS; Q.items = Q.qrec + 3 * (size_t)N; Q.q_items = q_items;
+    Q.item_out = (unsigned long long*)(((uintptr_t)(Q.items + 2 * q_items) + 7) & ~(uintptr_t)7);
+    ISM_HIP(ctx, hipMemsetAsync(Q.count, 0, KNN_CNT_WORDS * sizeof(uint32_t), ctx->stream));
+    hipLaunchKernelGGL(k_knn_range_layout, dim3(1), dim3(256), 0, ctx->stream, head_d, S, rps, n_rows, qrange);
+    ISM_CHECK_LAUNCH(ctx, "k_knn_range_layout");
+    hipLaunchKernelGGL(k_knn_gather_lists, dim3(N), dim3(256), 0, ctx->stream, head_d, lists_d, nq, (const int*)qrange, q, cb->dim, ld, q2, list2,
+                       (const int32_t*)idx_out, (const float*)dist_out, k, dk2);
+    ISM_CHECK_LAUNCH(ctx, "k_knn_gather_lists");
+    int chunk = 0;
+    for (int o = 0; o < N; ++chunk) {
+        const int n = knn_stage2_chunk(N, o);
+        KnnRequest r2 = knn_stage2_request(ctx, cb, n, seed ? dk2 + o : nullptr);
+        r2.qrange = qrange + 4 * (o / 256); r2.live = list2 + o; r2.queue = &Q; r2.q_base = o; r2.chunk = chunk;
+        r2.range_rows_min = rows_min; r2.range_rows_max = rows_max; r2.q_ld = ld; r2.known_dk = dk2 + o;
+        const int rc = run_knn(ctx, cb, ISMHIP_METRIC_L2SQ, n, q2 + (size_t)o * ld, k, 4, idx2 + (size_t)o * k, dist2 + (size_t)o * k, r2);
+        if (rc != ISMHIP_OK) return rc;
+        o += n;
+    }
+    int rc = knn_scan_queue(ctx, cb, ISMHIP_METRIC_L2SQ, k, q2, ld, Q, qrange, idx2, dist2);
+    if (rc != ISMHIP_OK) return rc;
+    if (ctx->timers_on) ISM_HIP(ctx, hipMemcpyAsync(ctx->knn_stats, Q.count, 8, hipMemcpyDeviceToHost, ctx->stream));
+    for (int s = 0; s < S; ++s) {
+        if (!cnt[s]) continue;
+        hipLaunchKernelGGL(k_knn_merge_lists, dim3((cnt[s] + 255) / 256), dim3(256), 0, ctx->stream, (const uint32_t*)list2, off[s], (int)cnt[s], k,
+                           (const int32_t*)idx2, (const float*)dist2, idx_out, dist_out);
+        ISM_CHECK_LAUNCH(ctx, "k_knn_merge_lists");
+    }
+    return ISMHIP_OK;
+}
+
 int run_knn_two_stage(ismhip_ctx* ctx, const ismhip_codebook* cb, int nq, const float* q, int k, int32_t* idx_out, float* dist_out) {
     KnnStage1 s1{};
     KnnRequest r1; r1.stage1 = &s1; r1.use_pca = 1;
@@ -947,15 +1148,20 @@
     if (rc != ISMHIP_OK) return rc;
     KnnStage2 g;
     const bool seed = ctx->knn_stage2_seed;
-    rc = knn_gather_stage2(ctx, cb, s1, q, k, g, seed ? idx_out : nullptr, seed ? dist_out : nullptr);
+    g.want_lists = ctx->knn_stage2_splits && s1.n_splits >= 2 && s1.n_splits <= 16;
+    rc = knn_gather_stage2(ctx, cb, s1, q, k, g, seed ? idx_out : nullptr, seed ? dist_out : nullptr, nq);
     if (rc != ISMHIP_OK || g.n2 == 0) return rc;
+    if (g.want_lists) {
+        bool taken = false;
+        rc = run_knn_stage2_lists(ctx, cb, s1, g.head_d, g.lists_d, g.cnt, g.n2, nq, q, k, idx_out, dist_out, taken);
+        if (rc != ISMHIP_OK || taken) return rc;
+        rc = knn_gather_unsplit(ctx, cb, s1, q, k, g, seed ? idx_out : nullptr, seed ? dist_out : nullptr);
+        if (rc != ISMHIP_OK) return rc;
+    }
     const int n2 = g.n2;
     for (int o = 0; o < n2;) {
-        const int left = n2 - o, n = left >= 32768 ? left / 32768 * 32768 : left;
-        KnnRequest r2; r2.tname = "knn_stage2"; r2.many_splits = n < 4096;
-        r2.use_pca = cb->pca2.m > 0 && !(n < 4096) ? 2 : 0;
-        r2.half = n >= 4096 && n < 32768 && !ctx->knn_stage2_t4;
-        r2.seed_dk = g.dk2 ? g.dk2 + o : nullptr;
+        const int n = knn_stage2_chunk(n2, o);
+        const KnnRequest r2 = knn_stage2_request(ctx, cb, n, g.dk2 ? g.dk2 + o : nullptr);
         rc = run_knn(ctx, cb, ISMHIP_METRIC_L2SQ, n, g.q2 + (size_t)o * cb->dim, k, 4, g.idx2 + (size_t)o * k, g.dist2 + (size_t)o * k, r2);
         if (rc != ISMHIP_OK) return rc;
         o += n;
diff --git a/point-cloud-donkey_amd/csrc/knn_internal.h b/point-cloud-donkey_amd/csrc/knn_internal.h
--- a/point-cloud-donkey_amd/csrc/knn_internal.h
+++ b/point-cloud-donkey_amd/csrc/knn_internal.h
@@ -152,8 +152,13 @@
     const u16 *wh, *wl; const float* word_norm; int n_tiles_m, ld, k_steps;
     const u16 *qh, *ql; int nq; const float* out_scale; int tiles_per_split, n_splits;
     float* cand_val; int* cand_idx; int cand_stride; float* cand_bound; int bound_stride;
+    const int* qrange;
 };
-const void* knn_ring16_kernel(int T, int WR, int QP, int PRE = 0);
+__host__ __device__ inline void knn_range_split(int lo, int hi, int split, int n_splits, int& mt0, int& mt1) {
+    const long long len = hi - lo;
+    mt0 = lo + (int)(len * split / n_splits); mt1 = lo + (int)(len * (split + 1) / n_splits);
+}
+const void* knn_ring16_kernel(int T, int WR, int QP, int PRE = 0, int RNG = 0);
 int knn_ring16_launch(ismhip_ctx* ctx, int T, const void* kern, unsigned grid, int threads, size_t lds, KnnCandArgs a,
                       unsigned int* stream_clock, float* thr0, int pre_step, float pre_relax);
 const void* knn_mfma16_kernel(int T, int mode, bool big_tile);
diff --git a/point-cloud-donkey_amd/csrc/knn_mfma16.hip b/point-cloud-donkey_amd/csrc/knn_mfma16.hip
--- a/point-cloud-donkey_amd/csrc/knn_mfma16.hip
+++ b/point-cloud-donkey_amd/csrc/knn_mfma16.hip
@@ -11,7 +11,8 @@
                                                           int tiles_per_split, int n_splits,
                                                           float* __restrict__ cand_val, int* __restrict__ cand_idx, int cand_stride,
                                                           float* __restrict__ cand_bound, int bound_stride,
-                                                          const float* __restrict__ emit_tau, uint32_t* __restrict__ emit_cnt, uint32_t* __restrict__ emit_list, int emit_cap) {
+                                                          const float* __restrict__ emit_tau, uint32_t* __restrict__ emit_cnt, uint32_t* __restrict__ emit_list, int emit_cap,
+                                                          const int* __restrict__ qrange ) {
     constexpr int BM = WR * MI * 32, BN = WC * NI * 32, NT = WR * WC * 64;
     constexpr int SEGS = KB / 8;
     constexpr int KS = KB / 16;
@@ -34,8 +35,9 @@
     const int xcd = blockIdx.x & 7, jx = blockIdx.x >> 3;
     const int split = jx % n_splits, qtile = (jx / n_splits) * 8 + xcd;
     if (qtile * BN >= nq) return;
-    const int mt0 = split * tiles_per_split;
-    const int mt1 = min(n_tiles_m, mt0 + tiles_per_split);
+    int mt0 = split * tiles_per_split;
+    int mt1 = min(n_tiles_m, mt0 + tiles_per_split);
+    if (qrange) { const int* rg = qrange + 4 * ((qtile * BN) >> 8); knn_range_split(rg[0] / BM, rg[1] / BM, split, n_splits, mt0, mt1); }
     const int nk = (k_steps + KS - 1) / KS;
 
     const int srow = tid / SEGS, sseg = tid % SEGS;
@@ -202,7 +204,7 @@
 int knn_mfma16_launch(ismhip_ctx* ctx, const void* kern, unsigned grid, int threads, size_t lds, KnnCandArgs a,
                       const float* emit_tau, uint32_t* emit_cnt, uint32_t* emit_list, int emit_cap) {
     void* args[] = {&a.wh, &a.wl, &a.word_norm, &a.n_tiles_m, &a.ld, &a.k_steps, &a.qh, &a.ql, &a.nq, &a.out_scale, &a.tiles_per_split, &a.n_splits,
-                    &a.cand_val, &a.cand_idx, &a.cand_stride, &a.cand_bound, &a.bound_stride, &emit_tau, &emit_cnt, &emit_list, &emit_cap};
+                    &a.cand_val, &a.cand_idx, &a.cand_stride, &a.cand_bound, &a.bound_stride, &emit_tau, &emit_cnt, &emit_list, &emit_cap, &a.qrange};
     ISM_HIP(ctx, hipLaunchKernel(kern, dim3(grid), dim3(threads), args, lds, ctx->stream));
     ISM_CHECK_LAUNCH(ctx, (emit_tau ? "k_knn_l2_mfma16<emit>" : "k_knn_l2_mfma16"));
     return ISMHIP_OK;
diff --git a/point-cloud-donkey_amd/csrc/knn_ring16.hip b/point-cloud-donkey_amd/csrc/knn_ring16.hip
--- a/point-cloud-donkey_amd/csrc/knn_ring16.hip
+++ b/point-cloud-donkey_amd/csrc/knn_ring16.hip
@@ -28,13 +28,14 @@
     tp.v[0] = sel_f(c[0], x, tp.v[0]);
     tp.i[0] = sel_i(c[0], idx, tp.i[0]);
 }
-template <int T, int WR = 2, int QP = 0, int PRE = 0>
+template <int T, int WR = 2, int QP = 0, int PRE = 0, int RNG = 0>
 __global__ __launch_bounds__(WR * 256, 2) void k_knn_l2_ring16(const u16* __restrict__ wh, const float* __restrict__ word_norm, int n_tiles_m, int ld, int k_steps,
                                                           const u16* __restrict__ qh, int nq, const float* __restrict__ out_scale,
                                                           int tiles_per_split, int n_splits,
                                                           float* __restrict__ cand_val, int* __restrict__ cand_idx, int cand_stride,
                                                           float* __restrict__ cand_bound, int bound_stride, unsigned int* __restrict__ stream_clock,
-                                                          const float* __restrict__ thr_init, float* __restrict__ thr_out, int tile_step, float thr_relax) {
+                                                          const float* __restrict__ thr_init, float* __restrict__ thr_out, int tile_step, float thr_relax,
+                                                          const int* __restrict__ qrange) {
     using L = Ring16Lds<WR, QP>;
     constexpr int WC = 4, MT = 8, NT = 4, KB = RG_KB, BM = WR * 128, BN = RG_BN;
     constexpr int STAGES = L::STAGES, STAGE_HALVES = L::STAGE_HALVES, CNS = 256;
@@ -54,14 +55,20 @@
     const int xcd = blockIdx.x & 7, jx = blockIdx.x >> 3;
     const int split = jx % n_splits, qtile = (jx / n_splits) * 8 + xcd;
     if (qtile * BN >= nq) return;
-    const int mt0 = split * tiles_per_split;
-    const int n_t = PRE ? (n_tiles_m + tile_step - 1) / tile_step : min(n_tiles_m, mt0 + tiles_per_split) - mt0;
+    int mt0 = split * tiles_per_split, mt1 = min(n_tiles_m, mt0 + tiles_per_split);
+    int clk_slot = xcd * n_splits + split;
+    if (RNG) {
+        const int* rg = qrange + 4 * qtile;
+        knn_range_split(rg[0] / BM, rg[1] / BM, split, n_splits, mt0, mt1);
+        clk_slot = xcd * 64 + ((rg[2] * n_splits + split) & 63);
+    }
+    const int n_t = PRE ? (n_tiles_m + tile_step - 1) / tile_step : mt1 - mt0;
     if (n_t <= 0) return;
     const int nk = (k_steps + 1) / 2;
     const int G = n_t * nk;
     int toff = 0; unsigned c0 = 0u;
     if (stream_clock) {
-        unsigned int* clk = stream_clock + xcd * n_splits + split;
+        unsigned int* clk = stream_clock + clk_slot;
         if (tid == 0) *(volatile unsigned*)ring = __hip_atomic_load(clk, __ATOMIC_RELAXED, __HIP_MEMORY_SCOPE_AGENT);
         __syncthreads();
         c0 = __builtin_amdgcn_readfirstlane(*(volatile unsigned*)ring);
@@ -304,7 +311,11 @@
 }
 
 template <int T>
-const void* ring16_instance(int WR, int QP, int PRE) {
+const void* ring16_instance(int WR, int QP, int PRE, int RNG) {
+    if (RNG) {
+        if constexpr (T == 4) return WR == 1 ? (const void*)k_knn_l2_ring16<4, 1, 0, 0, 1> : (const void*)k_knn_l2_ring16<4, 2, 0, 0, 1>;
+        else return nullptr;
+    }
     if (PRE) return (const void*)k_knn_l2_ring16<T, 2, 0, 1>;
     if (WR == 1) return (const void*)k_knn_l2_ring16<T, 1>;
     return QP ? (const void*)k_knn_l2_ring16<T, 2, 2> : (const void*)k_knn_l2_ring16<T, 2>;
@@ -312,12 +323,12 @@
 
 }
 
-const void* knn_ring16_kernel(int T, int WR, int QP, int PRE) {
+const void* knn_ring16_kernel(int T, int WR, int QP, int PRE, int RNG) {
     switch (T) {
-    case 1: return ring16_instance<1>(WR, QP, PRE);
-    case 2: return ring16_instance<2>(WR, QP, PRE);
-    case 3: return ring16_instance<3>(WR, QP, PRE);
-    case 4: return ring16_instance<4>(WR, QP, PRE);
+    case 1: return ring16_instance<1>(WR, QP, PRE, RNG);
+    case 2: return ring16_instance<2>(WR, QP, PRE, RNG);
+    case 3: return ring16_instance<3>(WR, QP, PRE, RNG);
+    case 4: return ring16_instance<4>(WR, QP, PRE, RNG);
     }
     return nullptr;
 }
@@ -330,14 +341,14 @@
         const size_t plds = Ring16Lds<2, 0>::total(0);
         const int rc2 = ism_lds_cap(ctx, pk, plds);
         if (rc2 != ISMHIP_OK) return rc2;
-        int one = 1, all = a.n_tiles_m; unsigned int* noclk = nullptr; const float* noinit = nullptr;
-        void* pargs[] = {&a.wh, &a.word_norm, &a.n_tiles_m, &a.ld, &a.k_steps, &a.qh, &a.nq, &a.out_scale, &all, &one, &a.cand_val, &a.cand_idx, &a.cand_stride, &a.cand_bound, &a.bound_stride, &noclk, &noinit, &thr0, &pre_step, &pre_relax};
+        int one = 1, all = a.n_tiles_m; unsigned int* noclk = nullptr; const float* noinit = nullptr; const int* norange = nullptr;
+        void* pargs[] = {&a.wh, &a.word_norm, &a.n_tiles_m, &a.ld, &a.k_steps, &a.qh, &a.nq, &a.out_scale, &all, &one, &a.cand_val, &a.cand_idx, &a.cand_stride, &a.cand_bound, &a.bound_stride, &noclk, &noinit, &thr0, &pre_step, &pre_relax, &norange};
         ISM_HIP(ctx, hipLaunchKernel(pk, dim3(grid / a.n_splits), dim3(512), pargs, plds, ctx->stream));
         ISM_CHECK_LAUNCH(ctx, "k_knn_l2_ring16<pre>");
     }
     thr_init = thr0;
     float no_relax = 0.f;
-    void* rargs[] = {&a.wh, &a.word_norm, &a.n_tiles_m, &a.ld, &a.k_steps, &a.qh, &a.nq, &a.out_scale, &a.tiles_per_split, &a.n_splits, &a.cand_val, &a.cand_idx, &a.cand_stride, &a.cand_bound, &a.bound_stride, &stream_clock, &thr_init, &thr_out, &tile_step, &no_relax};
+    void* rargs[] = {&a.wh, &a.word_norm, &a.n_tiles_m, &a.ld, &a.k_steps, &a.qh, &a.nq, &a.out_scale, &a.tiles_per_split, &a.n_splits, &a.cand_val, &a.cand_idx, &a.cand_stride, &a.cand_bound, &a.bound_stride, &stream_clock, &thr_init, &thr_out, &tile_step, &no_relax, &a.qrange};
     ISM_HIP(ctx, hipLaunchKernel(kern, dim3(grid), dim3(threads), rargs, lds, ctx->stream));
     ISM_CHECK_LAUNCH(ctx, "k_knn_l2_ring16");
     return ISMHIP_OK;
```
